# sarpaykent/GotenNet

Measured on AMD Instinct MI355X. Metric: molecules/sec (energy+force forward), rMD17 aspirin batch=128, 1/2/4/8 MI355X, higher is better.
Workload: dtype f32 (2xfp16-split MFMA with block exponents, fp32 accumulate); 1 GPU; rmd17_aspirin batch=128/GPU (N=2688 atoms, E=54368 edges incl. self-loops), n_atom_basis=256, n_interactions=6, lmax=2, n_rbf=32, heads=8, sep_dir/sep_tensor, energy+forces; global_batch=128, parallelism=dp1 (molecule shards, 1 all-reduce)

## Files before the change

gotennet_amd/_lib.py:

```python
from __future__ import annotations

import ctypes as C
import os

_PKG = os.path.dirname(os.path.abspath(__file__))
LIB_PATH = os.environ.get("GN_LIB_PATH") or os.path.join(_PKG, "libgotennet_hip.so")

GN_ERR_BAD_ARG = 10001
ABI_VERSION = 11
LMAX_SLICED = 0x100
LMAX_MEAN, LMAX_MAX = 0x200, 0x400

ACT_NONE = 11
_P, _I, _F, _L, _D = C.c_void_p, C.c_int, C.c_float, C.c_long, C.c_double

class GemmDesc(C.Structure):
    _fields_ = [("A", _P), ("lda", _I), ("W", _P), ("bias", _P), ("C", _P), ("ldc", _I),
                ("M", _I), ("N", _I), ("K", _I), ("act_lo", _I), ("act_hi", _I),
                ("row_cnt", _I), ("row_gstride", _I), ("row_goff", _I),
                ("res", _P), ("gate", _P), ("gate_mode", _I), ("pre_out", _P),
                ("pro_mode", _I), ("pro_lo", _I), ("pro_hi", _I), ("a_pre", _P), ("ldp", _I),
                ("a_gate", _P), ("ldg", _I), ("A2", _P), ("A3", _P), ("a_seg", _I), ("act_kind", _I), ("lda2", _I)]


class WgradDesc(C.Structure):
    _fields_ = [("dY", _P), ("ldy", _I), ("y_off", _I), ("A", _P), ("lda", _I), ("a_off", _I),
                ("dW", _P), ("ldw", _I), ("db", _P), ("rows", _I), ("nout", _I), ("K", _I),
                ("row_cnt", _I), ("row_gstride", _I), ("row_goff", _I)]


SIGNATURES = {
    "gn_abi_version": [C.POINTER(C.c_char_p)],
    "gn_build_csr": [_P, _I, _I, _P, _P, _P, _P],
    "gn_check_edges": [_P, _I, _I, _P, _P],
    "gn_build_csc": [_P, _P, _I, _I, _P, _P, _P, _P, _P],
    "gn_molecule_ptr": [_P, _I, _I, _P, _P],
    "gn_cosine_cutoff": [_P, _I, _F, _P, _P],
    "gn_out_degree": [_P, _I, _P, _P],
    "gn_edge_geometry": [_P, _P, _P, _P, _I, _I, _I, _I, _P, _P, _F, _P, _P, _P, _P],
    "gn_node_init": [_P, _P, _P, _P, _I, _P, _P, _P, _I, _I, _P, _P],
    "gn_edge_init": [_P, _P, _P, _P, _I, _I, _I, _P, _P],
    "gn_layernorm_silu": [_P, _P, _P, _F, _I, _I, _P, _I, _P],
    "gn_layernorm": [_P, _P, _P, _F, _I, _I, _P, _P],
    "gn_tensor_norm": [_P, _P, _F, _I, _I, _I, _P, _P],
    "gn_gemm": [_P, _I, _P, _P, _P, _I, _I, _I, _I, _I, _I, _I, _I, _I, _P, _P, _P],
    "gn_attn_softmax": [_P, _P, _I, _P, _I, _P, _P, _P, _I, _I, _I, _P, _I, _P],
    "gn_attn_softmax_dropout": [_P, _P, _I, _P, _I, _P, _P, _P, _I, _I, _I, _P, _P, _P, _I, _D, _I, _P],
    "gn_attn_dropout_mask": [_P, _I, _D, _L, _I, _P, _P],
    "gn_message_aggregate": [_P, _P, _I, _P, _I, _P, _P, _P, _P, _P, _P, _P, _P, _P, _I, _I, _I, _I, _I, _I, _P],
    "gn_eqff_fused_supported": [_I, _I, _I],
    "gn_eqff_fused_forward": [_P, _P, _P, _P, _P, _F, _I, _I, _I, _P, _P, _P, _P, _P, _I, _P],
    "gn_eqff_fused_backward": [_P, _P, _P, _P, _P, _P, _P, _P, _I, _I, _I, _P, _P, _I, _P],
    "gn_htr_edge": [_P, _P, _P, _P, _P, _I, _I, _I, _I, _P, _P, _P],
    "gn_eqff_context": [_P, _P, _F, _I, _I, _I, _P, _P],
    "gn_eqff_update": [_P, _P, _I, _I, _I, _P, _P, _P],
    "gn_gemm_ex": [_P, _I, _P, _P, _P, _I, _I, _I, _I, _I, _I, _I, _I, _I, _P, _P, _I, _P, _I, _I, _I, _P, _I, _P, _I, _I, _P],
    "gn_gemm_group": [_P, _I, _P],
    "gn_edge_vectors": [_P, _P, _P, _I, _P, _P, _P],
    "gn_gemm_split": [_P, _I, _P, _P, _P, _I, _I, _I, _I, _I, _I, _I, _I, _I, _P, _P, _I, _P, _I, _I, _I, _P, _I, _P, _I, _I, _P],
    "gn_split_bf16x3": [_P, _I, _I, _P, _P],
    "gn_split_bf16x3_size": [_I, _I],
    "gn_gemm_group_split": [_P, _I, _P],
    "gn_gemm_f16x2": [_P, _I, _P, _P, _P, _I, _I, _I, _I, _I, _I, _I, _I, _I, _P, _P, _I, _P, _I, _I, _I, _P, _I, _P, _I, _I, _P],
    "gn_split_f16x2": [_P, _I, _I, _P, _P],
    "gn_split_f16x2_size": [_I, _I],
    "gn_gemm_group_f16x2": [_P, _I, _P],
    "gn_htr_backward": [_P, _P, _P, _P, _P, _P, _P, _P, _P, _P, _P, _P, _I, _I, _I, _I, _P, _P, _P, _P, _I, _P],
    "gn_message_backward": [_P, _P, _I, _P, _I, _P, _P, _I, _P, _P, _P, _P, _P, _P, _P, _P, _P, _P, _P,
                            _P, _P, _P, _I, _P, _P, _P, _P, _P, _P, C.c_long, _I, _I, _I, _I, _I, _I, _I, _P],
    "gn_message_backward_dropout": [_P, _P, _I, _P, _I, _P, _P, _P, _I, _P, _P, _P, _P, _P, _P, _P, _P, _P, _P, _P,
                                    _P, _P, _P, _I, _P, _P, _P, _P, _P, _P, C.c_long, _I, _I, _I, _I, _I, _I, _I, _P],
    "gn_message_backward_groups": [_I, _I, _I, _I],
    "gn_eqff_backward_a": [_P, _P, _P, _P, _I, _I, _I, _P, _P, _P],
    "gn_eqff_backward_b": [_P, _P, _P, _P, _I, _I, _I, _P, _P, _P],
    "gn_edge_init_backward": [_P, _P, _P, _I, _P, _P, _P, _P, _I, _I, _P, _P, _P],
    "gn_node_init_backward": [_P, _P, _P, _I, _P, _P, _P, _P, _I, _I, _P, _P, _P],
    "gn_layernorm_silu_backward": [_P, _P, _P, _F, _P, _I, _I, _P, _I, _P],
    "gn_layernorm_backward": [_P, _P, _F, _P, _I, _I, _P, _P],
    "gn_tensor_norm_backward": [_P, _P, _P, _F, _I, _I, _I, _P, _P],
    "gn_gate": [_P, _I, _L, _P, _P],
    "gn_gate_backward": [_P, _P, _I, _L, _P, _P],
    "gn_edge_gate_backward": [_P, _P, _I, _P, _L, _P, _P, _P],
    "gn_edge_geometry_backward": [_P, _P, _P, _P, _I, _I, _I, _I, _P, _P, _F, _P, _I, _P, _I, _P, _P, _P, _P],
    "gn_pos_scatter": [_P, _P, _P, _P, _P, _P, _I, _F, _P, _P],
    "gn_head_energy": [_P, _P, _F, _F, _F, _F, _P, _P, _P, _I, _I, _P, _P, _I, _P, _I, _P],
    "gn_head_grad": [_P, _P, _F, _P, _I, _I, _P, _I, _P],
    "gn_geb_context": [_P, _I, _I, _P, _I, _I, _I, _P, _I, _P],
    "gn_geb_gate": [_P, _I, _I, _I, _P, _I, _I, _I, _I, _P, _I, _P, _I, _P],
    "gn_dipole_reduce": [_P, _I, _P, _I, _P, _P, _I, _F, _F, _I, _I, _P, _P, _P],
    "gn_ese_reduce": [_P, _P, _P, _P, _I, _P, _I, _P, _P],
    "gn_radius_count": [_P, _P, _I, _F, _I, _P, _P],
    "gn_radius_fill": [_P, _P, _I, _F, _I, _P, C.c_int64, _P, _P, _P, _P],
    "gn_weight_grad_workspace": [_P, _I],
    "gn_weight_grad_group": [_P, _I, _P, _L, _P],
    "gn_embedding_grad": [_P, _P, _I, _P, _P, _P, _P, _P, _P, _I, _I, _I, _P, _P, _P, _P],
    "gn_layernorm_param_grad_workspace": [_I, _I],
    "gn_layernorm_param_grad": [_P, _P, _P, _F, _P, _I, _I, _I, _P, _P, _P, _P],
}

_LONG_RESULT = ("gn_split_bf16x3_size", "gn_split_f16x2_size", "gn_weight_grad_workspace", "gn_layernorm_param_grad_workspace")

_lib = None


class GotenNetHipError(RuntimeError):
    pass


def load():
    global _lib
    if _lib is not None:
        return _lib
    if not os.path.exists(LIB_PATH):
        raise GotenNetHipError(
            f"{LIB_PATH} is missing: the HIP extension has not been built "
            "(python gotennet_amd/build.py). There is no CPU fallback.")
    lib = C.CDLL(LIB_PATH)
    for name, argtypes in SIGNATURES.items():
        fn = getattr(lib, name)
        fn.argtypes = argtypes
        fn.restype = C.c_long if name in _LONG_RESULT else C.c_int
    if lib.gn_abi_version(None) != ABI_VERSION:
        raise GotenNetHipError("libgotennet_hip.so ABI version mismatch; rebuild")
    _lib = lib
    return lib


TIMER = None


def call(name: str, *args) -> None:
    t = TIMER
    tag = t.want(name, args) if t is not None else None
    if tag is not None:
        import torch
        e0, e1 = torch.cuda.Event(enable_timing=True), torch.cuda.Event(enable_timing=True)
        e0.record()
        rc = getattr(load(), name)(*args)
        e1.record()
        t.events.append((tag, e0, e1))
    else:
        rc = getattr(load(), name)(*args)
    if rc != 0:
        what = "unsupported shape/flag combination" if rc == GN_ERR_BAD_ARG else f"hipError_t {rc}"
        raise GotenNetHipError(f"{name} failed: {what}")


def ptr(t) -> int:
    return None if t is None else t.data_ptr()
```

gotennet_amd/csrc/gn_backward.hip:

```cpp
#include "gn_common.h"
#include "gn_tune.h"
#include "gn_sh.h"
#include "gn_highl.h"

namespace gn {



template <int LMAX, int FC = 0>
__global__ __launch_bounds__(256) GN_WPE(GN_W_HTR_TGT) void htr_bwd_target_kernel(
    const float* __restrict__ gtp, const float* __restrict__ pre_t, const float* __restrict__ w,
    const float* __restrict__ EQ, const float* __restrict__ EK, const float* __restrict__ rl,
    const int* __restrict__ rowptr, const int* __restrict__ src, int N, int F_rt,
    float* __restrict__ gEQ, float* __restrict__ g_rl, float* __restrict__ g_pre_t, int ) {
    constexpr int act = GN_ACT_SILU;
    constexpr int D = (LMAX + 1) * (LMAX + 1) - 1;
    constexpr int KP = D <= 4 ? 4 : (D <= 8 ? 8 : (D <= 16 ? 16 : 32));
    constexpr int CH = D < 9 ? D : 9;
    __shared__ __attribute__((aligned(16))) float red[CH * 1024];
    const int F = FC ? FC : F_rt;
    const int i = xcd_item(blockIdx.x, N);
    if (i < 0) return;
    GN_SLOT_GEOMETRY(FC);
    const int e0 = rowptr[i], e1 = rowptr[i + 1];
    float4 eq[D], acc[D];
#pragma unroll
    for (int m = 0; m < D; ++m) { eq[m] = ld4(EQ + ((size_t)i * D + m) * F + c0); acc[m] = zero4(); }
    for (int e = e0 + slot; e < e1; e += ns) {
        const float4 gte = ld4(gtp + (size_t)e * F + c0), pte = ld4(pre_t + (size_t)e * F + c0);
        float4 a_pt, d_pt;
        act_pair4(pte, act, a_pt, d_pt);
        const float4 gw = gte * a_pt;
        st4(g_pre_t + (size_t)e * F + c0, gte * ld4_nt(w + (size_t)e * F + c0) * d_pt);
        const float* kj = EK + (size_t)src[e] * D * F + c0;
        const float* re = rl + (size_t)e * D;
        float part[KP];
#pragma unroll
        for (int m = D; m < KP; ++m) part[m] = 0.f;
        int m0 = 0;
#pragma unroll
        for (int l = 1; l <= LMAX; ++l) {
            float4 ek[2 * LMAX + 1];
            float r[2 * LMAX + 1];
            float4 pa = zero4(), pb = zero4();
            float rr = 0.f;
#pragma unroll
            for (int mm = 0; mm < 2 * l + 1; ++mm) {
                ek[mm] = ld4(kj + (size_t)(m0 + mm) * F);
                r[mm] = re[m0 + mm];
                pa = fma4(r[mm], eq[m0 + mm], pa);
                pb = fma4(r[mm], ek[mm], pb);
                rr = fmaf(r[mm], r[mm], rr);
            }
            const float c = 2.0f - rr;
            const float4 u = gw * pb * (-c), v = gw * pa * (-c), s2 = gw * (pa * pb) * 2.0f;
#pragma unroll
            for (int mm = 0; mm < 2 * l + 1; ++mm) {
                acc[m0 + mm] = fma4(r[mm], u, fma4(gw, ek[mm], acc[m0 + mm]));
                part[m0 + mm] = hsum4(fma4(r[mm], s2, fma4(v, ek[mm], u * eq[m0 + mm])));
            }
            m0 += 2 * l + 1;
        }
        if (lps >= KP) {
            multi_group_sum<KP>(part, lps, lp);
            const int stride = lps / KP;
            if ((lp & (stride - 1)) == 0 && lp / stride < D) g_rl[(size_t)e * D + lp / stride] = part[0];
        } else {
#pragma unroll
            for (int m = 0; m < D; ++m) {
                const float s = group_sum(part[m], lps);
                if (lp == 0) g_rl[(size_t)e * D + m] = s;
            }
        }
    }
    reduce_rows<D>(acc, red, slot, c0, F, ns, [&](int row, float4 s) { st4(gEQ + ((size_t)i * D + row) * F + c0, s); });
}

template <int LMAX, int FC = 0>
__global__ __launch_bounds__(256) GN_WPE(GN_W_HTR_SRC) void htr_bwd_source_kernel(
    const float* __restrict__ gtp, const float* __restrict__ pre_t,
    const float* __restrict__ EQ, const float* __restrict__ EK, const float* __restrict__ rl,
    const int* __restrict__ colptr, const int* __restrict__ perm, const int* __restrict__ dst, int N, int F_rt,
    float* __restrict__ gEK, int ) {
    constexpr int act = GN_ACT_SILU;
    constexpr int D = (LMAX + 1) * (LMAX + 1) - 1;
    constexpr int CH = D < 9 ? D : 9;
    __shared__ __attribute__((aligned(16))) float red[CH * 1024];
    const int F = FC ? FC : F_rt;
    const int j = xcd_item(blockIdx.x, N);
    if (j < 0) return;
    GN_SLOT_GEOMETRY(FC);
    const int p0 = colptr[j], p1 = colptr[j + 1];
    float4 ek[D], acc[D];
#pragma unroll
    for (int m = 0; m < D; ++m) { ek[m] = ld4(EK + ((size_t)j * D + m) * F + c0); acc[m] = zero4(); }
    for (int pp = p0 + slot; pp < p1; pp += ns) {
        const int e = perm[pp];
        const float4 gw = ld4(gtp + (size_t)e * F + c0) * act4(ld4(pre_t + (size_t)e * F + c0), act);
        const float* qi = EQ + (size_t)dst[pp] * D * F + c0;
        const float* re = rl + (size_t)e * D;
        int m0 = 0;
#pragma unroll
        for (int l = 1; l <= LMAX; ++l) {
            float4 eq[2 * LMAX + 1];
            float r[2 * LMAX + 1];
            float4 pa = zero4();
            float rr = 0.f;
#pragma unroll
            for (int mm = 0; mm < 2 * l + 1; ++mm) {
                eq[mm] = ld4(qi + (size_t)(m0 + mm) * F);
                r[mm] = re[m0 + mm];
                pa = fma4(r[mm], eq[mm], pa);
                rr = fmaf(r[mm], r[mm], rr);
            }
            const float4 v = gw * pa * (rr - 2.0f);
#pragma unroll
            for (int mm = 0; mm < 2 * l + 1; ++mm)
                acc[m0 + mm] = fma4(r[mm], v, fma4(gw, eq[mm], acc[m0 + mm]));
            m0 += 2 * l + 1;
        }
    }
    reduce_rows<D>(acc, red, slot, c0, F, ns, [&](int row, float4 s) { st4(gEK + ((size_t)j * D + row) * F + c0, s); });
}

template <int LMAX, bool SEP_DIR, bool SEP_TENSOR>
struct MsgShape {
    static constexpr int D = (LMAX + 1) * (LMAX + 1) - 1;
    static constexpr int ND = SEP_DIR ? LMAX : 1;
    static constexpr int NT = SEP_TENSOR ? LMAX : 1;
    static constexpr int M = 1 + ND + NT;
    __host__ __device__ static constexpr bool is_dir(int b) { return b >= 1 && b < 1 + ND; }
    __host__ __device__ static constexpr int lo(int b) { return is_dir(b) ? (SEP_DIR ? b : 1) : (SEP_TENSOR ? b - ND : 1); }
    __host__ __device__ static constexpr int hi(int b) { return is_dir(b) ? (SEP_DIR ? b : LMAX) : (SEP_TENSOR ? b - ND : LMAX); }
    __host__ __device__ static constexpr int first_row(int l) { return l * l - 1; }
};


constexpr int GS_CAP = 2048;
template <int LMAX, bool SEP_DIR, bool SEP_TENSOR, bool GS_LDS, bool FIRST, int FC>
__device__ __forceinline__ void msg_bwd_target_body(const MsgBwdArgs& p, float* gsl, float* red, float* hsum, const float* __restrict__ x_, const float* __restrict__ v_, const float* __restrict__ eproj_, const float* __restrict__ a_, const float* __restrict__ qk_, const float* __restrict__ X_in_, const float* __restrict__ rl_, const float* __restrict__ cut_, const int* __restrict__ outdeg_, const float* __restrict__ g_h1_, const float* __restrict__ g_X1_, const int* __restrict__ rowptr_, const int* __restrict__ src_, float* __restrict__ g_eproj_, float* __restrict__ g_s_, float* __restrict__ g_nproj_, float* __restrict__ g_rl_, float* __restrict__ g_cut_) {
    using S = MsgShape<LMAX, SEP_DIR, SEP_TENSOR>;
    constexpr int D = S::D, M = S::M;
    constexpr int KP = D <= 4 ? 4 : (D <= 8 ? 8 : (D <= 16 ? 16 : 32));
    const int N = p.N, F = FC ? FC : p.F, H = p.H;
    const int i = xcd_item(blockIdx.x, N);
    if (i < 0) return;
    GN_SLOT_GEOMETRY(FC);
    const int e0 = rowptr_[i], e1 = rowptr_[i + 1];
    const int per_head = (M * F) / H;
    int hb[M];
#pragma unroll
    for (int b = 0; b < M; ++b) hb[b] = (b * F + c0) / per_head;
    auto GS = [&](int e, int h) -> float& {
        if constexpr (GS_LDS) return gsl[(e - e0) * H + h];
        else return g_s_[(size_t)e * H + h];
    };

    const float4 gdh = ld4(g_h1_ + (size_t)i * F + c0);
    float4 gdX[D];
#pragma unroll
    for (int m = 0; m < D; ++m) gdX[m] = ld4(g_X1_ + ((size_t)i * D + m) * F + c0);

    for (int e = e0 + slot; e < e1; e += ns) {
        const int j = src_[e];
        const float ce = cut_[e];
        const float* xr = x_ + (size_t)j * p.ldxv + c0;
        const float* vr = v_ + (size_t)j * p.ldxv + c0;
        const float* tr = eproj_ + (size_t)e * p.lde + F + c0;
        float* gtr = g_eproj_ + (size_t)e * p.lde + F + c0;
        const float* ar = a_ + (size_t)e * H;
        const float* Xj = X_in_ + (size_t)j * D * F + c0;
        const float* re = rl_ + (size_t)e * D;
        float pa_h[M];
        float cutp = 0.f;
        float rlp[D];
#pragma unroll
        for (int b = 0; b < M; ++b) {
            if (FIRST && b > 0 && !S::is_dir(b)) { pa_h[b] = 0.f; continue; }
            float4 go;
            if (b == 0) {
                go = gdh;
            } else {
                go = zero4();
#pragma unroll
                for (int l = S::lo(b); l <= S::hi(b); ++l)
#pragma unroll
                    for (int m = S::first_row(l); m < S::first_row(l) + 2 * l + 1; ++m)
                        go = S::is_dir(b) ? fma4(re[m], gdX[m], go) : fma4(gdX[m], ld4(Xj + (size_t)m * F), go);
            }
            const float4 tfb = ld4(tr + b * F), xb = ld4(xr + b * F), vb = ld4(vr + b * F);
            st4_nt(gtr + b * F, (go * xb) * ce);
            cutp += hsum4(go * tfb * xb);
            pa_h[b] = hsum4(go * vb);
            if (S::is_dir(b)) {
                const float4 od = fma4(ar[hb[b]], vb, (tfb * xb) * ce);
#pragma unroll
                for (int l = S::lo(b); l <= S::hi(b); ++l)
#pragma unroll
                    for (int m = S::first_row(l); m < S::first_row(l) + 2 * l + 1; ++m) rlp[m] = hsum4(gdX[m] * od);
            }
        }
        cutp = group_sum(cutp, lps);
        if (lp == 0) g_cut_[e] = cutp;
        {
            float* hrow = hsum + slot * (M * lps);
#pragma unroll
            for (int b = 0; b < M; ++b) hrow[b * lps + lp] = pa_h[b];
            const int rpl = lps / H, hh = lp / rpl, part = lp - hh * rpl;
            const float* hp = hrow + hh * (M * rpl) + part * M;
            float hv = hp[0];
#pragma unroll
            for (int k = 1; k < M; ++k) hv += hp[k];
            hv = group_sum(hv, rpl);
            if (part == 0) GS(e, hh) = hv;
        }
// ... 817 lines not shown
        if (basis == 0) {
            const float u = expf(alpha * (-d));
            auto term = [&](int r, float gp) {
                const float w = u - means[r];
                const float G = expf(-betas[r] * (w * w));
                s += gp * G * (dc + c * (2.0f * betas[r] * w * alpha * u));
            };
            if ((R & 3) == 0) {
                for (int r = 0; r < R; r += 4) {
                    const float4 gp = ld4(g_phi + (size_t)e * R + r);
                    term(r, gp.x); term(r + 1, gp.y); term(r + 2, gp.z); term(r + 3, gp.w);
                }
            } else {
                for (int r = 0; r < R; ++r) term(r, g_phi[(size_t)e * R + r]);
            }
        }
        float gc = 0.f;
        int q = 0;
        for (; q + 4 <= n_cut; q += 4) {
            const float c0 = g_cut[(size_t)q * E + e], c1 = g_cut[(size_t)(q + 1) * E + e];
            const float c2 = g_cut[(size_t)(q + 2) * E + e], c3 = g_cut[(size_t)(q + 3) * E + e];
            gc += c0; gc += c1; gc += c2; gc += c3;
        }
        for (; q < n_cut; ++q) gc += g_cut[(size_t)q * E + e];
        gd += s + gc * dc;
    }
    g_diff[e] = gd;
    const float x = vec[3 * e], y = vec[3 * e + 1], z = vec[3 * e + 2];
    const float n = sqrtf(x * x + y * y + z * z);
    const float ux = x / n, uy = y / n, uz = z / n;
    Dual3 o[D];
    real_harmonics<LMAX, Dual3>(Dual3{ux, {1.f, 0.f, 0.f}}, Dual3{uy, {0.f, 1.f, 0.f}}, Dual3{uz, {0.f, 0.f, 1.f}}, o);
    float gsum[D];
#pragma unroll
    for (int m = 0; m < D; ++m) gsum[m] = 0.f;
#pragma unroll 2
    for (int q = 0; q < n_rl; ++q) {
        const float* row = g_rl + ((size_t)q * E + e) * D;
        if constexpr (D % 4 == 0) {
#pragma unroll
            for (int m = 0; m < D; m += 4) {
                const float4 v = ld4(row + m);
                gsum[m] += v.x; gsum[m + 1] += v.y; gsum[m + 2] += v.z; gsum[m + 3] += v.w;
            }
        } else {
#pragma unroll
            for (int m = 0; m < D; ++m) gsum[m] += row[m];
        }
    }
    float gu0 = 0.f, gu1 = 0.f, gu2 = 0.f;
#pragma unroll
    for (int m = 0; m < D; ++m) {
        gu0 += gsum[m] * o[m].d[0]; gu1 += gsum[m] * o[m].d[1]; gu2 += gsum[m] * o[m].d[2];
    }
    const float dotp = gu0 * ux + gu1 * uy + gu2 * uz;
    g_vec[3 * e] = (gu0 - dotp * ux) / n;
    g_vec[3 * e + 1] = (gu1 - dotp * uy) / n;
    g_vec[3 * e + 2] = (gu2 - dotp * uz) / n;
}

__global__ __launch_bounds__(256) void pos_scatter_kernel(const float* __restrict__ g_vec, const float* __restrict__ g_diff,
                                                          const float* __restrict__ vec,
                                                          const int* __restrict__ rowptr, const int* __restrict__ colptr,
                                                          const int* __restrict__ perm, int N, float sign, float* __restrict__ g_pos) {
    const int n = blockIdx.x * 4 + (threadIdx.x >> 6), lane = threadIdx.x & 63;
    if (n >= N) return;
    float sx = 0.f, sy = 0.f, sz = 0.f;
    auto add = [&](int e, float w) {
        const float x = vec[3 * e], y = vec[3 * e + 1], z = vec[3 * e + 2];
        const float gd = g_diff[e];
        float rx = g_vec[3 * e], ry = g_vec[3 * e + 1], rz = g_vec[3 * e + 2];
        if (gd != 0.f) {
            const float q = gd / sqrtf(x * x + y * y + z * z);
            rx += q * x; ry += q * y; rz += q * z;
        }
        sx += w * rx; sy += w * ry; sz += w * rz;
    };
    const int p0 = colptr[n], p1 = colptr[n + 1], e0 = rowptr[n], e1 = rowptr[n + 1];
    for (int pp = p0 + lane; pp < p1; pp += 64) add(perm[pp], 1.0f);
    for (int e = e0 + lane; e < e1; e += 64) add(e, -1.0f);
    sx = wave_sum(sx); sy = wave_sum(sy); sz = wave_sum(sz);
    if (lane == 0) {
        g_pos[3 * n] = sign * sx;
        g_pos[3 * n + 1] = sign * sy;
        g_pos[3 * n + 2] = sign * sz;
    }
}

__global__ __launch_bounds__(1024) void head_energy_kernel(
    const float* __restrict__ pre1, const float* __restrict__ W2, float b2, float scale, float shift, float mol_shift,
    const float* __restrict__ atomref, const int* __restrict__ z, const int* __restrict__ mol_ptr,
    int Hd, float* __restrict__ y, float* __restrict__ energy, int mean, float* __restrict__ atom_scale, int act) {
    const int b = blockIdx.x;
    const int n0 = mol_ptr[b], n1 = mol_ptr[b + 1];
    const int wave = threadIdx.x >> 6, lane = threadIdx.x & 63;
    for (int n = n0 + wave; n < n1; n += 16) {
        float s = 0.f;
        for (int k = lane; k < Hd; k += 64) s += act1(pre1[(size_t)n * Hd + k], act) * W2[k];
        s = wave_sum(s);
        if (lane == 0) y[n] = (s + b2) * scale + shift + (atomref ? atomref[z[n]] : 0.f);
    }
    __syncthreads();
    if (wave == 0) {
        float s = 0.f;
        for (int n = n0 + lane; n < n1; n += 64) s += y[n];
        s = wave_sum(s);
        if (lane == 0) energy[b] = ((mean && n1 > n0) ? s / (float)(n1 - n0) : s) + mol_shift;
    }
    if (atom_scale)
        for (int n = n0 + (int)threadIdx.x; n < n1; n += 1024) atom_scale[n] = mean ? 1.0f / (float)(n1 - n0) : 1.0f;
}

__global__ void head_grad_kernel(const float* __restrict__ pre1, const float* __restrict__ W2, float scale,
                                 const float* __restrict__ atom_scale, int N, int Hd, float* __restrict__ gpre1, int act) {
    const size_t idx = (size_t)blockIdx.x * blockDim.x + threadIdx.x;
    if (idx >= (size_t)N * Hd) return;
    const float sc = atom_scale ? scale * atom_scale[idx / Hd] : scale;
    gpre1[idx] = sc * W2[idx % Hd] * dact1(pre1[idx], act);
}

}

static bool bwd_dim_ok_wide(int F) { return F >= 16 && F <= 1024 && gn::is_pow2(F); }

#define GN_SWITCH_LMAX(KERNEL, grid, block, st, ...)                                                   \
    switch (lmax) {                                                                                    \
        case 1: hipLaunchKernelGGL(gn::KERNEL<1>, grid, block, 0, st, __VA_ARGS__); break;             \
        case 2: hipLaunchKernelGGL(gn::KERNEL<2>, grid, block, 0, st, __VA_ARGS__); break;             \
        case 3: hipLaunchKernelGGL(gn::KERNEL<3>, grid, block, 0, st, __VA_ARGS__); break;             \
        default: hipLaunchKernelGGL(gn::KERNEL<4>, grid, block, 0, st, __VA_ARGS__); break;            \
    }

#define GN_SWITCH_LMAX8(KERNEL, grid, block, st, ...)                                                  \
    switch (lmax) {                                                                                    \
        case 1: hipLaunchKernelGGL(gn::KERNEL<1>, grid, block, 0, st, __VA_ARGS__); break;             \
        case 2: hipLaunchKernelGGL(gn::KERNEL<2>, grid, block, 0, st, __VA_ARGS__); break;             \
        case 3: hipLaunchKernelGGL(gn::KERNEL<3>, grid, block, 0, st, __VA_ARGS__); break;             \
        case 4: hipLaunchKernelGGL(gn::KERNEL<4>, grid, block, 0, st, __VA_ARGS__); break;             \
        case 5: hipLaunchKernelGGL(gn::KERNEL<5>, grid, block, 0, st, __VA_ARGS__); break;             \
        case 6: hipLaunchKernelGGL(gn::KERNEL<6>, grid, block, 0, st, __VA_ARGS__); break;             \
        case 7: hipLaunchKernelGGL(gn::KERNEL<7>, grid, block, 0, st, __VA_ARGS__); break;             \
        default: hipLaunchKernelGGL(gn::KERNEL<8>, grid, block, 0, st, __VA_ARGS__); break;            \
    }

extern "C" int gn_htr_backward(const float* g_t_out, const float* pre_t, const float* w, const float* w_raw,
                               const float* EQ,
                               const float* EK, const float* rl, const int* rowptr, const int* src, const int* dst,
                               const int* colptr, const int* perm, int N, int F, int lmax_arg, int mode,
                               float* gEQ, float* gEK, float* g_rl, float* g_pre_t, int act, void* stream) {
    const int lmax = lmax_arg & 0xff;
    if ((lmax_arg & ~(0xff | GN_LMAX_SLICED)) || !bwd_dim_ok_wide(F) || N < 0 || lmax < 1 || lmax > 8 || mode < 0 || mode > 31 ||
        act < 0 || act >= GN_ACT_COUNT)
        return GN_ERR_BAD_ARG;
    if (N == 0) return GN_OK;
    hipStream_t st = (hipStream_t)stream;
    if (gn_use_highl(lmax_arg) || F > 256 || (!mode && act != GN_ACT_SILU))
        return gn_highl_htr_backward(g_t_out, pre_t, w, w_raw, EQ, EK, rl, rowptr, src, dst, colptr, perm, N, F, lmax,
                                     mode, gEQ, gEK, g_rl, g_pre_t, act, st);
    if (mode)
        return gn_htr_backward_general(g_t_out, pre_t, w, w_raw, EQ, EK, rl, rowptr, src, dst, colptr, perm, N, F, lmax,
                                       mode, gEQ, gEK, g_rl, g_pre_t, act, st);
    const dim3 grid(gn::xcd_grid(N)), block(256);
#define GN_HTRB_T(L, LLO, LHI, FIRST, FC)                                                                        \
    hipLaunchKernelGGL((gn::htr_bwd_target_group_kernel<L, LLO, LHI, FIRST, FC>), grid, block, 0, st, g_t_out, pre_t, w, \
                       EQ, EK, rl, rowptr, src, N, F, gEQ, g_rl, g_pre_t, act)
#define GN_HTRB_S(L, LLO, LHI, FC)                                                                               \
    hipLaunchKernelGGL((gn::htr_bwd_source_group_kernel<L, LLO, LHI, FC>), grid, block, 0, st, g_t_out, pre_t, EQ, EK, \
                       rl, colptr, perm, dst, N, F, gEK, act)
#define GN_HTRB(L, LLO, LHI, FIRST, FC) GN_HTRB_T(L, LLO, LHI, FIRST, FC); GN_HTRB_S(L, LLO, LHI, FC)
#define GN_HTRB_ALL(FC)                                                                                          \
    if (lmax == 1) {                                                                                             \
        hipLaunchKernelGGL((gn::htr_bwd_target_kernel<1, FC>), grid, block, 0, st, g_t_out, pre_t, w, EQ, EK, rl, rowptr, src, N, F, gEQ, g_rl, g_pre_t, act); \
        hipLaunchKernelGGL((gn::htr_bwd_source_kernel<1, FC>), grid, block, 0, st, g_t_out, pre_t, EQ, EK, rl, colptr, perm, dst, N, F, gEK, act); \
    } else if (lmax == 2) {                                                                                      \
        hipLaunchKernelGGL((gn::htr_bwd_target_kernel<2, FC>), grid, block, 0, st, g_t_out, pre_t, w, EQ, EK, rl, rowptr, src, N, F, gEQ, g_rl, g_pre_t, act); \
        hipLaunchKernelGGL((gn::htr_bwd_source_kernel<2, FC>), grid, block, 0, st, g_t_out, pre_t, EQ, EK, rl, colptr, perm, dst, N, F, gEK, act); \
    } else if (lmax == 3) {                                                                                      \
        if (GN_HTRB_TGT_MODE == 1) { GN_HTRB_T(3, 1, 3, true, FC); }                                             \
        else { GN_HTRB_T(3, 1, 2, true, FC); GN_HTRB_T(3, 3, 3, false, FC); }                                    \
        if (GN_HTRB_SRC_ONE) { GN_HTRB_S(3, 1, 3, FC); }                                                         \
        else { GN_HTRB_S(3, 1, 2, FC); GN_HTRB_S(3, 3, 3, FC); }                                                 \
    } else {                                                                                                     \
        GN_HTRB_T(4, 1, 2, true, FC);                                                                            \
        if (GN_HTRB_TGT_MODE == 1) { GN_HTRB_T(4, 3, 4, false, FC); }                                            \
        else { GN_HTRB_T(4, 3, 3, false, FC); GN_HTRB_T(4, 4, 4, false, FC); }                                   \
        if (GN_HTRB_SRC_ONE) { GN_HTRB_S(4, 1, 4, FC); }                                                         \
        else { GN_HTRB_S(4, 1, 2, FC); GN_HTRB_S(4, 3, 3, FC); GN_HTRB_S(4, 4, 4, FC); }                         \
    }
    if (F == 256) { GN_HTRB_ALL(256) } else { GN_HTRB_ALL(0) }
    GN_LAUNCH_CHECK();
    return GN_OK;
}

template <int L, int LLO, int LHI, bool SC, int FC>
static inline void gn_launch_msg_bwd_group(dim3 grid, dim3 block, hipStream_t st, const gn::MsgBwdArgs& p, float* ga_slice, float* cut_slice) {
    if constexpr (LLO == 3 && LHI == 3)
        hipLaunchKernelGGL((gn::msg_bwd_merged_group3_kernel<L, LLO, LHI, SC, FC>), grid, block, 0, st, p, ga_slice, cut_slice);
    else
        hipLaunchKernelGGL((gn::msg_bwd_merged_group_kernel<L, LLO, LHI, SC, FC>), grid, block, 0, st, p, ga_slice, cut_slice);
}
template <int L, bool SD, bool ST, int FC>
static inline void gn_launch_msg_bwd_merged(dim3 grid, dim3 block, hipStream_t st, const gn::MsgBwdArgs& p, float* ga_parts) {
    if constexpr (!(L >= 3 && SD && ST))
        hipLaunchKernelGGL((gn::msg_bwd_merged_kernel<L, SD, ST, FC>), grid, block, 0, st, p, ga_parts);
}
#define GN_MSGB_LAUNCH_FC(L, SD, ST, FC)                                                                 \
    do {                                                                                                  \
        if (!X_in) {                                                                                      \
            if (GN_MSGB_MERGED_FIRST && ga_parts != nullptr) {    \
                hipLaunchKernelGGL((gn::msg_bwd_merged_first_kernel<L, SD, ST, FC>), grid, block, 0, st, p, ga_parts); \
                hipLaunchKernelGGL(gn::attn_bwd_kernel<FC>, grid, block, 0, st, p, ga_parts, 1, (size_t)0); \
                hipLaunchKernelGGL(gn::msg_bwd_gk_kernel<FC>, grid, block, 0, st, p);                     \
                break;                                                                                    \
            }                                                                                             \
            hipLaunchKernelGGL((gn::msg_bwd_target_kernel<L, SD, ST, true, FC>), grid, block, 0, st, p);  \
            hipLaunchKernelGGL((gn::msg_bwd_source_kernel<L, SD, ST, true, FC>), grid, block, 0, st, p);  \
            break;                                                                                        \
        }                                                                                                 \
        if (GN_MSGB_MERGED && ga_parts != nullptr) {      \
            gn_launch_msg_bwd_merged<L, SD, ST, FC>(grid, block, st, p, ga_parts);                        \
            hipLaunchKernelGGL(gn::attn_bwd_kernel<FC>, grid, block, 0, st, p, ga_parts, 1, (size_t)0);   \
            hipLaunchKernelGGL(gn::msg_bwd_gk_kernel<FC>, grid, block, 0, st, p);                         \
            break;                                                                                        \
        }                                                                                                 \
        hipLaunchKernelGGL((gn::msg_bwd_target_kernel<L, SD, ST>), grid, block, 0, st, p);                \
        hipLaunchKernelGGL((gn::msg_bwd_source_kernel<L, SD, ST>), grid, block, 0, st, p);                \
    } while (0)
#define GN_MSGB_LAUNCH(L, SD, ST) GN_MSGB_LAUNCH_FC(L, SD, ST, 0)
#define GN_MSGB_LAUNCH_DEFAULT(L)                                                                        \
    do {                                                                                                  \
        if (F == 256) GN_MSGB_LAUNCH_FC(L, true, true, 256); else GN_MSGB_LAUNCH_FC(L, true, true, 0);    \
    } while (0)

extern "C" int gn_message_backward_groups(int lmax_arg, int sep_dir, int sep_tensor, int act) {
    const int lmax = lmax_arg & 0xff;
    if (gn_use_highl(lmax_arg) || act != GN_ACT_SILU) return 1;
    return (lmax >= 3 && sep_dir && sep_tensor) ? lmax - 1 : 1;
}

static int message_backward(
    const float* x, const float* v, int ldxv, const float* eproj, int lde, const float* a,
    const float* qk, int ldqk, const float* X_in, const float* rl, const float* cut, const int* outdeg,
    const float* g_h1, const float* g_X1,
    const int* rowptr, const int* src, const int* dst, const int* colptr, const int* perm,
    float* g_eproj, float* g_s, float* g_nproj, int ldn, float* g_x, float* g_v, float* g_X_out,
    float* g_rl, float* g_cut, float* ga_parts, long E,
    int N, int F, int H, int lmax_arg, int sep_dir, int sep_tensor, int act, void* stream, const float* a_soft) {
    const int lmax = lmax_arg & 0xff;
    const bool amax = (lmax_arg & GN_LMAX_MAX) != 0;
    if (amax && ((lmax_arg & GN_LMAX_MEAN) || !ga_parts || !X_in)) return GN_ERR_BAD_ARG;
    if ((lmax_arg & ~(0xff | GN_LMAX_SLICED | GN_LMAX_MEAN | GN_LMAX_MAX)) || !bwd_dim_ok_wide(F) || N < 0 || H <= 0 || !gn::is_pow2(H) || (F / 4) % H || (F / 4) / H > 64 || lmax < 1 || lmax > 8 ||
        (ldxv & 3) || (lde & 3) || (ldqk & 3) || (ldn & 3) || g_X_out == g_X1 || act < 0 || act >= GN_ACT_COUNT)
        return GN_ERR_BAD_ARG;
    if (!X_in && (act != GN_ACT_SILU || gn_use_highl(lmax_arg) || F > 256)) return GN_ERR_BAD_ARG;
    if (N == 0) return GN_OK;
    gn::MsgBwdArgs p{x, v, ldxv, eproj, lde, a, qk, ldqk, X_in, rl, cut, outdeg, g_h1, g_X1,
                     rowptr, src, dst, colptr, perm, g_eproj, g_s, g_nproj, ldn, g_x, g_v, g_X_out, g_rl, g_cut,
                     N, F, H, (float)(1.0 / sqrt((double)F)), act, (lmax_arg & GN_LMAX_MEAN) ? 1 : 0, amax ? ga_parts : nullptr, a_soft};
    hipStream_t st = (hipStream_t)stream;
    const dim3 grid(gn::xcd_grid(N)), block(256);
    if (gn_use_highl(lmax_arg) || F > 256 || act != GN_ACT_SILU) return gn_highl_message_backward(p, lmax, sep_dir, sep_tensor, st);
    if (X_in && gn_message_backward_groups(lmax_arg, sep_dir, sep_tensor, act) > 1) {
        if (ga_parts == nullptr || E <= 0) return GN_ERR_BAD_ARG;
        const size_t gs = (size_t)E * H;
#define GN_MSGB_M(L, LLO, LHI, SC, G, FC)                                                                    \
    gn_launch_msg_bwd_group<L, LLO, LHI, SC, FC>(grid, block, st, p, ga_parts + (size_t)(G) * gs, g_cut + (size_t)(G) * E)
#define GN_MSGB_GROUPS(FC)                                                                                       \
        if (lmax == 3) { GN_MSGB_M(3, 1, 2, true, 0, FC); GN_MSGB_M(3, 3, 3, false, 1, FC); }                    \
        else { GN_MSGB_M(4, 1, 2, true, 0, FC); GN_MSGB_M(4, 3, 3, false, 1, FC); GN_MSGB_M(4, 4, 4, false, 2, FC); } \
        hipLaunchKernelGGL(gn::attn_bwd_kernel<FC>, grid, block, 0, st, p, ga_parts, lmax - 1, gs);              \
        hipLaunchKernelGGL(gn::msg_bwd_gk_kernel<FC>, grid, block, 0, st, p);
        if (F == 256) { GN_MSGB_GROUPS(256) } else { GN_MSGB_GROUPS(0) }
        GN_LAUNCH_CHECK();
        return GN_OK;
    }
    const int key = lmax * 4 + (sep_dir ? 2 : 0) + (sep_tensor ? 1 : 0);
    switch (key) {
        case 4: case 5: case 6: case 7:
            if (F == 256) GN_MSGB_LAUNCH_FC(1, false, false, 256); else GN_MSGB_LAUNCH(1, false, false);
            break;
        case 8: GN_MSGB_LAUNCH(2, false, false); break;
        case 9: GN_MSGB_LAUNCH(2, false, true); break;
        case 10: GN_MSGB_LAUNCH(2, true, false); break;
        case 11: GN_MSGB_LAUNCH_DEFAULT(2); break;
        case 12: GN_MSGB_LAUNCH(3, false, false); break;
        case 13: GN_MSGB_LAUNCH(3, false, true); break;
        case 14: GN_MSGB_LAUNCH(3, true, false); break;
        case 15: GN_MSGB_LAUNCH_DEFAULT(3); break;
        case 16: GN_MSGB_LAUNCH(4, false, false); break;
        case 17: GN_MSGB_LAUNCH(4, false, true); break;
        case 18: GN_MSGB_LAUNCH(4, true, false); break;
        default: GN_MSGB_LAUNCH_DEFAULT(4); break;
    }
    GN_LAUNCH_CHECK();
    return GN_OK;
}

extern "C" int gn_message_backward(
    const float* x, const float* v, int ldxv, const float* eproj, int lde, const float* a,
    const float* qk, int ldqk, const float* X_in, const float* rl, const float* cut, const int* outdeg,
    const float* g_h1, const float* g_X1,
    const int* rowptr, const int* src, const int* dst, const int* colptr, const int* perm,
    float* g_eproj, float* g_s, float* g_nproj, int ldn, float* g_x, float* g_v, float* g_X_out,
    float* g_rl, float* g_cut, float* ga_parts, long E,
    int N, int F, int H, int lmax_arg, int sep_dir, int sep_tensor, int act, void* stream) {
    return message_backward(x, v, ldxv, eproj, lde, a, qk, ldqk, X_in, rl, cut, outdeg, g_h1, g_X1, rowptr, src, dst, colptr,
                            perm, g_eproj, g_s, g_nproj, ldn, g_x, g_v, g_X_out, g_rl, g_cut, ga_parts, E, N, F, H, lmax_arg,
                            sep_dir, sep_tensor, act, stream, nullptr);
}

extern "C" int gn_message_backward_dropout(
    const float* x, const float* v, int ldxv, const float* eproj, int lde, const float* a, const float* a_soft,
    const float* qk, int ldqk, const float* X_in, const float* rl, const float* cut, const int* outdeg,
    const float* g_h1, const float* g_X1,
    const int* rowptr, const int* src, const int* dst, const int* colptr, const int* perm,
    float* g_eproj, float* g_s, float* g_nproj, int ldn, float* g_x, float* g_v, float* g_X_out,
    float* g_rl, float* g_cut, float* ga_parts, long E,
    int N, int F, int H, int lmax_arg, int sep_dir, int sep_tensor, int act, void* stream) {
    if (!a_soft) return GN_ERR_BAD_ARG;
    return message_backward(x, v, ldxv, eproj, lde, a, qk, ldqk, X_in, rl, cut, outdeg, g_h1, g_X1, rowptr, src, dst, colptr,
                            perm, g_eproj, g_s, g_nproj, ldn, g_x, g_v, g_X_out, g_rl, g_cut, ga_parts, E, N, F, H, lmax_arg,
                            sep_dir, sep_tensor, act, stream, a_soft);
}

extern "C" int gn_eqff_backward_a(const float* g_h, const float* g_X, const float* m, const float* Xp,
                                  int N, int F, int D, float* g_m, float* g_Xp, void* stream) {
    if (N < 0 || F <= 0 || (F & 3) || D <= 0) return GN_ERR_BAD_ARG;
    if (N == 0) return GN_OK;
// ... 107 lines not shown
```

gotennet_amd/csrc/gn_gata.hip:

```cpp
#include "gn_common.h"
#include "gn_tune.h"
#include "gn_highl.h"
#include "gn_dropout.h"

namespace gn {

constexpr int ATTN_CAP = 2048;
template <bool IN_LDS, bool ASILU, bool DROP = false>
__device__ __forceinline__ void attn_softmax_body(
    const float* __restrict__ q, const float* __restrict__ k, int ldqk, const float* __restrict__ ta, int ldt,
    const int* __restrict__ src, const int* __restrict__ outdeg, int i, int e0, int e1, int F, int H, float inv_sqrt_f,
    float* __restrict__ a, float* sc, int act, const AttnDrop drop = AttnDrop{}) {
    unsigned dk0 = 0, dk1 = 0;
    if constexpr (DROP) {
        const unsigned long long key = (unsigned long long)drop.key[0];
        dk0 = (unsigned)key, dk1 = (unsigned)(key >> 32);
    }
    auto mult = [&](size_t n) { return drop_mult(dk0, dk1, drop.layer, drop.thresh, drop.scale, drop.all, n); };
    const int lps = F >> 2, ns = 256 / lps;
    const int slot = threadIdx.x / lps, lp = threadIdx.x % lps, c0 = lp * 4;
    const int lph = lps / H;
    auto S = [&](int e, int h) -> float& {
        if constexpr (IN_LDS) return sc[(e - e0) * H + h];
        else if constexpr (DROP) return drop.a_soft[(size_t)e * H + h];
        else return a[(size_t)e * H + h];
    };
    const float4 qi = ld4(q + (size_t)i * ldqk + c0);
    for (int e = e0 + slot; e < e1; e += 2 * ns) {
        const int eb = e + ns < e1 ? e + ns : e;
        const int ja = src[e], jb = src[eb];
        const float4 ka = ld4(k + (size_t)ja * ldqk + c0), kb = ld4(k + (size_t)jb * ldqk + c0);
        const float4 ta_ = act4(ld4_nt(ta + (size_t)e * ldt + c0), act);
        const float4 tb_ = act4(ld4_nt(ta + (size_t)eb * ldt + c0), act);
        float pa = qi.x * ka.x * ta_.x;
        pa += qi.y * ka.y * ta_.y;
        pa += qi.z * ka.z * ta_.z;
        pa += qi.w * ka.w * ta_.w;
        float pb = qi.x * kb.x * tb_.x;
        pb += qi.y * kb.y * tb_.y;
        pb += qi.z * kb.z * tb_.z;
        pb += qi.w * kb.w * tb_.w;
        pa = group_sum(pa, lph);
        pb = group_sum(pb, lph);
        if ((lp & (lph - 1)) == 0) {
            S(e, lp / lph) = pa;
            if (eb != e) S(eb, lp / lph) = pb;
        }
    }
    __syncthreads();
    const int wave = threadIdx.x >> 6, lane = threadIdx.x & 63;
    for (int h = wave; h < H; h += 4) {
        float mx = -INFINITY;
        for (int e = e0 + lane; e < e1; e += 64) mx = fmaxf(mx, S(e, h));
        mx = wave_max(mx);
        float sm = 0.f;
        for (int e = e0 + lane; e < e1; e += 64) {
            const float ex = fast_exp(S(e, h) - mx);
            S(e, h) = ex;
            sm += ex;
        }
        const float rsm = __builtin_amdgcn_rcpf(wave_sum(sm) + 1e-16f);
        for (int e = e0 + lane; e < e1; e += 64) {
            const float nrm = outdeg ? sqrtf((float)outdeg[src[e]]) * inv_sqrt_f : inv_sqrt_f;
            S(e, h) = S(e, h) * rsm * nrm;
            if constexpr (DROP && !IN_LDS) a[(size_t)e * H + h] = S(e, h) * mult((size_t)e * H + h);
        }
    }
    if constexpr (IN_LDS) {
        __syncthreads();
        const int n = (e1 - e0) * H;
        for (int idx = threadIdx.x; idx < n; idx += 256) {
            if constexpr (DROP) {
                drop.a_soft[(size_t)e0 * H + idx] = sc[idx];
                a[(size_t)e0 * H + idx] = sc[idx] * mult((size_t)e0 * H + idx);
            } else {
                a[(size_t)e0 * H + idx] = sc[idx];
            }
        }
    }
}

template <bool ASILU>
__global__ __launch_bounds__(256) GN_WPE(GN_W_ATTN) void attn_softmax_kernel(
    const float* __restrict__ q, const float* __restrict__ k, int ldqk,
    const float* __restrict__ ta, int ldt,
    const int* __restrict__ rowptr, const int* __restrict__ src, const int* __restrict__ outdeg,
    int N, int F, int H, float inv_sqrt_f, float* __restrict__ a, int act_rt) {
    __shared__ float sc[ATTN_CAP];
    const int act = ASILU ? (int)GN_ACT_SILU : act_rt;
    const int i = xcd_item(blockIdx.x, N);
    if (i < 0) return;
    const int e0 = rowptr[i], e1 = rowptr[i + 1];
    if ((e1 - e0) * H <= ATTN_CAP)
        attn_softmax_body<true, ASILU>(q, k, ldqk, ta, ldt, src, outdeg, i, e0, e1, F, H, inv_sqrt_f, a, sc, act);
    else
        attn_softmax_body<false, ASILU>(q, k, ldqk, ta, ldt, src, outdeg, i, e0, e1, F, H, inv_sqrt_f, a, sc, act);
}

template <bool ASILU>
__global__ __launch_bounds__(256) void attn_softmax_drop_kernel(
    const float* __restrict__ q, const float* __restrict__ k, int ldqk,
    const float* __restrict__ ta, int ldt,
    const int* __restrict__ rowptr, const int* __restrict__ src, const int* __restrict__ outdeg,
    int N, int F, int H, float inv_sqrt_f, float* __restrict__ a, int act_rt, const AttnDrop drop) {
    __shared__ float sc[ATTN_CAP];
    const int act = ASILU ? (int)GN_ACT_SILU : act_rt;
    const int i = xcd_item(blockIdx.x, N);
    if (i < 0) return;
    const int e0 = rowptr[i], e1 = rowptr[i + 1];
    if ((e1 - e0) * H <= ATTN_CAP)
        attn_softmax_body<true, ASILU, true>(q, k, ldqk, ta, ldt, src, outdeg, i, e0, e1, F, H, inv_sqrt_f, a, sc, act, drop);
    else
        attn_softmax_body<false, ASILU, true>(q, k, ldqk, ta, ldt, src, outdeg, i, e0, e1, F, H, inv_sqrt_f, a, sc, act, drop);
}

constexpr int ATTN_W_STRIP = 512;
template <bool IN_LDS, bool ASILU, int FC, bool DROP = false>
__device__ __forceinline__ void attn_softmax_wave_body(
    const float* __restrict__ q, const float* __restrict__ k, int ldqk, const float* __restrict__ ta, int ldt,
    const int* __restrict__ src, const int* __restrict__ outdeg, int i, int e0, int e1, int F_rt, int H, float inv_sqrt_f,
    float* __restrict__ a, float* sc, int act, const AttnDrop drop = AttnDrop{}) {
    const int F = FC ? FC : F_rt;
    const int lane = threadIdx.x & 63;
    const int lps = F >> 2, ns = 64 / lps;
    const int slot = FC == 256 ? 0 : lane / lps, lp = lane % lps, c0 = lp * 4;
    const int lph = lps / H;
    float* const S = IN_LDS ? sc : (DROP ? drop.a_soft : a) + (size_t)e0 * H;
    const int n = (e1 - e0) * H;
    const float4 qi = ld4(q + (size_t)i * ldqk + c0);
    constexpr int U = 8;
    for (int eb = e0; eb < e1; eb += U * ns) {
        float4 kj[U], te[U];
        int ee[U];
#pragma unroll
        for (int u = 0; u < U; ++u) {
            const int e = eb + u * ns + slot;
            ee[u] = e < e1 ? e : e1 - 1;
            kj[u] = ld4(k + (size_t)src[ee[u]] * ldqk + c0);
            te[u] = ld4_nt(ta + (size_t)ee[u] * ldt + c0);
        }
#pragma unroll
        for (int u = 0; u < U; ++u) {
            const float4 t4 = act4(te[u], act);
            float p = qi.x * kj[u].x * t4.x;
            p += qi.y * kj[u].y * t4.y;
            p += qi.z * kj[u].z * t4.z;
            p += qi.w * kj[u].w * t4.w;
            p = group_sum(p, lph);
            if ((lp & (lph - 1)) == 0 && eb + u * ns + slot < e1) S[(ee[u] - e0) * H + lp / lph] = p;
        }
    }
    if constexpr (!IN_LDS) __builtin_amdgcn_s_waitcnt(0);
    __builtin_amdgcn_wave_barrier();
    float mx = -INFINITY;
    for (int idx = lane; idx < n; idx += 64) mx = fmaxf(mx, S[idx]);
    mx = stride_max(mx, H);
// ... 107 lines not shown
    for (int e = e0 + slot; e < e1; e += ns) {
        const int j = src[e];
        const float ce = cut[e];
        const float* xr = x + (size_t)j * ldxv + c0;
        const float* vr = v + (size_t)j * ldxv + c0;
        const float* tr = tf + (size_t)e * ldt + c0;
        const float* ar = a + (size_t)e * H;
        const float* Xj = X_in + (size_t)j * D * F + c0;
        const float* re = rl + (size_t)e * D;
        float4 o[M];
#pragma unroll
        for (int b = 0; b < (FIRST ? 1 + ND : M); ++b) {
            const float4 sp = (ld4_nt(tr + b * F) * ld4(xr + b * F)) * ce;
            const float ab = ar[hb[b]];
            o[b] = fma4(ab, ld4(vr + b * F), sp);
        }
        acc[0] = acc[0] + o[0];
        int m = 0;
#pragma unroll
        for (int l = 1; l <= LMAX; ++l) {
            const float4 od = o[SEP_DIR ? l : 1];
#pragma unroll
            for (int mm = 0; mm < 2 * l + 1; ++mm, ++m) {
                if constexpr (FIRST)
                    acc[1 + m] = acc[1 + m] + od * re[m];
                else
                    acc[1 + m] = acc[1 + m] + fma4(ld4(Xj + (size_t)m * F), o[1 + ND + (SEP_TENSOR ? l - 1 : 0)], od * re[m]);
            }
        }
    }

#pragma unroll
    for (int base = 0; base < ROWS; base += CH) {
        if (base) __syncthreads();
#pragma unroll
        for (int r = 0; r < CH; ++r)
            if (base + r < ROWS) st4(&red[r * 1024 + slot * F + c0], acc[base + r]);
        __syncthreads();
        for (int r = slot; r < CH && base + r < ROWS; r += ns) {
            const float4 s = red4(red + r * 1024, c0, F, ns);
            const int row = base + r;
            if (row == 0) {
                st4(h_out + (size_t)i * F + c0, ld4(h_in + (size_t)i * F + c0) + s);
            } else {
                const size_t off = ((size_t)i * D + (row - 1)) * F + c0;
                if constexpr (FIRST) st4(X_out + off, s);
                else st4(X_out + off, ld4(X_in + off) + s);
            }
        }
    }
}

template <int LMAX, bool SEP_DIR, bool SEP_TENSOR, int LLO, int LHI, bool SCALAR, int FC>
__device__ __forceinline__ void message_aggregate_group_body(
    const float* __restrict__ x, const float* __restrict__ v, int ldxv,
    const float* __restrict__ tf, int ldt, const float* __restrict__ a,
    const float* __restrict__ rl, const float* __restrict__ cut,
    const int* __restrict__ rowptr, const int* __restrict__ src,
    const float* __restrict__ h_in, const float* __restrict__ X_in,
    float* __restrict__ h_out, float* __restrict__ X_out, int N, int F_rt, int H) {
    constexpr int D = (LMAX + 1) * (LMAX + 1) - 1;
    constexpr int ND = SEP_DIR ? LMAX : 1;
    constexpr int NT = SEP_TENSOR ? LMAX : 1;
    constexpr int M = 1 + ND + NT;
    constexpr int XROWS = (LHI + 1) * (LHI + 1) - LLO * LLO;
    constexpr int ROWS = (SCALAR ? 1 : 0) + XROWS;
    constexpr int M0 = LLO * LLO - 1;
    constexpr int CH = ROWS < GN_K6G_CH ? ROWS : GN_K6G_CH;
    __shared__ __attribute__((aligned(16))) float red[CH * 1024];

    const int F = FC ? FC : F_rt;
    const int i = xcd_item(blockIdx.x, N);
    if (i < 0) return;
    GN_SLOT_GEOMETRY(FC);
    const int e0 = rowptr[i], e1 = rowptr[i + 1];
    const int per_head = (M * F) / H;

    int hb[M];
#pragma unroll
    for (int b = 0; b < M; ++b) hb[b] = (b * F + c0) / per_head;

    float4 acc[ROWS];
#pragma unroll
    for (int r = 0; r < ROWS; ++r) acc[r] = zero4();

    for (int e = e0 + slot; e < e1; e += ns) {
        const int j = src[e];
        const float ce = cut[e];
        const float* xr = x + (size_t)j * ldxv + c0;
        const float* vr = v + (size_t)j * ldxv + c0;
        const float* tr = tf + (size_t)e * ldt + c0;
        const float* ar = a + (size_t)e * H;
        const float* Xj = X_in + (size_t)j * D * F + c0;
        const float* re = rl + (size_t)e * D;
        auto gate = [&](int b) {
            const float4 sp = (ld4_nt(tr + b * F) * ld4(xr + b * F)) * ce;
            const float ab = ar[hb[b]];
            return fma4(ab, ld4(vr + b * F), sp);
        };
        constexpr int NL = LHI - LLO + 1;
        float4 gd[NL], gt[NL];
#pragma unroll
        for (int l = LLO; l <= LHI; ++l) {
            gd[l - LLO] = (SEP_DIR || l == LLO) ? gate(SEP_DIR ? l : 1) : gd[0];
            gt[l - LLO] = (SEP_TENSOR || l == LLO) ? gate(1 + ND + (SEP_TENSOR ? l - 1 : 0)) : gt[0];
        }
        if (SCALAR) acc[0] = acc[0] + gate(0);
#pragma unroll
        for (int l = LLO; l <= LHI; ++l) {
#pragma unroll
            for (int mm = 0; mm < 2 * l + 1; ++mm) {
                const int m = l * l - 1 + mm;
                acc[(SCALAR ? 1 : 0) + m - M0] = acc[(SCALAR ? 1 : 0) + m - M0] +
                                                 fma4(ld4(Xj + (size_t)m * F), gt[l - LLO], gd[l - LLO] * re[m]);
            }
        }
    }

#pragma unroll
    for (int base = 0; base < ROWS; base += CH) {
        if (base) __syncthreads();
#pragma unroll
        for (int r = 0; r < CH; ++r)
            if (base + r < ROWS) st4(&red[r * 1024 + slot * F + c0], acc[base + r]);
        __syncthreads();
        for (int r = slot; r < CH && base + r < ROWS; r += ns) {
            const float4 s = red4(red + r * 1024, c0, F, ns);
            const int row = base + r;
            if (SCALAR && row == 0) {
                st4(h_out + (size_t)i * F + c0, ld4(h_in + (size_t)i * F + c0) + s);
            } else {
                const size_t off = ((size_t)i * D + (M0 + row - (SCALAR ? 1 : 0))) * F + c0;
                st4(X_out + off, ld4(X_in + off) + s);
            }
        }
    }
}

#define GN_MSG_GROUP_ARGS                                                                                   \
    const float *__restrict__ x, const float *__restrict__ v, int ldxv, const float *__restrict__ tf, int ldt,            \
        const float *__restrict__ a, const float *__restrict__ rl, const float *__restrict__ cut, const int *__restrict__ rowptr,    \
        const int *__restrict__ src, const float *__restrict__ h_in, const float *__restrict__ X_in,                     \
        float *__restrict__ h_out, float *__restrict__ X_out, int N, int F, int H
#define GN_MSG_GROUP_PASS x, v, ldxv, tf, ldt, a, rl, cut, rowptr, src, h_in, X_in, h_out, X_out, N, F, H
template <int LMAX, bool SEP_DIR, bool SEP_TENSOR, int LLO, int LHI, bool SCALAR, int FC = 0>
__global__ __launch_bounds__(256) GN_WPE(GN_W_K6_G) void message_aggregate_group_kernel(GN_MSG_GROUP_ARGS) {
    message_aggregate_group_body<LMAX, SEP_DIR, SEP_TENSOR, LLO, LHI, SCALAR, FC>(GN_MSG_GROUP_PASS);
}
template <int LMAX, bool SEP_DIR, bool SEP_TENSOR, int LLO, int LHI, bool SCALAR, int FC = 0>
__global__ __launch_bounds__(256) GN_WPE(GN_W_K6_G34) void message_aggregate_group34_kernel(GN_MSG_GROUP_ARGS) {
    message_aggregate_group_body<LMAX, SEP_DIR, SEP_TENSOR, LLO, LHI, SCALAR, FC>(GN_MSG_GROUP_PASS);
}

template <int LMAX, int FC = 0>
__global__ __launch_bounds__(256) GN_WPE(GN_W_HTR_EDGE) void htr_edge_kernel(
    const float* __restrict__ EQ, const float* __restrict__ EK, const float* __restrict__ rl,
    const int* __restrict__ rowptr, const int* __restrict__ src, int N, int F_rt, float* __restrict__ w) {
    constexpr int D = (LMAX + 1) * (LMAX + 1) - 1;
    constexpr bool CLOSED = LMAX == 3 && GN_HTR_CLOSED;
    const int F = FC ? FC : F_rt;
    const int i = xcd_item(blockIdx.x, N);
    if (i < 0) return;
    GN_SLOT_GEOMETRY(FC);
    const int e0 = rowptr[i], e1 = rowptr[i + 1];
    float4 eq[D];
#pragma unroll
    for (int m = 0; m < D; ++m) eq[m] = ld4(EQ + ((size_t)i * D + m) * F + c0);
    for (int e = e0 + slot; e < e1; e += ns) {
        const float* kj = EK + (size_t)src[e] * D * F + c0;
        const float* re = rl + (size_t)e * D;
        float4 wsum = zero4();
        int m0 = 0;
#if GN_HTR_CLOSED_ALL
        if constexpr (LMAX >= GN_HTR_CLOSED_ALL) {
            float4 eka[D];
            float ra[D];
#pragma unroll
            for (int m = 0; m < D; ++m) { eka[m] = ld4(kj + (size_t)m * F); ra[m] = re[m]; }
            __builtin_amdgcn_sched_barrier(0);
#pragma unroll
            for (int l = 1; l <= LMAX; ++l) {
                float4 pq = zero4(), pk = zero4(), ab = zero4();
                float rr = 0.f;
#pragma unroll
                for (int mm = 0; mm < 2 * l + 1; ++mm) {
                    const int m = l * l - 1 + mm;
                    rr = fmaf(ra[m], ra[m], rr);
                    pq = fma4(ra[m], eq[m], pq);
                    pk = fma4(ra[m], eka[m], pk);
                    ab = fma4(eq[m], eka[m], ab);
                }
                wsum = wsum + (ab + (pq * pk) * (rr - 2.0f));
            }
            st4_nt(w + (size_t)e * F + c0, wsum);
            continue;
        }
#endif
#pragma unroll
        for (int l = 1; l <= LMAX; ++l) {
            float4 ek[2 * LMAX + 1];
            float r[2 * LMAX + 1];
            float4 pq = zero4(), pk = zero4();
            if constexpr (CLOSED) {
                float4 ab = zero4();
                float rr = 0.f;
#pragma unroll
                for (int mm = 0; mm < 2 * l + 1; ++mm) {
                    ek[mm] = ld4(kj + (size_t)(m0 + mm) * F);
                    r[mm] = re[m0 + mm];
                }
#pragma unroll
                for (int mm = 0; mm < 2 * l + 1; ++mm) {
                    rr = fmaf(r[mm], r[mm], rr);
                    pq = fma4(r[mm], eq[m0 + mm], pq);
                    pk = fma4(r[mm], ek[mm], pk);
                    ab = fma4(eq[m0 + mm], ek[mm], ab);
                }
                wsum = wsum + (ab + (pq * pk) * (rr - 2.0f));
            } else {
#pragma unroll
                for (int mm = 0; mm < 2 * l + 1; ++mm) {
                    ek[mm] = ld4(kj + (size_t)(m0 + mm) * F);
                    r[mm] = re[m0 + mm];
                    pq = fma4(r[mm], eq[m0 + mm], pq);
                    pk = fma4(-r[mm], ek[mm], pk);
                }
#pragma unroll
                for (int mm = 0; mm < 2 * l + 1; ++mm) {
                    const float4 a_ = eq[m0 + mm] + pq * (-r[mm]);
                    const float4 b_ = ek[mm] + pk * r[mm];
                    wsum = fma4(a_, b_, wsum);
                }
            }
            m0 += 2 * l + 1;
        }
        st4_nt(w + (size_t)e * F + c0, wsum);
    }
}

}

static bool feature_dim_ok(int F) { return F >= 16 && F <= 1024 && gn::is_pow2(F); }

extern "C" int gn_attn_softmax(const float* q, const float* k, int ldqk, const float* t_attn, int ldt,
                               const int* rowptr, const int* src, const int* outdeg,
                               int N, int F, int H, float* a, int act, void* stream) {
    if (!feature_dim_ok(F) || N < 0 || H <= 0 || !gn::is_pow2(H) || (F / 4) % H || (F / 4) / H > 64 ||
        (ldqk & 3) || (ldt & 3) || act < 0 || act >= GN_ACT_COUNT)
        return GN_ERR_BAD_ARG;
    if (N == 0) return GN_OK;
    const float inv_sqrt_f = (float)(1.0 / sqrt((double)F));
    if (GN_ATTN_WAVE && F <= 256 && H <= 64) {
        const dim3 grid(gn::xcd_grid((N + 3) / 4)), block(256);
        if (act == GN_ACT_SILU && F == 256)
            hipLaunchKernelGGL((gn::attn_softmax_wave_kernel<true, 256>), grid, block, 0, (hipStream_t)stream,
                               q, k, ldqk, t_attn, ldt, rowptr, src, outdeg, N, F, H, inv_sqrt_f, a, act);
        else if (act == GN_ACT_SILU)
            hipLaunchKernelGGL(gn::attn_softmax_wave_kernel<true>, grid, block, 0, (hipStream_t)stream,
                               q, k, ldqk, t_attn, ldt, rowptr, src, outdeg, N, F, H, inv_sqrt_f, a, act);
        else
            hipLaunchKernelGGL(gn::attn_softmax_wave_kernel<false>, grid, block, 0, (hipStream_t)stream,
                               q, k, ldqk, t_attn, ldt, rowptr, src, outdeg, N, F, H, inv_sqrt_f, a, act);
        GN_LAUNCH_CHECK();
        return GN_OK;
    }
    if (act == GN_ACT_SILU)
        hipLaunchKernelGGL(gn::attn_softmax_kernel<true>, dim3(gn::xcd_grid(N)), dim3(256), 0, (hipStream_t)stream,
                           q, k, ldqk, t_attn, ldt, rowptr, src, outdeg, N, F, H, inv_sqrt_f, a, act);
    else
        hipLaunchKernelGGL(gn::attn_softmax_kernel<false>, dim3(gn::xcd_grid(N)), dim3(256), 0, (hipStream_t)stream,
                           q, k, ldqk, t_attn, ldt, rowptr, src, outdeg, N, F, H, inv_sqrt_f, a, act);
    GN_LAUNCH_CHECK();
    return GN_OK;
}

static bool drop_params(double p, unsigned& thresh, float& scale, int& all) {
    if (!(p >= 0.0)) return false;
    all = p >= 1.0 ? 1 : 0;
    thresh = all ? 0xffffffffu : (unsigned)floor(p * 4294967296.0);
    scale = all ? 0.f : (float)(1.0 / (1.0 - p));
    return true;
}

extern "C" int gn_attn_softmax_dropout(const float* q, const float* k, int ldqk, const float* t_attn, int ldt,
                                       const int* rowptr, const int* src, const int* outdeg,
                                       int N, int F, int H, float* a_soft, float* a, const long long* key, int layer, double p,
                                       int act, void* stream) {
    gn::AttnDrop d{a_soft, key, (unsigned)layer, 0u, 0.f, 0};
    if (!feature_dim_ok(F) || N < 0 || H <= 0 || !gn::is_pow2(H) || (F / 4) % H || (F / 4) / H > 64 ||
        (ldqk & 3) || (ldt & 3) || act < 0 || act >= GN_ACT_COUNT || !key || !a_soft || a_soft == a || layer < 0 ||
        !drop_params(p, d.thresh, d.scale, d.all))
        return GN_ERR_BAD_ARG;
    if (N == 0) return GN_OK;
    const float inv_sqrt_f = (float)(1.0 / sqrt((double)F));
    if (GN_ATTN_WAVE && F <= 256 && H <= 64) {
        const dim3 grid(gn::xcd_grid((N + 3) / 4)), block(256);
        if (act == GN_ACT_SILU)
            hipLaunchKernelGGL(gn::attn_softmax_drop_wave_kernel<true>, grid, block, 0, (hipStream_t)stream,
                               q, k, ldqk, t_attn, ldt, rowptr, src, outdeg, N, F, H, inv_sqrt_f, a, act, d);
        else
            hipLaunchKernelGGL(gn::attn_softmax_drop_wave_kernel<false>, grid, block, 0, (hipStream_t)stream,
                               q, k, ldqk, t_attn, ldt, rowptr, src, outdeg, N, F, H, inv_sqrt_f, a, act, d);
        GN_LAUNCH_CHECK();
        return GN_OK;
    }
    if (act == GN_ACT_SILU)
        hipLaunchKernelGGL(gn::attn_softmax_drop_kernel<true>, dim3(gn::xcd_grid(N)), dim3(256), 0, (hipStream_t)stream,
                           q, k, ldqk, t_attn, ldt, rowptr, src, outdeg, N, F, H, inv_sqrt_f, a, act, d);
    else
        hipLaunchKernelGGL(gn::attn_softmax_drop_kernel<false>, dim3(gn::xcd_grid(N)), dim3(256), 0, (hipStream_t)stream,
                           q, k, ldqk, t_attn, ldt, rowptr, src, outdeg, N, F, H, inv_sqrt_f, a, act, d);
    GN_LAUNCH_CHECK();
    return GN_OK;
}

extern "C" int gn_attn_dropout_mask(const long long* key, int layer, double p, long E, int H, float* m_out, void* stream) {
    unsigned thresh; float scale; int all;
    if (!key || layer < 0 || E < 0 || H <= 0 || !drop_params(p, thresh, scale, all)) return GN_ERR_BAD_ARG;
    const unsigned long long n = (unsigned long long)E * (unsigned long long)H;
    if (n == 0) return GN_OK;
    const unsigned long long blocks = (n + 255) / 256;
    hipLaunchKernelGGL(gn::attn_dropout_mask_kernel, dim3((unsigned)(blocks < 65536 ? blocks : 65536)), dim3(256), 0,
                       (hipStream_t)stream, key, (unsigned)layer, thresh, scale, all, n, m_out);
    GN_LAUNCH_CHECK();
    return GN_OK;
}

#define GN_MSG_ONE(L, SD, ST, LLO, LHI, SC, FC)                                                                 \
    hipLaunchKernelGGL((gn::message_aggregate_group_kernel<L, SD, ST, LLO, LHI, SC, FC>), dim3(gn::xcd_grid(N)), dim3(256), \
                       0, (hipStream_t)stream, x, v, ldxv, t_filter, ldt, a, rl, cut, rowptr, src, h_in, X_in,      \
                       h_out, X_out, N, F, H)
#define GN_MSG_MONO(L, SD, ST, FC)                                                                          \
    if (X_in)                                                                                                   \
        hipLaunchKernelGGL((gn::message_aggregate_kernel<L, SD, ST, false, FC>), dim3(gn::xcd_grid(N)), dim3(256), 0, \
                           (hipStream_t)stream, x, v, ldxv, t_filter, ldt, a, rl, cut, rowptr, src, h_in, X_in, \
                           h_out, X_out, N, F, H);                                                              \
    else                                                                                                        \
        hipLaunchKernelGGL((gn::message_aggregate_kernel<L, SD, ST, true, FC>), dim3(gn::xcd_grid(N)), dim3(256), 0,  \
                           (hipStream_t)stream, x, v, ldxv, t_filter, ldt, a, rl, cut, rowptr, src, h_in, X_in, \
                           h_out, X_out, N, F, H)
#define GN_MSG_LAUNCH_FC(L, SD, ST, FC)                                   \
    do {                                                                  \
        if (L <= 2 || !X_in) { GN_MSG_MONO(L, SD, ST, FC); }   \
        else {                                                            \
            GN_MSG_ONE(L, SD, ST, 1, 2, true, FC);                        \
            if constexpr (L >= 4 && GN_K6_MERGE34) {                      \
                hipLaunchKernelGGL((gn::message_aggregate_group34_kernel<L, SD, ST, 3, 4, false, FC>), dim3(gn::xcd_grid(N)), \
                                   dim3(256), 0, (hipStream_t)stream, x, v, ldxv, t_filter, ldt, a, rl, cut, rowptr, src, \
                                   h_in, X_in, h_out, X_out, N, F, H);    \
            }                                                             \
            else {                                                        \
                GN_MSG_ONE(L, SD, ST, 3, 3, false, FC);                   \
                if constexpr (L >= 4) { GN_MSG_ONE(L, SD, ST, 4, 4, false, FC); } \
            }                                                             \
        }                                                                 \
    } while (0)
#define GN_MSG_LAUNCH(L, SD, ST) GN_MSG_LAUNCH_FC(L, SD, ST, 0)
#define GN_MSG_LAUNCH_DEFAULT(L)                                                                 \
    do {                                                                                          \
        if (F == 256) GN_MSG_LAUNCH_FC(L, true, true, 256); else GN_MSG_LAUNCH_FC(L, true, true, 0); \
    } while (0)

extern "C" int gn_message_aggregate(const float* x, const float* v, int ldxv, const float* t_filter, int ldt,
                                    const float* a, const float* rl, const float* cut,
                                    const int* rowptr, const int* src,
                                    const float* h_in, const float* X_in, float* h_out, float* X_out,
                                    int N, int F, int H, int lmax_arg, int sep_dir, int sep_tensor, void* stream) {
    const int lmax = lmax_arg & 0xff;
    const int aggr = (lmax_arg & GN_LMAX_MEAN) ? 1 : ((lmax_arg & GN_LMAX_MAX) ? 2 : 0);
    if ((lmax_arg & ~(0xff | GN_LMAX_SLICED | GN_LMAX_MEAN | GN_LMAX_MAX)) ||
        ((lmax_arg & GN_LMAX_MEAN) && (lmax_arg & GN_LMAX_MAX)) || !feature_dim_ok(F) || N < 0 || H <= 0 || lmax < 1 ||
        lmax > 8 || (ldxv & 3) || (ldt & 3) || X_in == X_out)
        return GN_ERR_BAD_ARG;
    if (!X_in && gn_use_highl(lmax_arg)) return GN_ERR_BAD_ARG;
    const int M = 1 + (sep_dir ? lmax : 1) + (sep_tensor ? lmax : 1);
    if ((M * F) % H || ((M * F) / H) % 4) return GN_ERR_BAD_ARG;
    if (N == 0) return GN_OK;
    if (gn_use_highl(lmax_arg))
        return gn_highl_message(x, v, ldxv, t_filter, ldt, a, rl, cut, rowptr, src, h_in, X_in, h_out, X_out, N, F, H,
                                lmax, sep_dir, sep_tensor, aggr, (hipStream_t)stream);
    const int key = lmax * 4 + (sep_dir ? 2 : 0) + (sep_tensor ? 1 : 0);
    switch (key) {
        case 4: case 5: case 6: case 7:
            if (F == 256) GN_MSG_LAUNCH_FC(1, false, false, 256); else GN_MSG_LAUNCH(1, false, false);
            break;
        case 8: GN_MSG_LAUNCH(2, false, false); break;
        case 9: GN_MSG_LAUNCH(2, false, true); break;
        case 10: GN_MSG_LAUNCH(2, true, false); break;
        case 11: GN_MSG_LAUNCH_DEFAULT(2); break;
        case 12: GN_MSG_LAUNCH(3, false, false); break;
        case 13: GN_MSG_LAUNCH(3, false, true); break;
        case 14: GN_MSG_LAUNCH(3, true, false); break;
        case 15: GN_MSG_LAUNCH_DEFAULT(3); break;
        case 16: GN_MSG_LAUNCH(4, false, false); break;
        case 17: GN_MSG_LAUNCH(4, false, true); break;
        case 18: GN_MSG_LAUNCH(4, true, false); break;
        default: GN_MSG_LAUNCH_DEFAULT(4); break;
    }
    GN_LAUNCH_CHECK();
    return GN_OK;
}

extern "C" int gn_htr_edge(const float* EQ, const float* EK, const float* rl, const int* rowptr, const int* src,
                           int N, int F, int lmax_arg, int mode, float* w_raw, float* w, void* stream) {
    const int lmax = lmax_arg & 0xff;
    if ((lmax_arg & ~(0xff | GN_LMAX_SLICED)) || !feature_dim_ok(F) || N < 0 || lmax < 1 || lmax > 8 || mode < 0 || mode > 15)
        return GN_ERR_BAD_ARG;
    if (N == 0) return GN_OK;
    hipStream_t st = (hipStream_t)stream;
    if (gn_use_highl(lmax_arg)) return gn_highl_htr_edge(EQ, EK, rl, rowptr, src, N, F, lmax, mode, w_raw, w, st);
    if (mode) return gn_htr_edge_general(EQ, EK, rl, rowptr, src, N, F, lmax, mode, w_raw, w, st);
    const dim3 grid(gn::xcd_grid(N)), block(256);
#define GN_HTR_EDGE(FC)                                                                                                  \
    switch (lmax) {                                                                                                      \
        case 1: hipLaunchKernelGGL((gn::htr_edge_kernel<1, FC>), grid, block, 0, st, EQ, EK, rl, rowptr, src, N, F, w); break; \
        case 2: hipLaunchKernelGGL((gn::htr_edge_kernel<2, FC>), grid, block, 0, st, EQ, EK, rl, rowptr, src, N, F, w); break; \
        case 3: hipLaunchKernelGGL((gn::htr_edge_kernel<3, FC>), grid, block, 0, st, EQ, EK, rl, rowptr, src, N, F, w); break; \
        default: hipLaunchKernelGGL((gn::htr_edge_kernel<4, FC>), grid, block, 0, st, EQ, EK, rl, rowptr, src, N, F, w); break; \
    }
    if (F == 256) { GN_HTR_EDGE(256) } else { GN_HTR_EDGE(0) }
    GN_LAUNCH_CHECK();
    return GN_OK;
}
```

gotennet_amd/csrc/gn_gemm.h:

```cpp
#pragma once
#include "gn_common.h"

namespace gn {

typedef float f32x16 __attribute__((ext_vector_type(16)));

struct GemmArgs {
    const float* A; const float* W; const float* bias; float* C;
    const float* res; const float* gate; float* pre_out;
    const float* a_pre; const float* a_gate;
    int lda, ldc, ldp, ldg, M, N, K;
    int act_lo, act_hi;
    int pro_mode, pro_lo, pro_hi;
    int row_cnt, row_gstride, row_goff;
    int gate_mode;
    const float* A2; const float* A3; int a_seg;
    int nt_store;
    int act_kind;
    int lda2;
};

constexpr int GN_MAX_GROUP = 4;
struct GroupArgs {
    GemmArgs g[GN_MAX_GROUP];
    int tile_end[GN_MAX_GROUP];
    int n;
    int spread;
};

constexpr int BK = 32, PITCH = 36;

typedef __bf16 bf16x8 __attribute__((ext_vector_type(8)));
typedef __bf16 bf16x4 __attribute__((ext_vector_type(4)));
constexpr int SPLIT_PB = 40;

__device__ __forceinline__ unsigned pack_hi16(float a, float b) {
    return __builtin_amdgcn_perm(__float_as_uint(b), __float_as_uint(a), 0x07060302u);
}
__device__ __forceinline__ float trunc_bf16(float x) { return __uint_as_float(__float_as_uint(x) & 0xffff0000u); }
__device__ __forceinline__ void split4_trunc(float4 v, bf16x4& hi, bf16x4& mid, bf16x4& lo) {
    const float r0 = v.x - trunc_bf16(v.x), r1 = v.y - trunc_bf16(v.y);
    const float r2 = v.z - trunc_bf16(v.z), r3 = v.w - trunc_bf16(v.w);
    const float s0 = r0 - trunc_bf16(r0), s1 = r1 - trunc_bf16(r1);
    const float s2 = r2 - trunc_bf16(r2), s3 = r3 - trunc_bf16(r3);
    uint2 h, m, l;
    h.x = pack_hi16(v.x, v.y); h.y = pack_hi16(v.z, v.w);
    m.x = pack_hi16(r0, r1);   m.y = pack_hi16(r2, r3);
    l.x = pack_hi16(s0, s1);   l.y = pack_hi16(s2, s3);
    hi = __builtin_bit_cast(bf16x4, h);
    mid = __builtin_bit_cast(bf16x4, m);
    lo = __builtin_bit_cast(bf16x4, l);
}

typedef _Float16 f16x8 __attribute__((ext_vector_type(8)));
typedef _Float16 f16x4 __attribute__((ext_vector_type(4)));
typedef _Float16 f16x2 __attribute__((ext_vector_type(2)));
typedef float f32x2 __attribute__((ext_vector_type(2)));
__device__ __forceinline__ void split4_f16(float4 v, float scale , f16x4& hi, f16x4& lo) {
    const f32x2 a0 = f32x2{v.x, v.y} * scale, a1 = f32x2{v.z, v.w} * scale;
    const f16x2 h0 = __builtin_convertvector(a0, f16x2), h1 = __builtin_convertvector(a1, f16x2);
    const f16x2 l0 = __builtin_convertvector(a0 - __builtin_convertvector(h0, f32x2), f16x2);
    const f16x2 l1 = __builtin_convertvector(a1 - __builtin_convertvector(h1, f32x2), f16x2);
    hi = f16x4{h0.x, h0.y, h1.x, h1.y};
    lo = f16x4{l0.x, l0.y, l1.x, l1.y};
}

__device__ __forceinline__ unsigned wave_umax_sgpr(unsigned v) {
    auto mx = [](unsigned a, unsigned b) { return a > b ? a : b; };
    v = mx(v, (unsigned)__builtin_amdgcn_update_dpp(0, (int)v, 0x111, 0xf, 0xf, true));
    v = mx(v, (unsigned)__builtin_amdgcn_update_dpp(0, (int)v, 0x112, 0xf, 0xf, true));
    v = mx(v, (unsigned)__builtin_amdgcn_update_dpp(0, (int)v, 0x114, 0xf, 0xf, true));
    v = mx(v, (unsigned)__builtin_amdgcn_update_dpp(0, (int)v, 0x118, 0xf, 0xf, true));
    v = mx(v, (unsigned)__builtin_amdgcn_update_dpp(0, (int)v, 0x142, 0xa, 0xf, false));
    v = mx(v, (unsigned)__builtin_amdgcn_update_dpp(0, (int)v, 0x143, 0xc, 0xf, false));
    return (unsigned)__builtin_amdgcn_readlane((int)v, 63);
}

__device__ __forceinline__ int phys_row(const GemmArgs& p, int r) {
    if (p.row_cnt == 1) return r * p.row_gstride + p.row_goff;
    return (r / p.row_cnt) * p.row_gstride + p.row_goff + (r % p.row_cnt);
}



}

namespace gn {
struct ClArgs {
    GemmArgs g[GN_MAX_GROUP];
    long wend[GN_MAX_GROUP];
    int n;
};
constexpr int CL_KC = 256;
__device__ __forceinline__ void lds_barrier() { asm volatile("s_waitcnt lgkmcnt(0)\n\ts_barrier" ::: "memory"); }
}

int gn_gemm_launch(const gn::GemmArgs* g, int n, hipStream_t st, int split);
int gn_gemm_panel_launch(const gn::GemmArgs* g, int n, hipStream_t st);
int gn_gemm_colpipe_launch(const gn::GemmArgs* g, int n, hipStream_t st);
```

gotennet_amd/csrc/gn_gemm.hip:

```cpp
#include <type_traits>
#include "gn_gemm.h"
#include "gn_tune.h"

#ifndef GN_SPLIT_LOOP
#define GN_SPLIT_LOOP 2
#endif
#ifndef GN_SPLIT_MINW
#define GN_SPLIT_MINW 2
#endif

namespace gn {

template <int TM, int TN, int WM, int WN, bool PRO, int PF, int MODE, bool ASILU>
__device__ __forceinline__ void gemm_body(const GroupArgs ga) {
    static_assert(WM * WN == 4, "four waves per workgroup");
    constexpr bool SPLIT = MODE != 0;
    constexpr bool F16 = MODE == 2;
    constexpr int NP = F16 ? 2 : 3;
    constexpr int BM = 32 * TM * WM, BN = 32 * TN * WN;
    constexpr int RA = BM / 32, RB = BN / 32;
    constexpr int STAGE = (BM + BN) * PITCH;
    constexpr int CP = BN + 4;
    constexpr int APL = BM * SPLIT_PB;
    constexpr int STAGE_S = NP * APL;
// ... 397 lines not shown
#pragma unroll
            for (int j = 0; j < TN; ++j) {
                const float* bp = &Bs[(wn * 32 * TN + j * 32 + frow) * PITCH + khalf + hh * 8];
                const float4 b0 = ld4(bp), b1 = ld4(bp + 4);
                b[j][0] = b0.x; b[j][1] = b0.y; b[j][2] = b0.z; b[j][3] = b0.w;
                b[j][4] = b1.x; b[j][5] = b1.y; b[j][6] = b1.z; b[j][7] = b1.w;
            }
#pragma unroll
            for (int q = 0; q < 8; ++q)
#pragma unroll
                for (int i = 0; i < TM; ++i)
#pragma unroll
                    for (int j = 0; j < TN; ++j)
                        acc[i][j] = __builtin_amdgcn_mfma_f32_32x32x2f32(a[i][q], b[j][q], acc[i][j], 0, 0, 0);
        }
        if (kt + 1 < nk) stash((kt + 1) & 1, pa[s], pb[s]);
        __syncthreads();
        if (kt + 1 + PF < nk) fetch((kt + 1 + PF) * BK, pa[s], pb[s]);
      }
    }
    }

    const int next = idx + stride;
    const bool has_next = next < tile_stop;
    const bool same = has_next && next < g_end;
    if (same) {
        set_tile(next);
        fetch(0, pa[0], pb[0]);
    }

    {
#pragma unroll
    for (int i = 0; i < TM; ++i)
#pragma unroll
        for (int j = 0; j < TN; ++j)
#pragma unroll
            for (int r = 0; r < 16; ++r) {
                const int row = wm * 32 * TM + i * 32 + (r & 3) + 8 * (r >> 2) + 4 * (lane >> 5);
                float v = acc[i][j][r];
                if constexpr (F16) v = ldexpf(v, (int)(signed char)(e_acc >> (8 * (r >> 2))) + ewt);
                smem[row * CP + wn * 32 * TN + j * 32 + (lane & 31)] = v;
            }
    __syncthreads();
    {
        constexpr int C4 = BN / 4;
        const int cc = (tid % C4) * 4, gn = n0 + cc;
        if (gn < p.N) {
            const float4 bias4 = p.bias ? ld4(p.bias + gn) : zero4();
            const bool act = gn >= p.act_lo && gn < p.act_hi;
            if (p.res || p.gate) {
                constexpr int ITS = (BM * C4) / 256, UN = ITS < 4 ? ITS : 4;
                for (int it0 = 0; it0 < ITS; it0 += UN) {
                    size_t off[UN];
                    bool ok[UN];
                    float4 rv[UN], gv[UN];
#pragma unroll
                    for (int u = 0; u < UN; ++u) {
                        const int gm = m0 + (it0 + u) * (256 / C4) + tid / C4;
                        ok[u] = gm < p.M;
                        off[u] = (size_t)phys_row(p, ok[u] ? gm : 0) * p.ldc + gn;
                        rv[u] = (ok[u] && p.res) ? ld4(p.res + off[u]) : zero4();
                        gv[u] = (ok[u] && p.gate) ? ld4(p.gate + off[u]) : zero4();
                    }
#pragma unroll
                    for (int u = 0; u < UN; ++u) {
                        if (!ok[u]) continue;
                        const int row = (it0 + u) * (256 / C4) + tid / C4;
                        float4 v = ld4(&smem[row * CP + cc]) + bias4;
                        if (p.pre_out) st4(p.pre_out + off[u], v);
                        if (act) v = act4(v, ASILU ? (int)GN_ACT_SILU : p.act_kind);
                        if (p.gate) v = v * (p.gate_mode ? dact4(gv[u], ASILU ? (int)GN_ACT_SILU : p.act_kind) : gv[u]);
                        if (p.res) v = rv[u] + v;
                        st4(p.C + off[u], v);
                    }
                }
            } else {
#pragma unroll 4
                for (int it = 0; it < (BM * C4) / 256; ++it) {
                    const int row = it * (256 / C4) + tid / C4;
                    const int gm = m0 + row;
                    if (gm >= p.M) continue;
                    float4 v = ld4(&smem[row * CP + cc]) + bias4;
                    const size_t off = (size_t)phys_row(p, gm) * p.ldc + gn;
                    if (p.pre_out) st4(p.pre_out + off, v);
                    if (act) v = act4(v, ASILU ? (int)GN_ACT_SILU : p.act_kind);
                    if (gn >= p.nt_store) st4_nt(p.C + off, v); else st4(p.C + off, v);
                }
            }
        }
    }
    __syncthreads();
    }
    if (!has_next) break;
    if (!same) {
        select(next);
        set_tile(next);
        fetch(0, pa[0], pb[0]);
    }
    idx = next;
  }
}

template <int TM, int TN, int WM, int WN, bool PRO, int PF, bool ASILU>
__global__ __launch_bounds__(256) void gemm_f32_mfma(const GroupArgs ga) {
    gemm_body<TM, TN, WM, WN, PRO, PF, 0, ASILU>(ga);
}

template <int TM, int TN, int WM, int WN, bool PRO, bool ASILU>
__global__ __launch_bounds__(256, GN_SPLIT_MINW) void gemm_bf16x3_mfma(const GroupArgs ga) {
    gemm_body<TM, TN, WM, WN, PRO, 1, 1, ASILU>(ga);
}

template <int TM, int TN, int WM, int WN, bool PRO, bool ASILU>
__global__ __launch_bounds__(256, GN_SPLIT_MINW) void gemm_f16x2_mfma(const GroupArgs ga) {
    gemm_body<TM, TN, WM, WN, PRO, 1, 2, ASILU>(ga);
}

}

extern "C" int gn_gemm_ex(const float* A, int lda, const float* W, const float* bias, float* C, int ldc,
                          int Mrows, int Nout, int K, int act_lo, int act_hi,
                          int row_cnt, int row_gstride, int row_goff,
                          const float* res, const float* gate, int gate_mode, float* pre_out,
                          int pro_mode, int pro_lo, int pro_hi, const float* a_pre, int ldp,
                          const float* a_gate, int ldg, int act_kind, void* stream) {
    if (act_kind < 0 || act_kind >= GN_ACT_COUNT) return GN_ERR_BAD_ARG;
    if (Mrows < 0 || Nout <= 0 || K <= 0 || (K & 3) || (lda & 3) || (Nout & 3) || (ldc & 3) || (act_lo & 3) ||
        (act_hi & 3) || row_cnt <= 0)
        return GN_ERR_BAD_ARG;
    if (gate != nullptr && res == nullptr && gate_mode == 0) return GN_ERR_BAD_ARG;
    if (pro_mode < 0 || pro_mode > 2 || (pro_mode == 2 && (!a_pre || (ldp & 3))) || (a_gate && (ldg & 3)) ||
        (pro_mode && ((pro_lo & 3) || (pro_hi & 3))))
        return GN_ERR_BAD_ARG;
    if (Mrows == 0) return GN_OK;
    gn::GemmArgs p{A, W, bias, C, res, gate, pre_out, a_pre, a_gate, lda, ldc, ldp, ldg, Mrows, Nout, K,
                   act_lo, act_hi, pro_mode, pro_lo, pro_hi, row_cnt, row_gstride, row_goff, gate_mode,
                   nullptr, nullptr, 0, 0, act_kind};
    return gn_gemm_launch(&p, 1, (hipStream_t)stream, 0);
}

static int gemm_args_ok(int Mrows, int Nout, int K, int lda, int ldc, int act_lo, int act_hi, int row_cnt,
                        const float* res, const float* gate, int gate_mode, int pro_mode, int pro_lo, int pro_hi,
                        const float* a_pre, int ldp, const float* a_gate, int ldg) {
    if (Mrows < 0 || Nout <= 0 || K <= 0 || (K & 3) || (lda & 3) || (Nout & 3) || (ldc & 3) || (act_lo & 3) ||
        (act_hi & 3) || row_cnt <= 0)
        return 0;
    if (gate != nullptr && res == nullptr && gate_mode == 0) return 0;
    if (pro_mode < 0 || pro_mode > 2 || (pro_mode == 2 && (!a_pre || (ldp & 3))) || (a_gate && (ldg & 3)) ||
        (pro_mode && ((pro_lo & 3) || (pro_hi & 3))))
        return 0;
    return 1;
}

static int gemm_group_impl(const gn_gemm_desc* d, int n, void* stream, int split) {
    if (n < 0 || n > gn::GN_MAX_GROUP || (n > 0 && !d)) return GN_ERR_BAD_ARG;
    gn::GemmArgs g[gn::GN_MAX_GROUP];
    int m = 0;
    for (int i = 0; i < n; ++i) {
        const gn_gemm_desc& q = d[i];
        if (!gemm_args_ok(q.M, q.N, q.K, q.lda, q.ldc, q.act_lo, q.act_hi, q.row_cnt, q.res, q.gate, q.gate_mode,
                          q.pro_mode, q.pro_lo, q.pro_hi, q.a_pre, q.ldp, q.a_gate, q.ldg))
            return GN_ERR_BAD_ARG;
        if (q.a_seg < 0 || (q.a_seg && ((q.a_seg % gn::BK) || q.pro_mode || q.a_gate || q.K > 3 * q.a_seg ||
                                        !q.A2 || (q.K > 2 * q.a_seg && !q.A3) || q.lda2 < 0 || (q.lda2 & 3))))
            return GN_ERR_BAD_ARG;
        if (q.M == 0) continue;
        g[m++] = gn::GemmArgs{q.A, q.W, q.bias, q.C, q.res, q.gate, q.pre_out, q.a_pre, q.a_gate, q.lda, q.ldc, q.ldp,
                              q.ldg, q.M, q.N, q.K, q.act_lo, q.act_hi, q.pro_mode, q.pro_lo, q.pro_hi, q.row_cnt,
                              q.row_gstride, q.row_goff, q.gate_mode, q.A2, q.A3, q.a_seg};
        if (q.act_kind < 0 || q.act_kind >= GN_ACT_COUNT) return GN_ERR_BAD_ARG;
        g[m - 1].act_kind = q.act_kind;
        g[m - 1].lda2 = q.lda2 ? q.lda2 : q.lda;
    }
    if (m == 0) return GN_OK;
    return gn_gemm_launch(g, m, (hipStream_t)stream, split);
}

extern "C" int gn_gemm_group(const gn_gemm_desc* d, int n, void* stream) { return gemm_group_impl(d, n, stream, 0); }
extern "C" int gn_gemm_group_split(const gn_gemm_desc* d, int n, void* stream) { return gemm_group_impl(d, n, stream, 1); }
extern "C" int gn_gemm_group_f16x2(const gn_gemm_desc* d, int n, void* stream) { return gemm_group_impl(d, n, stream, 2); }

int gn_gemm_launch(const gn::GemmArgs* g, int n, hipStream_t st, int split) {
#ifndef GN_SPLIT_GRID
#define GN_SPLIT_GRID 14
#endif
#if GN_SPLIT_GRID == 12
    const int BMB = split ? 64 : 128, BNB = 128;
    const long cap_big = split ? 768 : 512;
#else
    const int BMB = 128, BNB = 128;
    const long cap_big = GN_GEMM_BIG_CAP;
#endif
    if (split == 2) {
        const int r = gn_gemm_panel_launch(g, n, st);
        if (r != 0) return r > 0 ? GN_OK : -r;
    }
    gn::GroupArgs ga;
    long big = 0;
    bool pro = false;
    for (int i = 0; i < n; ++i) {
        big += (long)((g[i].M + 127) / 128) * ((g[i].N + 127) / 128);
        pro = pro || g[i].pro_mode != 0 || g[i].a_gate != nullptr;
    }
    const bool use_big = big >= (long)GN_GEMM_BIG_MIN;
    bool wide = GN_F16_SMALL_WIDE && split == 2;
    for (int i = 0; i < n; ++i) wide = wide && g[i].N >= 128;
    long rows_all = 0;
    bool gated = false;
    for (int i = 0; i < n; ++i) {
        rows_all += g[i].M;
        gated = gated || (g[i].gate != nullptr && g[i].res != nullptr);
    }
    const bool mid = wide && !use_big && gated && GN_F16_MID_ROWS > 0 && rows_all >= (long)GN_F16_MID_ROWS;
    long end = 0;
    const double nt_min = (double)GN_GEMM_NT_MB * 1048576.0;
    for (int i = 0; i < gn::GN_MAX_GROUP; ++i) {
        ga.g[i] = g[i < n ? i : n - 1];
        const int nt_lo = GN_GEMM_NT_LO >= 0 ? GN_GEMM_NT_LO : ga.g[i].K;
        ga.g[i].nt_store = (double)ga.g[i].M * ga.g[i].N * 4.0 >= nt_min ? (ga.g[i].N > nt_lo ? nt_lo : 0) : 0x7fffffff;
        if (i < n) end += use_big ? (long)((g[i].M + BMB - 1) / BMB) * ((g[i].N + BNB - 1) / BNB)
                                  : (mid ? (long)((g[i].M + 63) / 64) * ((g[i].N + 127) / 128)
                                  : wide ? (long)((g[i].M + 31) / 32) * ((g[i].N + 127) / 128)
                                                                     : (long)((g[i].M + 63) / 64) * ((g[i].N + 63) / 64));
        ga.tile_end[i] = (int)end;
    }
    ga.n = n;
    if (split == 2) {
        const int r = gn_gemm_colpipe_launch(ga.g, n, st);
        if (r != 0) return r > 0 ? GN_OK : -r;
    }
    ga.spread = 0;
    for (int i = 1; i < n; ++i) {
        const long t0 = ga.tile_end[0], ti = ga.tile_end[i] - ga.tile_end[i - 1];
        ga.spread |= (g[i].K != g[0].K) || ti * 4 < t0 || t0 * 4 < ti;
    }
    if (end == 0) return GN_OK;
    long grid = 8L * ((end + 7) / 8);
    const long cap = use_big ? cap_big : (mid ? (long)GN_F16_MID_CAP : (wide ? (long)GN_F16_SMALL_CAP : 1024));
    if (grid > cap) grid = cap;
    bool silu = true;
    for (int i = 0; i < n; ++i) silu = silu && g[i].act_kind == GN_ACT_SILU;
#define GN_GEMM_GO_S(TM_, TN_, WM_, WN_, PRO_)                                                                        \
    do {                                                                                                              \
        if (silu) hipLaunchKernelGGL((gn::gemm_bf16x3_mfma<TM_, TN_, WM_, WN_, PRO_, true>), dim3((unsigned)grid), dim3(256), 0, st, ga); \
        else hipLaunchKernelGGL((gn::gemm_bf16x3_mfma<TM_, TN_, WM_, WN_, PRO_, false>), dim3((unsigned)grid), dim3(256), 0, st, ga);     \
    } while (0)
#define GN_GEMM_GO_H(TM_, TN_, WM_, WN_, PRO_)                                                                        \
    do {                                                                                                              \
        if (silu) hipLaunchKernelGGL((gn::gemm_f16x2_mfma<TM_, TN_, WM_, WN_, PRO_, true>), dim3((unsigned)grid), dim3(256), 0, st, ga); \
        else hipLaunchKernelGGL((gn::gemm_f16x2_mfma<TM_, TN_, WM_, WN_, PRO_, false>), dim3((unsigned)grid), dim3(256), 0, st, ga);     \
    } while (0)
#define GN_GEMM_GO_F(TM_, TN_, WM_, WN_, PRO_)                                                                        \
    do {                                                                                                              \
        if (silu) hipLaunchKernelGGL((gn::gemm_f32_mfma<TM_, TN_, WM_, WN_, PRO_, 1, true>), dim3((unsigned)grid), dim3(256), 0, st, ga); \
        else hipLaunchKernelGGL((gn::gemm_f32_mfma<TM_, TN_, WM_, WN_, PRO_, 1, false>), dim3((unsigned)grid), dim3(256), 0, st, ga);     \
    } while (0)
#if GN_SPLIT_GRID == 14
#define GN_SPLIT_BIG(PRO_) GN_GEMM_GO_S(4, 1, 1, 4, PRO_)
#elif GN_SPLIT_GRID == 12
#define GN_SPLIT_BIG(PRO_) GN_GEMM_GO_S(2, 1, 1, 4, PRO_)
#else
#define GN_SPLIT_BIG(PRO_) GN_GEMM_GO_S(2, 2, 2, 2, PRO_)
#endif
    if (split == 2) {
        if (use_big) { if (pro) GN_GEMM_GO_H(4, 1, 1, 4, true); else GN_GEMM_GO_H(4, 1, 1, 4, false); }
        else if (mid) { if (pro) GN_GEMM_GO_H(2, 1, 1, 4, true); else GN_GEMM_GO_H(2, 1, 1, 4, false); }
        else if (wide) { if (pro) GN_GEMM_GO_H(1, 1, 1, 4, true); else GN_GEMM_GO_H(1, 1, 1, 4, false); }
        else { if (pro) GN_GEMM_GO_H(1, 1, 2, 2, true); else GN_GEMM_GO_H(1, 1, 2, 2, false); }
    } else if (split) {
        if (use_big) { if (pro) GN_SPLIT_BIG(true); else GN_SPLIT_BIG(false); }
        else { if (pro) GN_GEMM_GO_S(1, 1, 2, 2, true); else GN_GEMM_GO_S(1, 1, 2, 2, false); }
    } else {
        if (use_big) { if (pro) GN_GEMM_GO_F(2, 2, 2, 2, true); else GN_GEMM_GO_F(2, 2, 2, 2, false); }
        else { if (pro) GN_GEMM_GO_F(1, 1, 2, 2, true); else GN_GEMM_GO_F(1, 1, 2, 2, false); }
    }
#undef GN_SPLIT_BIG
#undef GN_GEMM_GO_S
#undef GN_GEMM_GO_H
#undef GN_GEMM_GO_F
    GN_LAUNCH_CHECK();
    return GN_OK;
}

static int gemm_planes_single(const float* A, int lda, const unsigned short* W3, const float* bias, float* C, int ldc,
                              int Mrows, int Nout, int K, int act_lo, int act_hi,
                              int row_cnt, int row_gstride, int row_goff,
                              const float* res, const float* gate, int gate_mode, float* pre_out,
                              int pro_mode, int pro_lo, int pro_hi, const float* a_pre, int ldp,
                              const float* a_gate, int ldg, int act_kind, void* stream, int mode) {
    if (!gemm_args_ok(Mrows, Nout, K, lda, ldc, act_lo, act_hi, row_cnt, res, gate, gate_mode, pro_mode, pro_lo, pro_hi,
                      a_pre, ldp, a_gate, ldg) || !W3 || act_kind < 0 || act_kind >= GN_ACT_COUNT)
        return GN_ERR_BAD_ARG;
    if (Mrows == 0) return GN_OK;
    gn::GemmArgs p{A, reinterpret_cast<const float*>(W3), bias, C, res, gate, pre_out, a_pre, a_gate, lda, ldc, ldp, ldg,
                   Mrows, Nout, K, act_lo, act_hi, pro_mode, pro_lo, pro_hi, row_cnt, row_gstride, row_goff, gate_mode,
                   nullptr, nullptr, 0, 0, act_kind};
    return gn_gemm_launch(&p, 1, (hipStream_t)stream, mode);
}

extern "C" int gn_gemm_split(const float* A, int lda, const unsigned short* W3, const float* bias, float* C, int ldc,
                             int Mrows, int Nout, int K, int act_lo, int act_hi,
                             int row_cnt, int row_gstride, int row_goff,
                             const float* res, const float* gate, int gate_mode, float* pre_out,
                             int pro_mode, int pro_lo, int pro_hi, const float* a_pre, int ldp,
                             const float* a_gate, int ldg, int act_kind, void* stream) {
    return gemm_planes_single(A, lda, W3, bias, C, ldc, Mrows, Nout, K, act_lo, act_hi, row_cnt, row_gstride, row_goff, res,
                              gate, gate_mode, pre_out, pro_mode, pro_lo, pro_hi, a_pre, ldp, a_gate, ldg, act_kind, stream, 1);
}

extern "C" int gn_gemm_f16x2(const float* A, int lda, const unsigned short* W2, const float* bias, float* C, int ldc,
                             int Mrows, int Nout, int K, int act_lo, int act_hi,
                             int row_cnt, int row_gstride, int row_goff,
                             const float* res, const float* gate, int gate_mode, float* pre_out,
                             int pro_mode, int pro_lo, int pro_hi, const float* a_pre, int ldp,
                             const float* a_gate, int ldg, int act_kind, void* stream) {
    return gemm_planes_single(A, lda, W2, bias, C, ldc, Mrows, Nout, K, act_lo, act_hi, row_cnt, row_gstride, row_goff, res,
                              gate, gate_mode, pre_out, pro_mode, pro_lo, pro_hi, a_pre, ldp, a_gate, ldg, act_kind, stream, 2);
}

extern "C" int gn_gemm(const float* A, int lda, const float* W, const float* bias, float* C, int ldc,
                       int Mrows, int Nout, int K, int act_lo, int act_hi,
                       int row_cnt, int row_gstride, int row_goff,
                       const float* res, const float* gate, void* stream) {
    return gn_gemm_ex(A, lda, W, bias, C, ldc, Mrows, Nout, K, act_lo, act_hi, row_cnt, row_gstride, row_goff,
                      res, gate, 0, nullptr, 0, 0, 0, nullptr, 0, nullptr, 0, GN_ACT_SILU, stream);
}
```

gotennet_amd/csrc/gn_gemm_colpipe.hip:

```cpp
#include <type_traits>
#include "gn_gemm.h"
#include "gn_tune.h"

#ifndef GN_CP_NB
#define GN_CP_NB 2
#endif
#ifndef GN_CP_GRID
#define GN_CP_GRID 512
#endif
#ifndef GN_CP_MIN_N
#define GN_CP_MIN_N 1024
#endif
#ifndef GN_CP_MIN_TILES
#define GN_CP_MIN_TILES 2048
#endif

namespace gn {

__global__ __launch_bounds__(256, 2) void gemm_f16x2_colpipe(const ClArgs ca) {
    constexpr int TM = 2, BM = 64, BN = 128, KC = CL_KC;
    constexpr int NS = KC / 16;
    constexpr int NB = GN_CP_NB;
    constexpr int RPW = BM / 4;
    constexpr int APL = BM * KC;
    static_assert(NS % NB == 0, "ring slots are compile-time");
    __shared__ __attribute__((aligned(16))) _Float16 panel[2 * APL];
    __shared__ __attribute__((aligned(16))) float scratch[4 * 1024];

    const int tid = threadIdx.x, lane = tid & 63;
    const int wave = __builtin_amdgcn_readfirstlane(tid >> 6);
    float* const scr = scratch + wave * 1024;
    const int lm = lane & 31, lh = lane >> 5;
    const int x0 = lh ^ (lm & 15);
    const _Float16* const Arow = panel + lm * KC;
    const int c4 = lane & 7, rq = lane >> 3;

    long T = ca.wend[0];
#pragma unroll
    for (int gi = 1; gi < GN_MAX_GROUP; ++gi)
        if (gi < ca.n) T = ca.wend[gi];
    const long w_lo = T * (long)blockIdx.x / (long)gridDim.x, w_hi = T * ((long)blockIdx.x + 1) / (long)gridDim.x;

    for (int gi = 0; gi < ca.n; ++gi) {
#if defined(__HIP_DEVICE_COMPILE__)
        typedef const __attribute__((address_space(4))) ClArgs* KargPtr;
        const GemmArgs& p = ((KargPtr)__builtin_amdgcn_kernarg_segment_ptr())->g[gi];
        const long base = gi ? ((KargPtr)__builtin_amdgcn_kernarg_segment_ptr())->wend[gi - 1] : 0;
#else
        const GemmArgs& p = ca.g[gi];
        const long base = gi ? ca.wend[gi - 1] : 0;
#endif
        const int M = p.M, N = p.N;
        const int npass = (N + BN - 1) / BN;
        const long nun = (long)((M + BM - 1) / BM) * npass;
        long k0l = w_lo - base, k1l = w_hi - base;
        k0l = k0l < 0 ? 0 : (k0l < nun ? k0l : nun);
        k1l = k1l < 0 ? 0 : (k1l < nun ? k1l : nun);
        int k = (int)k0l;
        const int k1 = (int)k1l;
        if (k >= k1) continue;
        const uint4* const wfrag = reinterpret_cast<const uint4*>(p.W) + 16 + lane;
        const int ewt = __builtin_amdgcn_readfirstlane(*reinterpret_cast<const int*>(p.W));
        const int nt_last = (N + 31) / 32 - 1;
        auto boff = [&](int ps) -> unsigned {
            int nt = ps * 4 + wave;
            nt = nt < nt_last ? nt : nt_last;
            return (unsigned)nt * (NS * 128u);
        };
        uint4 bq[NB][2];
        auto load_b = [&](unsigned bo, int g, uint4 (&q)[2]) __attribute__((always_inline)) {
            q[0] = wfrag[bo + (unsigned)g * 128u];
            q[1] = wfrag[bo + (unsigned)g * 128u + 64u];
        };
        const int kind = GN_ACT_SILU;
        const float* const res = p.res; const float* const gate = p.gate; float* const pre_out = p.pre_out; float* const C = p.C;
        const float* const bias = p.bias;
        const int ldc = p.ldc, gate_mode = p.gate_mode, nt_store = p.nt_store, act_lo = p.act_lo, act_hi = p.act_hi;

        while (k < k1) {
            const int m0 = (k / npass) * BM;
            const int ps0 = k % npass;
            const int ps1 = ps0 + (k1 - k) < npass ? ps0 + (k1 - k) : npass;
            k += ps1 - ps0;
            const int prow_v = phys_row(p, m0 + lane < M ? m0 + lane : 0);
            {
                float4 va[RPW];
                const float* Ak = p.A + 4 * lane;
                const int lda = p.lda;
#pragma unroll
                for (int u = 0; u < RPW; ++u)
                    va[u] = ld4(Ak + (size_t)__builtin_amdgcn_readlane(prow_v, 4 * u + wave) * lda);
                const unsigned bo0 = boff(ps0);
#pragma unroll
                for (int g = 0; g < NB; ++g) load_b(bo0, g, bq[g]);
#pragma unroll
                for (int u = 0; u < RPW; ++u) {
                    const int r = 4 * u + wave;
                    const bool inside = m0 + r < M;
                    const float4 v = make_float4(inside ? va[u].x : 0.f, inside ? va[u].y : 0.f, inside ? va[u].z : 0.f, inside ? va[u].w : 0.f);
                    const float m = fmaxf(fmaxf(fabsf(v.x), fabsf(v.y)), fmaxf(fabsf(v.z), fabsf(v.w)));
                    int need = (int)((wave_umax_sgpr(__float_as_uint(m)) >> 23) & 0xffu) - 126 - 15;
                    need = need < -120 ? -120 : need;
                    const float scale = __uint_as_float((unsigned)(127 - need) << 23);
                    f16x4 h, l;
                    split4_f16(v, scale, h, l);
                    _Float16* d = panel + r * KC + (((lane >> 1) ^ (r & 15)) << 3) + ((lane & 1) << 2);
                    *reinterpret_cast<f16x4*>(d) = h;
                    *reinterpret_cast<f16x4*>(d + APL) = l;
                    if (lane < 4) reinterpret_cast<int*>(scratch + lane * 1024)[r] = need;
                }
            }
            lds_barrier();
            int e_r[TM][4], prow_e[TM][4];
#pragma unroll
            for (int i = 0; i < TM; ++i)
#pragma unroll
                for (int q = 0; q < 4; ++q) {
                    e_r[i][q] = reinterpret_cast<const int*>(scr)[i * 32 + 8 * q + rq] + ewt;
                    prow_e[i][q] = __shfl(prow_v, i * 32 + 8 * q + rq, 64);
                }
            asm volatile("s_waitcnt lgkmcnt(0)" ::: "memory");

            f32x16 acc[2][TM];
            float4 t[4], rv[4], gv[4], bias4 = zero4();
            auto read_a = [&](int g, f16x8 (&a)[TM][2]) __attribute__((always_inline)) {
                const int ch8 = ((2 * g) ^ x0) * 8;
#pragma unroll
                for (int i = 0; i < TM; ++i) {
                    a[i][0] = *reinterpret_cast<const f16x8*>(Arow + i * 32 * KC + ch8);
                    a[i][1] = *reinterpret_cast<const f16x8*>(Arow + APL + i * 32 * KC + ch8);
                }
            };
            auto epi_slice = [&](auto PP, int g, int ps) __attribute__((always_inline)) {
                constexpr int P = decltype(PP)::value;
                const int i = g >> 3, sub = g & 7;
                const int gn = ps * BN + wave * 32 + 4 * c4;
                const bool col_ok = gn < N;
                if (sub == 0) {
                    if (i == 0) bias4 = (bias && col_ok) ? ld4(bias + gn) : zero4();
                    __builtin_amdgcn_wave_barrier();
#pragma unroll
                    for (int gg = 0; gg < 4; ++gg)
                        st4(scr + lm * 32 + (((2 * gg + lh) ^ (lm & 7)) << 2),
                            make_float4(acc[P][i][4 * gg + 0], acc[P][i][4 * gg + 1], acc[P][i][4 * gg + 2], acc[P][i][4 * gg + 3]));
                    __builtin_amdgcn_wave_barrier();
                } else if (sub == 2) {
#pragma unroll
                    for (int q = 0; q < 4; ++q) {
                        const int rr = 8 * q + rq;
                        t[q] = ld4(scr + rr * 32 + ((c4 ^ (rr & 7)) << 2));
                    }
                    if (res || gate) {
#pragma unroll
                        for (int q = 0; q < 4; ++q) {
                            const bool ok = m0 + i * 32 + 8 * q + rq < M && col_ok;
                            const size_t off = (size_t)prow_e[i][q] * ldc + gn;
                            rv[q] = (ok && res) ? ld4(res + off) : zero4();
                            gv[q] = (ok && gate) ? ld4(gate + off) : zero4();
                        }
                    }
                    __builtin_amdgcn_wave_barrier();
                } else if (sub == 4 || sub == 6) {
                    const bool act = gn >= act_lo && gn < act_hi;
#pragma unroll
                    for (int qq = 0; qq < 2; ++qq) {
                        const int q = (sub == 4 ? 0 : 2) + qq;
                        const bool ok = m0 + i * 32 + 8 * q + rq < M && col_ok;
                        if (!ok) continue;
                        const size_t off = (size_t)prow_e[i][q] * ldc + gn;
                        const int e = e_r[i][q];
                        float4 v = make_float4(ldexpf(t[q].x, e), ldexpf(t[q].y, e), ldexpf(t[q].z, e), ldexpf(t[q].w, e)) + bias4;
                        if (pre_out) st4(pre_out + off, v);
                        if (act) v = act4(v, kind);
                        if (gate) v = v * (gate_mode ? dact4(gv[q], kind) : gv[q]);
                        if (res) v = rv[q] + v;
                        if (gn >= nt_store) st4_nt(C + off, v); else st4(C + off, v);
                    }
                }
            };
            auto pass = [&](auto PP, auto EE, int ps, bool has_next) __attribute__((always_inline)) {
                constexpr int P = decltype(PP)::value;
                constexpr bool EPI = decltype(EE)::value;
                const unsigned bo = boff(ps), bo_next = boff(has_next ? ps + 1 : ps);
                f16x8 ab[2][TM][2];
                read_a(0, ab[0]);
#pragma unroll
                for (int g = 0; g < NS; ++g) {
                    if (g + 1 < NS) read_a(g + 1, ab[(g + 1) & 1]);
                    __builtin_amdgcn_sched_barrier(0);
                    constexpr int TA[3] = {1, 0, 0};
                    constexpr int TB[3] = {0, 1, 0};
#pragma unroll
                    for (int tt = 0; tt < 3; ++tt)
#pragma unroll
                        for (int i = 0; i < TM; ++i) {
                            if (g == 0 && tt == 0) {
                                f32x16 z;
#pragma unroll
                                for (int r = 0; r < 16; ++r) z[r] = 0.f;
                                acc[P][i] = __builtin_amdgcn_mfma_f32_32x32x16_f16(
                                    __builtin_bit_cast(f16x8, bq[g % NB][TB[tt]]), ab[g & 1][i][TA[tt]], z, 0, 0, 0);
                            } else {
                                acc[P][i] = __builtin_amdgcn_mfma_f32_32x32x16_f16(
                                    __builtin_bit_cast(f16x8, bq[g % NB][TB[tt]]), ab[g & 1][i][TA[tt]], acc[P][i], 0, 0, 0);
                            }
                        }
                    __builtin_amdgcn_sched_barrier(0);
                    if (g + NB < NS) load_b(bo, g + NB, bq[g % NB]);
                    else if (has_next) load_b(bo_next, g + NB - NS, bq[g % NB]);
                    if constexpr (EPI) {
                        epi_slice(std::integral_constant<int, P ^ 1>{}, g, ps - 1);
                    }
                }
            };
            using P0 = std::integral_constant<int, 0>; using P1 = std::integral_constant<int, 1>;
            using No = std::false_type; using Yes = std::true_type;
            int ps = ps0;
            pass(P0{}, No{}, ps, ps + 1 < ps1);
            ++ps;
            while (ps + 1 < ps1) {
                pass(P1{}, Yes{}, ps, true);
                pass(P0{}, Yes{}, ps + 1, ps + 2 < ps1);
                ps += 2;
            }
            if (ps < ps1) {
                pass(P1{}, Yes{}, ps, false);
#pragma unroll
                for (int g = 0; g < NS; g += 2) epi_slice(P1{}, g, ps);
            } else {
#pragma unroll
                for (int g = 0; g < NS; g += 2) epi_slice(P0{}, g, ps - 1);
            }
            lds_barrier();
        }
    }
}

}

int gn_gemm_colpipe_launch(const gn::GemmArgs* g, int n, hipStream_t st) {
    if (GN_CP_MIN_TILES < 0) return 0;
    gn::ClArgs ca;
    int n_max = 0;
    long end = 0;
    for (int i = 0; i < n; ++i) {
        if (g[i].pro_mode != 0 || g[i].a_gate != nullptr || g[i].K != gn::CL_KC || g[i].a_seg != 0 || g[i].act_kind != GN_ACT_SILU) return 0;
        n_max = g[i].N > n_max ? g[i].N : n_max;
    }
    for (int i = 0; i < gn::GN_MAX_GROUP; ++i) {
        ca.g[i] = g[i < n ? i : n - 1];
        if (i < n) end += (long)((g[i].M + 63) / 64) * ((g[i].N + 127) / 128);
        ca.wend[i] = end;
    }
    ca.n = n;
    if (n_max < GN_CP_MIN_N || end < (long)GN_CP_MIN_TILES) return 0;
    const unsigned grid = (unsigned)(end < (long)GN_CP_GRID ? end : (long)GN_CP_GRID);
    hipLaunchKernelGGL(gn::gemm_f16x2_colpipe, dim3(grid), dim3(256), 0, st, ca);
    hipError_t e = hipGetLastError();
    if (e != hipSuccess) return -(int)e;
    return 1;
}
```

gotennet_amd/engine.py:

```python
from __future__ import annotations

import dataclasses
import os
from dataclasses import dataclass, field
from typing import Any, List, Optional

import torch

from . import _lib
from ._lib import call, ptr


@dataclass
class LayerWeights:
    Wn1: Optional[torch.Tensor] = None; bn1: Optional[torch.Tensor] = None
    Ws2: Optional[torch.Tensor] = None; bs2: Optional[torch.Tensor] = None
    Wv2: Optional[torch.Tensor] = None; bv2: Optional[torch.Tensor] = None
    We: Optional[torch.Tensor] = None; be: Optional[torch.Tensor] = None
    Wvu: Optional[torch.Tensor] = None
    Wm0: Optional[torch.Tensor] = None; bm0: Optional[torch.Tensor] = None
    Wm1: Optional[torch.Tensor] = None; bm1: Optional[torch.Tensor] = None
    Wt: Optional[torch.Tensor] = None; bt: Optional[torch.Tensor] = None
    Wvq: Optional[torch.Tensor] = None
    Wvk: List[torch.Tensor] = field(default_factory=list)
    ln_w: Optional[torch.Tensor] = None; ln_b: Optional[torch.Tensor] = None
    tln_w: Optional[torch.Tensor] = None
    Wt0: Optional[torch.Tensor] = None; bt0: Optional[torch.Tensor] = None
    t_ln_w: Optional[torch.Tensor] = None; t_ln_b: Optional[torch.Tensor] = None
    Wedp: Optional[torch.Tensor] = None; bedp: Optional[torch.Tensor] = None
    w_ln_w: Optional[torch.Tensor] = None; w_ln_b: Optional[torch.Tensor] = None
    T: dict = field(default_factory=dict)


@dataclass
class PackedWeights:
    A_na: torch.Tensor; A_nbr: torch.Tensor
    Winit: torch.Tensor; binit: torch.Tensor
    Wa: torch.Tensor; ba: torch.Tensor; ln_w: torch.Tensor; ln_b: torch.Tensor
    Wb: torch.Tensor; bb: torch.Tensor
    rb0: torch.Tensor; rb1: torch.Tensor
    layers: List[LayerWeights] = field(default_factory=list)
    T: dict = field(default_factory=dict)
    emb_idx: Optional[torch.Tensor] = None
    F_model: int = 0


ZERO_X_FIRST = os.environ.get("GN_ZERO_X_FIRST", "1") != "0"
MSG_BWD_PAIR = False
DT_KCAT = True


def zero_X_in(cfg: "Config", li: int) -> bool:
    return (ZERO_X_FIRST and li == 0 and cfg.lmax <= 4 and cfg.act == 0 and not cfg.steerable_norm and not cfg.sliced
            and cfg.aggr == 0 and not cfg.wide)


def derived(holder, key, build):
    t = holder.T.get(key)
    if t is None:
        t = holder.T[key] = build()
    return t


def _T(holder, name: str, lo: int = 0, hi: Optional[int] = None) -> torch.Tensor:
    key = name if hi is None else (name, lo, hi)
    t = holder.T.get(key)
    return t if t is not None else derived(holder, key, lambda: getattr(holder, name)[lo:hi].t().contiguous())


def _rows(lw, name: str, n: int) -> torch.Tensor:
    return derived(lw, ("rows", name, n), lambda: getattr(lw, name)[:n])


@dataclass
class Config:
    F: int; L: int; R: int; H: int; lmax: int; M: int
    cutoff: float; eps: float
    scale_edge: bool; sep_dir: bool; sep_tensor: bool
    basis: int = 0
    htr_mode: int = 0
    layernorm: bool = False
    steerable_norm: bool = False
    composed_update: bool = False
    gate_kind: int = 0
    t_last_act: int = 3
    lin_w: int = 0
    lin_ln: int = 0
    act: int = 0
    evec: int = 0
    emlp: int = 0
    gemm_mode: str = ""
    sliced: bool = False
    aggr: int = 0
    Fc: int = 0
    F_model: int = 0
    fuse_eqff: Optional[bool] = None
    attn_p: float = 0.0

    @property
    def Fe(self) -> int:
        return self.evec or self.F

    @property
    def Fm(self) -> int:
        return self.emlp or self.F

    @property
    def D(self) -> int:
        return (self.lmax + 1) ** 2 - 1

    def degree_blocks(self, N: int, explicit: bool = False):
        D = self.D
        if self.htr_mode & 1:
            return [(0, N * D, (D, D, 0) if explicit else (1, 1, 0))]
        blocks, off = [], 0
        for l in range(1, self.lmax + 1):
            blocks.append((l - 1, N * (2 * l + 1), (2 * l + 1, D, off)))
            off += 2 * l + 1
        return blocks

    @property
    def lmax_arg(self) -> int:
        return self.lmax | (_lib.LMAX_SLICED if self.sliced else 0)

    @property
    def wide(self) -> bool:
        return self.F > 256 or self.Fe > 256

    @property
    def lmax_arg_bwd(self) -> int:
        return self.lmax_arg | (_lib.LMAX_SLICED if self.wide else 0)

    @property
    def lmax_arg_msg_bwd(self) -> int:
        return self.lmax_arg_msg | (_lib.LMAX_SLICED if self.wide else 0)

    @property
    def lmax_arg_msg(self) -> int:
        return self.lmax_arg | {0: 0, 1: _lib.LMAX_MEAN, 2: _lib.LMAX_MAX}[self.aggr]


_raw_stream = getattr(torch._C, "_cuda_getCurrentRawStream", None)


def _stream() -> int:
    if _raw_stream is not None:
        return _raw_stream(torch.cuda.current_device())
    return torch.cuda.current_stream().cuda_stream


GEMM_MODE = os.environ.get("GN_GEMM_MODE", "f16x2")
MODES = ("f16x2", "split", "f32")


_PLANE_MODES = {"split": ("gn_gemm_split", "gn_gemm_group_split", "gn_split_bf16x3", "gn_split_bf16x3_size", torch.bfloat16),
                "f16x2": ("gn_gemm_f16x2", "gn_gemm_group_f16x2", "gn_split_f16x2", "gn_split_f16x2_size", torch.float16)}


def resolve_mode(mode: Optional[str]) -> str:
    mode = mode or GEMM_MODE
    if mode not in MODES:
        raise ValueError(f"projection arithmetic {mode!r}: one of {MODES}")
    return mode


def split_weight(W: torch.Tensor, mode: Optional[str] = None) -> torch.Tensor:
    mode = resolve_mode(mode)
    key = "_gn_split_" + mode
    cached = getattr(W, key, None)
    if cached is not None and cached[0] == W._version and cached[1] == W.data_ptr():
        return cached[2]
    _, _, packer, sizer, dt = _PLANE_MODES[mode]
    N, K = W.shape
    planes = torch.empty(getattr(_lib.load(), sizer)(N, K), dtype=dt, device=W.device)
    call(packer, ptr(W.contiguous()), N, K, ptr(planes), _stream())
    setattr(W, key, (W._version, W.data_ptr(), planes))
    return planes


def gemm(A, lda, W, bias, C, ldc, rows, nout, K, act=(0, 0), rowmap=(1, 1, 0), res=None, gate=None,
         a_off=0, c_off=0, pre_out=None, pro=(0, 0, 0), a_pre=None, ldp=0, p_off=0, a_gate=None, ldg=0,
         dgate=None, g_off=0, kind=None, mode=None):
    mode = resolve_mode(mode)
    name = "gn_gemm_ex"
    if mode in _PLANE_MODES:
        name, W = _PLANE_MODES[mode][0], split_weight(W, mode)
    call(name, A.data_ptr() + 4 * a_off, lda, ptr(W), ptr(bias), C.data_ptr() + 4 * c_off, ldc,
         rows, nout, K, act[0], act[1], rowmap[0], rowmap[1], rowmap[2], ptr(res),
         (dgate.data_ptr() + 4 * g_off) if dgate is not None else ptr(gate), 1 if dgate is not None else 0, ptr(pre_out),
         pro[0], pro[1], pro[2], (a_pre.data_ptr() + 4 * p_off) if a_pre is not None else None, ldp,
         ptr(a_gate), ldg, 0 if kind is None else kind, _stream())


def gemm_group(problems, mode=None, kind=None):
    mode = resolve_mode(mode)
    kind = 0 if kind is None else kind
    problems = [q for q in problems if q is not None]
    split = mode in _PLANE_MODES
    for i0 in range(0, len(problems), 4):
        chunk = problems[i0:i0 + 4]
        arr = (_lib.GemmDesc * len(chunk))()
        for d, q in zip(arr, chunk):
            g = q.get
            act, rowmap, pro = g("act", (0, 0)), g("rowmap", (1, 1, 0)), g("pro", (0, 0, 0))
            dgate = g("dgate")
            d.A = q["A"].data_ptr() + 4 * g("a_off", 0); d.lda = q["lda"]
            d.W = ptr(split_weight(q["W"], mode) if split else q["W"]); d.bias = ptr(g("bias"))
            d.C = q["C"].data_ptr() + 4 * g("c_off", 0); d.ldc = q["ldc"]
            d.M, d.N, d.K = q["rows"], q["nout"], q["K"]
            d.act_lo, d.act_hi = act
            d.row_cnt, d.row_gstride, d.row_goff = rowmap
            d.res = ptr(g("res"))
            d.gate = (dgate.data_ptr() + 4 * g("g_off", 0)) if dgate is not None else ptr(g("gate"))
            d.gate_mode = 1 if dgate is not None else 0
            d.pre_out = ptr(g("pre_out"))
            d.pro_mode, d.pro_lo, d.pro_hi = pro
            a_pre = g("a_pre")
            d.a_pre = (a_pre.data_ptr() + 4 * g("p_off", 0)) if a_pre is not None else None
            d.ldp = g("ldp", 0)
            d.a_gate = ptr(g("a_gate")); d.ldg = g("ldg", 0)
            d.A2, d.A3, d.a_seg = ptr(g("A2")), ptr(g("A3")), g("a_seg", 0)
            d.act_kind = g("kind", kind)
            d.lda2 = g("lda2", 0)
        call(_PLANE_MODES[mode][1] if split else "gn_gemm_group", arr, len(chunk), _stream())


class _Call:
    __slots__ = ("mode", "act", "cfg", "g", "st", "N", "E", "F", "D", "Fe", "lde", "blocks", "cols", "key")

    def __init__(self, cfg: "Config", g: Optional["Graph"] = None, explicit_blocks: bool = False,
                 key: Optional[torch.Tensor] = None):
        self.key = key
        self.mode, self.act, self.cfg, self.g, self.st = resolve_mode(cfg.gemm_mode), cfg.act, cfg, g, _stream()
        self.F, self.D, self.Fe, self.lde = cfg.F, cfg.D, cfg.Fe, (1 + cfg.M) * cfg.F
        n = cfg.lmax if cfg.sep_dir else 1
        self.cols = ((self.lde, cfg.M * cfg.F), ((2 + n) * cfg.F, (1 + n) * cfg.F))
        self.N, self.E = (g.N, g.E) if g is not None else (None, None)
        self.blocks = cfg.degree_blocks(g.N, explicit_blocks) if g is not None else None

    def gemm(self, *args, **kw):
        kw.setdefault("kind", self.act)
        kw.setdefault("mode", self.mode)
        return gemm(*args, **kw)

    def group(self, problems):
        return gemm_group(problems, mode=self.mode, kind=self.act)


def validate_edges(edge_index: torch.Tensor, n_atoms: int) -> int:
    flag = torch.zeros(1, dtype=torch.int32, device=edge_index.device)
    call("gn_check_edges", ptr(edge_index), edge_index.shape[1], n_atoms, ptr(flag), _stream())
    return int(flag.item())


def sorted_edges(edge_index, edge_diff, edge_vec, n_atoms: int):
    if edge_index.shape[1] == 0:
        return edge_index, edge_diff, edge_vec, None
    bits = validate_edges(edge_index, n_atoms)
    if bits & 2:
        raise ValueError(f"edge_index holds indices outside [0, {n_atoms})")
    if not bits & 1:
        return edge_index, edge_diff, edge_vec, None
    order = torch.sort(edge_index[1], stable=True).indices
    return edge_index[:, order].contiguous(), edge_diff[order], edge_vec[order], order


class Graph:

    def __init__(self, cfg: Config, pw: PackedWeights, n_atoms: int, edge_index: torch.Tensor,
                 edge_diff: Optional[torch.Tensor] = None, edge_vec: Optional[torch.Tensor] = None):
        dev = edge_index.device
        E = edge_index.shape[1]
        self.N, self.E = n_atoms, E
        self.cfg, self.pw = cfg, pw
        i32 = dict(dtype=torch.int32, device=dev)
        f32 = dict(dtype=torch.float32, device=dev)
        self.src = torch.empty(E, **i32)
        self.dst = torch.empty(E, **i32)
        self.rowptr = torch.empty(n_atoms + 1, **i32)
        call("gn_build_csr", ptr(edge_index), E, n_atoms, ptr(self.src), ptr(self.dst), ptr(self.rowptr), _stream())
        self.outdeg = None
        if cfg.scale_edge:
            self.outdeg = torch.zeros(n_atoms, **i32)
            call("gn_out_degree", ptr(self.src), E, ptr(self.outdeg), _stream())
        self.rl = torch.empty((E, cfg.D), **f32)
        self.phi = torch.empty((E, max(cfg.R, 0)), **f32)
        self.cut = torch.empty(E, **f32)
        self.perm = self.colptr = self.tgt_by_src = None
        self.edge_diff = self.edge_vec = None
        if edge_vec is not None:
            self.set_geometry(edge_diff, edge_vec)

    def set_geometry(self, edge_diff: torch.Tensor, edge_vec: torch.Tensor):
        cfg, pw = self.cfg, self.pw
        self.edge_diff, self.edge_vec = edge_diff, edge_vec
        call("gn_edge_geometry", ptr(edge_vec), ptr(edge_diff), ptr(self.src), ptr(self.dst), self.E,
             cfg.lmax, cfg.R, cfg.basis, ptr(pw.rb0), ptr(pw.rb1), float(cfg.cutoff),
             ptr(self.rl), ptr(self.phi), ptr(self.cut), _stream())

    def set_positions(self, pos: torch.Tensor):
        if self.edge_vec is None:
            self.edge_vec = torch.empty((self.E, 3), dtype=torch.float32, device=pos.device)
            self.edge_diff = torch.empty(self.E, dtype=torch.float32, device=pos.device)
        call("gn_edge_vectors", ptr(pos), ptr(self.src), ptr(self.dst), self.E, ptr(self.edge_vec), ptr(self.edge_diff),
             _stream())
        self.set_geometry(self.edge_diff, self.edge_vec)

    def csc(self):
        if self.perm is None:
            i32 = dict(dtype=torch.int32, device=self.src.device)
            self.colptr, self.perm = torch.empty(self.N + 1, **i32), torch.empty(self.E, **i32)
            self.tgt_by_src = torch.empty(self.E, **i32)
            work = torch.empty(self.N + self.E, **i32)
            call("gn_build_csc", ptr(self.src), ptr(self.dst), self.E, self.N, ptr(self.colptr), ptr(self.perm),
                 ptr(self.tgt_by_src), ptr(work), _stream())
        return self.colptr, self.perm


@dataclass
class LayerTape:
    first: bool = False
    h_in: torch.Tensor = None; X_in: torch.Tensor = None; t_in: torch.Tensor = None
    nproj: torch.Tensor = None; xs: torch.Tensor = None; vs: torch.Tensor = None
    eproj: torch.Tensor = None; attn: torch.Tensor = None
    attn_soft: torch.Tensor = None
    EQ: torch.Tensor = None; EK: torch.Tensor = None; w: torch.Tensor = None; pre_t: torch.Tensor = None
    w_raw: torch.Tensor = None; h_raw: torch.Tensor = None; X_raw: torch.Tensor = None
    upd: dict = None
    Xp: torch.Tensor = None; ctx: torch.Tensor = None; pre_g1: torch.Tensor = None; mm: torch.Tensor = None
    X_msg: torch.Tensor = None; nact: torch.Tensor = None; g1act: torch.Tensor = None


@dataclass
class Tape:
    feat: torch.Tensor = None; y_pre: torch.Tensor = None; h0: torch.Tensor = None
    ctx0: torch.Tensor = None; y: torch.Tensor = None
    layers: List[LayerTape] = field(default_factory=list)
    key: torch.Tensor = None


def draw_dropout_key(device, generator: Optional[torch.Generator] = None) -> torch.Tensor:
    return torch.randint(0, 2 ** 63 - 1, (2,), dtype=torch.int64, device=device, generator=generator)


def attention_dropout_mask(key: torch.Tensor, layer: int, E: int, H: int, p: float) -> torch.Tensor:
    if not key.is_cuda or key.dtype != torch.int64 or key.numel() < 2 or not key.is_contiguous():
        raise ValueError("key: a contiguous int64 device tensor of two values (GotenNet.last_dropout_key)")
    m = torch.empty((E, H), dtype=torch.float32, device=key.device)
    with torch.cuda.device(key.device):
        call("gn_attn_dropout_mask", ptr(key), int(layer), float(p), E, H, ptr(m), _stream())
    return m


def check_backward_supported(cfg: Config) -> None:
    if cfg.wide and (cfg.F // 4) // cfg.H > 64:
        raise NotImplementedError(f"n_atom_basis={cfg.F_model or cfg.F} with {cfg.H} heads: the input-gradient kernels keep one "
                                  "attention head inside one wave (at most 256 channels per head)")


def check_param_grads_supported(cfg: Config) -> None:
    if cfg.composed_update:
        raise NotImplementedError("parameter_grads: composed edge updates (edge_updates with 'mlp' / 'mlpa' / 'linw' / "
                                  "'linwa'; evec_dim != n_atom_basis needs one) have no parameter-gradient path")
    if cfg.F_model or cfg.F & (cfg.F - 1):
        raise NotImplementedError(f"parameter_grads: n_atom_basis={cfg.F_model or cfg.F} is not a power of two (the model "
                                  "runs embedded in a wider one); parameter gradients need a power-of-two width")
    check_backward_supported(cfg)


def param_grad_config(cfg: Config) -> Config:
    return dataclasses.replace(cfg, fuse_eqff=False)


def _norm_h(lw: LayerWeights, h: torch.Tensor, emb_idx: Optional[torch.Tensor] = None) -> torch.Tensor:
    x = h if emb_idx is None else h.index_select(1, emb_idx)
    y = torch.empty_like(x)
    call("gn_layernorm", ptr(x), ptr(lw.ln_w), ptr(lw.ln_b), 1e-5, x.shape[0], x.shape[1], ptr(y), _stream())
    return y if emb_idx is None else torch.zeros_like(h).index_copy_(1, emb_idx, y)


def _norm_X(lw: LayerWeights, X: torch.Tensor, lmax: int, emb_idx: Optional[torch.Tensor] = None) -> torch.Tensor:
    x = X if emb_idx is None else X.index_select(2, emb_idx)
    y = torch.empty_like(x)
    call("gn_tensor_norm", ptr(x), ptr(lw.tln_w), 1e-12, x.shape[0], x.shape[2], lmax, ptr(y), _stream())
    return y if emb_idx is None else torch.zeros_like(X).index_copy_(2, emb_idx, y)


def _norm_h_backward(lw: LayerWeights, h_raw, g_y, g_x, emb_idx: Optional[torch.Tensor] = None):
    x, gy, gx = h_raw, g_y, g_x
    if emb_idx is not None:
        x, gy = h_raw.index_select(1, emb_idx), g_y.index_select(1, emb_idx)
        gx = torch.empty_like(gy)
    call("gn_layernorm_backward", ptr(x), ptr(lw.ln_w), 1e-5, ptr(gy), x.shape[0], x.shape[1], ptr(gx), _stream())
    if emb_idx is not None:
        g_x.zero_().index_copy_(1, emb_idx, gx)


def _norm_X_backward(lw: LayerWeights, X_raw, g_y, g_x, lmax: int, emb_idx: Optional[torch.Tensor] = None):
    x, gy, gx = X_raw, g_y, g_x
    if emb_idx is not None:
        x, gy = X_raw.index_select(2, emb_idx), g_y.index_select(2, emb_idx)
        gx = torch.empty_like(gy)
    call("gn_tensor_norm_backward", ptr(x), ptr(lw.tln_w), ptr(gy), 1e-12, x.shape[0], x.shape[2], lmax, ptr(gx), _stream())
    if emb_idx is not None:
        g_x.zero_().index_copy_(2, emb_idx, gx)


def gata_input_norms(cfg: Config, lw: LayerWeights, h: torch.Tensor, X: torch.Tensor):
    N = h.shape[0]
    return (_norm_h(lw, h) if cfg.layernorm and N else h), (_norm_X(lw, X, cfg.lmax) if cfg.steerable_norm and N else X)


def _htr_problems(p: _Call, lw: LayerWeights, X, EQ, EK):
    F_, Fe, N = p.F, p.Fe, p.N
    return [dict(A=X, lda=F_, W=lw.Wvq, C=EQ, ldc=Fe, rows=N * p.D, nout=Fe, K=F_)] + [
        dict(A=X, lda=F_, W=lw.Wvk[k], C=EK, ldc=Fe, rows=rows, nout=Fe, K=F_, rowmap=rowmap)
        for k, rows, rowmap in p.blocks]


def _init_forward(p: _Call, pw: PackedWeights, z32, new, tape: Optional[Tape], pgrads: bool):
    cfg, g, st, F_, R, N, E, gemm = p.cfg, p.g, p.st, p.F, p.cfg.R, p.N, p.E, p.gemm
    feat = new(E, 2 * F_)
    gemm(g.phi, R, pw.Winit, pw.binit, feat, 2 * F_, E, 2 * F_, R)
    ctx0 = new(N, 2 * F_)
    call("gn_node_init", ptr(z32), ptr(g.rowptr), ptr(g.src), ptr(feat), 2 * F_, ptr(g.cut),
         ptr(pw.A_na), ptr(pw.A_nbr), N, F_, ptr(ctx0), st)
    Fc = cfg.Fc or F_
    y_pre = new(N, Fc)
    gemm(ctx0, 2 * F_, pw.Wa, pw.ba, y_pre, Fc, N, Fc, 2 * F_)
    y = new(N, Fc)
    call("gn_layernorm_silu", ptr(y_pre), ptr(pw.ln_w), ptr(pw.ln_b), 1e-5, N, Fc, ptr(y), cfg.act, st)
    h = new(N, F_)
    gemm(y, Fc, pw.Wb, pw.bb, h, F_, N, F_, Fc)
    t = new(E, F_)
    call("gn_edge_init", ptr(h), ptr(g.rowptr), ptr(g.src), feat.data_ptr() + 4 * F_, 2 * F_, N, F_, ptr(t), st)
    if tape is not None:
        tape.feat, tape.y_pre, tape.h0 = feat, y_pre, h
        if pgrads:
            tape.ctx0, tape.y = ctx0, y
    return h, t


def _layer_buffers(cfg: Config, N: int, E: int, new, last: bool, save: bool, pgrads: bool = False):
    F_, D, M, Fe = cfg.F, cfg.D, cfg.M, cfg.Fe
    lt = LayerTape(xs=new(N, M * F_), vs=new(N, M * F_), eproj=new(E, (1 + M) * F_), attn=new(E, cfg.H),
                   Xp=new(N, D, F_), ctx=new(N, 2 * F_), mm=new(N, 2 * F_))
    if cfg.attn_p > 0:
        lt.attn_soft = new(E, cfg.H)
    if save:
        lt.nproj, lt.pre_g1 = new(N, 4 * F_), new(N, F_)
    if not last:
        lt.EQ, lt.EK, lt.w = new(N, D, Fe), new(N, D, Fe), new(E, Fe)
        if save:
            lt.pre_t = new(E, F_)
            lt.w_raw = new(E, Fe) if (cfg.htr_mode >> 2) else None
    if pgrads:
        lt.nact, lt.g1act = new(N, 4 * F_), new(N, F_)
    return lt, new(N, F_), new(N, D, F_), (None if last else new(E, F_))


def _gata_forward(p: _Call, lw: LayerWeights, lt: LayerTape, nact, h, X, t, h2, X2, li: int = 0):
    cfg, g, st, F_, lde, N, E, first = p.cfg, p.g, p.st, p.F, p.lde, p.N, p.E, lt.first
    H, M, xs, vs, eproj, attn = cfg.H, cfg.M, lt.xs, lt.vs, lt.eproj, lt.attn
    ne, nv = p.cols[first]
    p.group([dict(A=t, lda=F_, W=_rows(lw, "We", ne) if first else lw.We, bias=lw.be, C=eproj, ldc=lde, rows=E, nout=ne, K=F_),
             dict(A=h, lda=F_, W=lw.Wn1, bias=lw.bn1, C=nact, ldc=4 * F_, rows=N, nout=4 * F_, K=F_,
                  act=(2 * F_, 4 * F_), pre_out=lt.nproj)])
    p.group([dict(A=nact, lda=4 * F_, W=_rows(lw, "Ws2", nv) if first else lw.Ws2, bias=lw.bs2, C=xs, ldc=M * F_, rows=N,
                  nout=nv, K=F_, a_off=2 * F_),
             dict(A=nact, lda=4 * F_, W=_rows(lw, "Wv2", nv) if first else lw.Wv2, bias=lw.bv2, C=vs, ldc=M * F_, rows=N,
                  nout=nv, K=F_, a_off=3 * F_)])
    if cfg.attn_p > 0:
        call("gn_attn_softmax_dropout", ptr(nact), nact.data_ptr() + 4 * F_, 4 * F_, ptr(eproj), lde,
             ptr(g.rowptr), ptr(g.src), ptr(g.outdeg), N, F_, H, ptr(lt.attn_soft), ptr(attn), ptr(p.key), li,
             float(cfg.attn_p), cfg.act, st)
    else:
        call("gn_attn_softmax", ptr(nact), nact.data_ptr() + 4 * F_, 4 * F_, ptr(eproj), lde,
             ptr(g.rowptr), ptr(g.src), ptr(g.outdeg), N, F_, H, ptr(attn), cfg.act, st)
    call("gn_message_aggregate", ptr(xs), ptr(vs), M * F_, eproj.data_ptr() + 4 * F_, lde,
         ptr(attn), ptr(g.rl), ptr(g.cut), ptr(g.rowptr), ptr(g.src), ptr(h), None if first else ptr(X), ptr(h2), ptr(X2),
         N, F_, H, cfg.lmax_arg_msg, int(cfg.sep_dir), int(cfg.sep_tensor), st)


def _eqff_htr_forward(p: _Call, lw: LayerWeights, lt: LayerTape, g1act, h, X, t, t2, save: bool, eq_fused: bool):
    cfg, g, st, F_, D, Fe, N, E = p.cfg, p.g, p.st, p.F, p.D, p.Fe, p.N, p.E
    last, Xp, ctx, mm = lw.Wt is None, lt.Xp, lt.ctx, lt.mm
    xprods = [dict(A=X, lda=F_, W=lw.Wvu, C=Xp, ldc=F_, rows=N * D, nout=F_, K=F_)]
    if not last:
        xprods += _htr_problems(p, lw, X, lt.EQ, lt.EK)
    p.group(xprods)
    m0 = None
    if eq_fused:
        call("gn_eqff_fused_forward", ptr(Xp), ptr(split_weight(lw.Wm0, p.mode)), ptr(lw.bm0),
             ptr(split_weight(lw.Wm1, p.mode)), ptr(lw.bm1), float(cfg.eps), N, F_, D, ptr(h), ptr(X),
             ptr(ctx) if save else None, ptr(lt.pre_g1), ptr(mm) if save else None, 1 if p.mode == "split" else 2, st)
    else:
        call("gn_eqff_context", ptr(h), ptr(Xp), float(cfg.eps), N, F_, D, ptr(ctx), st)
        m0 = dict(A=ctx, lda=2 * F_, W=lw.Wm0, bias=lw.bm0, C=g1act, ldc=F_, rows=N, nout=F_, K=2 * F_, act=(0, F_),
                  pre_out=lt.pre_g1)
    if last:
        p.group([m0])
    else:
        call("gn_htr_edge", ptr(lt.EQ), ptr(lt.EK), ptr(g.rl), ptr(g.rowptr), ptr(g.src), N, Fe, cfg.lmax_arg, cfg.htr_mode,
             ptr(lt.w_raw), ptr(lt.w), st)
        if cfg.composed_update:
            upd = _edge_update_composed(cfg, lw, t, lt.w, t2, E, lt.pre_t)
            if save:
                lt.upd = upd
            p.group([m0])
        else:
            p.group([dict(A=t, lda=F_, W=lw.Wt, bias=lw.bt, C=t2, ldc=F_, rows=E, nout=F_, K=F_, act=(0, F_), res=t,
                          gate=lt.w, pre_out=lt.pre_t), m0])
    if not eq_fused:
        p.gemm(g1act, F_, lw.Wm1, lw.bm1, mm, 2 * F_, N, 2 * F_, F_)
        call("gn_eqff_update", ptr(mm), ptr(Xp), N, F_, D, ptr(h), ptr(X), st)


def forward(cfg: Config, pw: PackedWeights, z32: torch.Tensor, g: Graph, save: bool = False,
            trace: Optional[list] = None, pgrads: bool = False, key: Optional[torch.Tensor] = None):
    F_, D, N, E = cfg.F, cfg.D, g.N, g.E
    if save:
        check_backward_supported(cfg)
    if pgrads:
        check_param_grads_supported(cfg)
        if not save or cfg.fuse_eqff is not False:
            raise ValueError("internal: a parameter-gradient forward saves its tape and runs the un-fused EQFF chain")
    if cfg.attn_p > 0 and key is None:
        raise ValueError("internal: a forward with attention dropout needs the call's key (draw_dropout_key)")
    p = _Call(cfg, g, key=key)
    f32 = dict(dtype=torch.float32, device=z32.device)
    new = lambda *shape: torch.empty(shape, **f32)
    tape = Tape(key=key) if save else None
    h, t = _init_forward(p, pw, z32, new, tape, pgrads)
    X = new(N, D, F_) if (zero_X_in(cfg, 0) and pw.layers) else torch.zeros((N, D, F_), **f32)
    nact, g1act = new(N, 4 * F_), new(N, F_)
    eq_fused = eqff_fused_ok(cfg, N)
    if not save:
        lt, h2, X2, t2 = _layer_buffers(cfg, N, E, new, last=False, save=False)

    for li, lw in enumerate(pw.layers):
        first = zero_X_in(cfg, li)
        h_raw, X_raw = h, X
        if cfg.layernorm:
            h = _norm_h(lw, h, pw.emb_idx)
        if cfg.steerable_norm:
            X = _norm_X(lw, X, cfg.lmax, pw.emb_idx)
        if save:
            lt, h2, X2, t2 = _layer_buffers(cfg, N, E, new, lw.Wt is None, True, pgrads)
            lt.h_in, lt.t_in, lt.h_raw = h, t, h_raw
            if not first:
                lt.X_in, lt.X_raw = X, X_raw
            tape.layers.append(lt)
            if pgrads:
                nact, g1act = lt.nact, lt.g1act
        lt.first = first
        _gata_forward(p, lw, lt, nact, h, X, t, h2, X2, li)
        h, h2 = h2, h
        X, X2 = X2, X
        if pgrads:
            lt.X_msg = X.clone()
        _eqff_htr_forward(p, lw, lt, g1act, h, X, t, t2, save, eq_fused)
        if lw.Wt is not None:
            t, t2 = t2, t
        if trace is not None:
            trace.append((h.clone(), X.clone(), t.clone()) if pw.emb_idx is None else
                         tuple(v.index_select(v.dim() - 1, pw.emb_idx) for v in (h, X, t)))
    if pw.emb_idx is not None:
        h, X = h.index_select(1, pw.emb_idx), X.index_select(2, pw.emb_idx)
    return h, X, tape


def gata_layer(cfg: Config, lw: LayerWeights, g: "Graph", h: torch.Tensor, X: torch.Tensor, t: torch.Tensor,
               key: Optional[torch.Tensor] = None):
    F_, D, M, Fe, N, E = cfg.F, cfg.D, cfg.M, cfg.Fe, g.N, g.E
    if cfg.attn_p > 0 and key is None:
        raise ValueError("internal: a layer with attention dropout needs the call's key (draw_dropout_key)")
    p = _Call(cfg, g, key=key)
    new = lambda *shape: torch.empty(shape, dtype=torch.float32, device=h.device)
    if cfg.layernorm:
        h = _norm_h(lw, h)
    if cfg.steerable_norm:
        X = _norm_X(lw, X, cfg.lmax)
    lt = LayerTape(xs=new(N, M * F_), vs=new(N, M * F_), eproj=new(E, p.lde), attn=new(E, cfg.H),
                   attn_soft=new(E, cfg.H) if cfg.attn_p > 0 else None)
    h2, X2 = new(N, F_), new(N, D, F_)
    _gata_forward(p, lw, lt, new(N, 4 * F_), h, X, t, h2, X2)
    if lw.Wt is None:
        return h2, X2, t
    EQ, EK, w, t2 = new(N, D, Fe), new(N, D, Fe), new(E, Fe), new(E, F_)
    p.group(_htr_problems(p, lw, X2, EQ, EK))
    call("gn_htr_edge", ptr(EQ), ptr(EK), ptr(g.rl), ptr(g.rowptr), ptr(g.src), N, Fe, cfg.lmax_arg, cfg.htr_mode, None, ptr(w),
         p.st)
    if cfg.composed_update:
        _edge_update_composed(cfg, lw, t, w, t2, E, None)
    else:
        p.gemm(t, F_, lw.Wt, lw.bt, t2, F_, E, F_, F_, act=(0, F_), res=t, gate=w)
    return h2, X2, t2


def eqff_layer(cfg: Config, lw: LayerWeights, h: torch.Tensor, X: torch.Tensor):
    F_, D, N = cfg.F, cfg.D, h.shape[0]
    p = _Call(cfg)
    new = lambda *shape: torch.empty(shape, dtype=torch.float32, device=h.device)
    Xp, ctx, g1, mm = new(N, D, F_), new(N, 2 * F_), new(N, F_), new(N, 2 * F_)
    p.gemm(X, F_, lw.Wvu, None, Xp, F_, N * D, F_, F_)
    call("gn_eqff_context", ptr(h), ptr(Xp), float(cfg.eps), N, F_, D, ptr(ctx), p.st)
    p.gemm(ctx, 2 * F_, lw.Wm0, lw.bm0, g1, F_, N, F_, 2 * F_, act=(0, F_))
    p.gemm(g1, F_, lw.Wm1, lw.bm1, mm, 2 * F_, N, 2 * F_, F_)
    h, X = h.clone(), X.clone()
    call("gn_eqff_update", ptr(mm), ptr(Xp), N, F_, D, ptr(h), ptr(X), p.st)
    return h, X

EQFF_FUSED_MAX_ATOMS = 1024


def eqff_fused_ok(cfg: Config, n_atoms: Optional[int] = None) -> bool:
    mode = resolve_mode(cfg.gemm_mode)
    want = cfg.fuse_eqff if cfg.fuse_eqff is not None else (n_atoms is not None and n_atoms <= EQFF_FUSED_MAX_ATOMS)
    if not want or mode not in _PLANE_MODES:
        return False
    return bool(_lib.load().gn_eqff_fused_supported(cfg.F, cfg.act, 1 if mode == "split" else 2))


def _edge_update_composed(cfg: Config, lw: LayerWeights, t, w_raw, t2, E: int, pre_t):
    F_, Fe, Fm = cfg.F, cfg.Fe, cfg.Fm
    gemm = _Call(cfg).gemm
    new = lambda width=F_: torch.empty((E, width), dtype=torch.float32, device=t.device)
    st = _stream()
    u = dict(w_raw=w_raw)
    x = w_raw
    if cfg.lin_w:
        a_in = x
        if cfg.lin_ln == 1:
            a_in = new(Fe)
            call("gn_layernorm", ptr(x), ptr(lw.w_ln_w), ptr(lw.w_ln_b), 1e-5, E, Fe, ptr(a_in), st)
        lin = new()
        gemm(a_in, Fe, lw.Wedp, lw.bedp, lin, F_, E, F_, Fe, pro=(1, 0, Fe) if cfg.lin_w == 2 else (0, 0, 0))
        x = lin
        if cfg.lin_ln == 2:
            x = new()
            call("gn_layernorm", ptr(lin), ptr(lw.w_ln_w), ptr(lw.w_ln_b), 1e-5, E, F_, ptr(x), st)
        u.update(a_in=a_in, lin=lin)
    u["pre_gate"] = x
    if cfg.gate_kind:
        wg = new()
        call("gn_gate", ptr(x), cfg.gate_kind, E * F_, ptr(wg), st)
    else:
        wg = x
    u["wg"] = wg
    act = (0, F_) if cfg.t_last_act == 3 else (0, 0)
    if lw.Wt0 is not None:
        hid = new(Fm)
        gemm(t, F_, lw.Wt0, lw.bt0, hid, Fm, E, Fm, F_)
        u_in = hid
        if lw.t_ln_w is not None:
            u_in = new(Fm)
            call("gn_layernorm", ptr(hid), ptr(lw.t_ln_w), ptr(lw.t_ln_b), 1e-5, E, Fm, ptr(u_in), st)
        gemm(u_in, Fm, lw.Wt, lw.bt, t2, F_, E, F_, Fm, act=act, res=t, gate=wg, pre_out=pre_t, pro=(1, 0, Fm))
        u.update(hid=hid, u_in=u_in)
    else:
        gemm(t, F_, lw.Wt, lw.bt, t2, F_, E, F_, F_, act=act, res=t, gate=wg, pre_out=pre_t)
    return u


def _edge_update_composed_backward(cfg: Config, lw: LayerWeights, lt, gt, gt_a, E: int):
    F_, Fe, Fm = cfg.F, cfg.Fe, cfg.Fm
    gemm = _Call(cfg).gemm
    new = lambda width=F_: torch.empty((E, width), dtype=torch.float32, device=gt.device)
    st = _stream()
    u = lt.upd
    g_pre, g_wg = new(), new()
    call("gn_edge_gate_backward", ptr(gt), ptr(lt.pre_t), cfg.act if cfg.t_last_act else -1, ptr(u["wg"]), E * F_, ptr(g_pre), ptr(g_wg), st)
    if lw.Wt0 is not None:
        g_u = new(Fm)
        gemm(g_pre, F_, _T(lw, "Wt"), None, g_u, Fm, E, Fm, F_, dgate=u["u_in"])
        if lw.t_ln_w is not None:
            g_h = new(Fm)
            call("gn_layernorm_backward", ptr(u["hid"]), ptr(lw.t_ln_w), 1e-5, ptr(g_u), E, Fm, ptr(g_h), st)
            g_u = g_h
        gemm(g_u, Fm, _T(lw, "Wt0"), None, gt_a, F_, E, F_, Fm, res=gt)
    else:
        gemm(g_pre, F_, _T(lw, "Wt"), None, gt_a, F_, E, F_, F_, res=gt)
    gq = g_wg
    if cfg.gate_kind:
        g2 = new()
        call("gn_gate_backward", ptr(gq), ptr(u["pre_gate"]), cfg.gate_kind, E * F_, ptr(g2), st)
        gq = g2
    if cfg.lin_w:
        if cfg.lin_ln == 2:
            g2 = new()
            call("gn_layernorm_backward", ptr(u["lin"]), ptr(lw.w_ln_w), 1e-5, ptr(gq), E, F_, ptr(g2), st)
            gq = g2
        g3 = new(Fe)
        gemm(gq, F_, _T(lw, "Wedp"), None, g3, Fe, E, Fe, F_, dgate=u["a_in"] if cfg.lin_w == 2 else None)
        gq = g3
        if cfg.lin_ln == 1:
            g4 = new(Fe)
            call("gn_layernorm_backward", ptr(u["w_raw"]), ptr(lw.w_ln_w), 1e-5, ptr(gq), E, Fe, ptr(g4), st)
            gq = g4
    return gq


def weight_grad_group(problems):
    problems = [q for q in problems if q is not None]
    if not problems:
        return
    arr = (_lib.WgradDesc * len(problems))()
    for d, q in zip(arr, problems):
        g = q.get
# ... 301 lines not shown
```

include/gotennet_hip.h:

```cpp
#ifndef GOTENNET_HIP_H
#define GOTENNET_HIP_H

#include <stdint.h>

#ifdef __cplusplus
extern "C" {
#endif

#define GN_OK 0
#define GN_ERR_BAD_ARG 10001
#define GN_ABI_VERSION 11
#define GN_LMAX_SLICED 0x100
#define GN_LMAX_MEAN 0x200
#define GN_LMAX_MAX 0x400

enum {
    GN_ACT_SILU = 0, GN_ACT_SSP = 1, GN_ACT_RELU = 2, GN_ACT_TANH = 3, GN_ACT_SIGMOID = 4, GN_ACT_ELU = 5,
    GN_ACT_SELU = 6, GN_ACT_MISH = 7, GN_ACT_GELU = 8, GN_ACT_SOFTPLUS = 9, GN_ACT_LEAKY = 10,
    GN_ACT_NONE = 11 , GN_ACT_COUNT = 12
};

int gn_abi_version(const char** arch_out);


int gn_build_csr(const int64_t* edge_index, int E, int N, int* src, int* dst, int* rowptr, void* stream);

int gn_check_edges(const int64_t* edge_index, int E, int N, int* flag, void* stream);

int gn_build_csc(const int* src, const int* dst, int E, int N, int* colptr, int* perm, int* tgt_by_src, int* work,
                 void* stream);

int gn_molecule_ptr(const int64_t* batch, int N, int n_mol, int* mol_ptr, void* stream);

int gn_out_degree(const int* src, int E, int* outdeg, void* stream);

int gn_cosine_cutoff(const float* dist, int E, float cutoff, float* cut, void* stream);

int gn_edge_geometry(const float* edge_vec, const float* edge_diff, const int* src, const int* dst, int E,
                     int lmax, int R, int basis, const float* means, const float* betas, float cutoff,
                     float* rl, float* phi, float* cut, void* stream);


int gn_node_init(const int* z, const int* rowptr, const int* src, const float* feat, int ldf,
                 const float* cut, const float* A_na, const float* A_nbr,
                 int N, int F, float* ctx, void* stream);

int gn_edge_init(const float* h, const int* rowptr, const int* src, const float* feat, int ldf,
                 int N, int F, float* t, void* stream);

int gn_layernorm_silu(const float* x, const float* gamma, const float* beta, float eps,
                      int N, int F, float* y, int act , void* stream);

int gn_layernorm(const float* x, const float* gamma, const float* beta, float eps,
                 int N, int F, float* y, void* stream);
int gn_tensor_norm(const float* X, const float* weight, float eps, int N, int F, int lmax, float* Y, void* stream);

int gn_gemm(const float* A, int lda, const float* W, const float* bias, float* C, int ldc,
            int Mrows, int Nout, int K, int act_lo, int act_hi,
            int row_cnt, int row_gstride, int row_goff,
            const float* res, const float* gate, void* stream);

int gn_gemm_ex(const float* A, int lda, const float* W, const float* bias, float* C, int ldc,
               int Mrows, int Nout, int K, int act_lo, int act_hi,
               int row_cnt, int row_gstride, int row_goff,
               const float* res, const float* gate, int gate_mode, float* pre_out,
               int pro_mode, int pro_lo, int pro_hi, const float* a_pre, int ldp,
               const float* a_gate, int ldg, int act_kind , void* stream);

typedef struct gn_gemm_desc {
    const float* A; int lda;
    const float* W; const float* bias;
    float* C; int ldc;
    int M, N, K;
    int act_lo, act_hi;
    int row_cnt, row_gstride, row_goff;
    const float* res; const float* gate; int gate_mode;
    float* pre_out;
    int pro_mode, pro_lo, pro_hi;
    const float* a_pre; int ldp;
    const float* a_gate; int ldg;
    const float* A2; const float* A3; int a_seg;
    int act_kind;
    int lda2;
} gn_gemm_desc;
int gn_gemm_group(const gn_gemm_desc* problems, int n, void* stream);

long gn_split_bf16x3_size(int N, int K);
int gn_split_bf16x3(const float* w , int N, int K, unsigned short* out, void* stream);
int gn_gemm_split(const float* A, int lda, const unsigned short* W3, const float* bias, float* C, int ldc,
                  int Mrows, int Nout, int K, int act_lo, int act_hi,
                  int row_cnt, int row_gstride, int row_goff,
                  const float* res, const float* gate, int gate_mode, float* pre_out,
                  int pro_mode, int pro_lo, int pro_hi, const float* a_pre, int ldp,
                  const float* a_gate, int ldg, int act_kind, void* stream);
int gn_gemm_group_split(const gn_gemm_desc* problems, int n, void* stream);

long gn_split_f16x2_size(int N, int K);
int gn_split_f16x2(const float* w , int N, int K, unsigned short* out, void* stream);
int gn_gemm_f16x2(const float* A, int lda, const unsigned short* W2, const float* bias, float* C, int ldc,
                  int Mrows, int Nout, int K, int act_lo, int act_hi,
                  int row_cnt, int row_gstride, int row_goff,
                  const float* res, const float* gate, int gate_mode, float* pre_out,
                  int pro_mode, int pro_lo, int pro_hi, const float* a_pre, int ldp,
                  const float* a_gate, int ldg, int act_kind, void* stream);
int gn_gemm_group_f16x2(const gn_gemm_desc* problems, int n, void* stream);

int gn_attn_softmax(const float* q, const float* k, int ldqk, const float* t_attn, int ldt,
                    const int* rowptr, const int* src, const int* outdeg,
                    int N, int F, int H, float* a, int act , void* stream);

int gn_attn_softmax_dropout(const float* q, const float* k, int ldqk, const float* t_attn, int ldt,
                            const int* rowptr, const int* src, const int* outdeg,
                            int N, int F, int H, float* a_soft, float* a, const long long* key, int layer, double p,
                            int act, void* stream);
int gn_attn_dropout_mask(const long long* key, int layer, double p, long E, int H, float* m_out, void* stream);

int gn_message_aggregate(const float* x, const float* v, int ldxv, const float* t_filter, int ldt,
                         const float* a, const float* rl, const float* cut,
                         const int* rowptr, const int* src,
                         const float* h_in, const float* X_in, float* h_out, float* X_out,
                         int N, int F, int H, int lmax, int sep_dir, int sep_tensor, void* stream);

int gn_eqff_fused_supported(int F, int act, int arith);
int gn_eqff_fused_forward(const float* Xp, const void* W0p, const float* b0, const void* W1p, const float* b1,
                          float eps, int N, int F, int D, float* h, float* X,
                          float* ctx_out, float* pre_out, float* mm_out, int arith, void* stream);
int gn_eqff_fused_backward(const float* gh, const float* gX, const float* mm, const float* Xp, const float* ctx,
                           const float* pre_g1, const void* W1Tp, const void* W0Tp, int N, int F, int D,
                           float* gXp, float* gh1, int arith, void* stream);

#define GN_HTR_JOINT 1
#define GN_HTR_NOREJ 2
#define GN_HTR_GATE_SIGMOID (1 << 2)
#define GN_HTR_GATE_TANH (2 << 2)
#define GN_HTR_GATE_SILU (3 << 2)
#define GN_HTR_DIRECT 16
int gn_htr_edge(const float* EQ, const float* EK, const float* rl, const int* rowptr, const int* src,
                int N, int F, int lmax, int mode, float* w_raw, float* w, void* stream);

int gn_eqff_context(const float* h, const float* Xp, float eps, int N, int F, int D, float* ctx, void* stream);
int gn_eqff_update(const float* m, const float* Xp, int N, int F, int D, float* h, float* X, void* stream);


int gn_htr_backward(const float* g_t_out, const float* pre_t, const float* w, const float* w_raw,
                    const float* EQ, const float* EK,
                    const float* rl, const int* rowptr, const int* src, const int* tgt_by_src,
                    const int* colptr, const int* perm, int N, int F, int lmax, int mode,
                    float* gEQ, float* gEK, float* g_rl, float* g_pre_t, int act , void* stream);

int gn_message_backward(const float* x, const float* v, int ldxv, const float* eproj, int lde, const float* a,
                        const float* qk, int ldqk, const float* X_in, const float* rl, const float* cut,
                        const int* outdeg, const float* g_h1, const float* g_X1,
                        const int* rowptr, const int* src, const int* tgt_by_src, const int* colptr, const int* perm,
                        float* g_eproj, float* g_s, float* g_nproj, int ldn, float* g_x, float* g_v,
                        float* g_X_out, float* g_rl, float* g_cut, float* ga_parts, long E,
                        int N, int F, int H, int lmax, int sep_dir, int sep_tensor, int act, void* stream);
int gn_message_backward_dropout(const float* x, const float* v, int ldxv, const float* eproj, int lde, const float* a,
                                const float* a_soft,
                                const float* qk, int ldqk, const float* X_in, const float* rl, const float* cut,
                                const int* outdeg, const float* g_h1, const float* g_X1,
                                const int* rowptr, const int* src, const int* tgt_by_src, const int* colptr, const int* perm,
                                float* g_eproj, float* g_s, float* g_nproj, int ldn, float* g_x, float* g_v,
                                float* g_X_out, float* g_rl, float* g_cut, float* ga_parts, long E,
                                int N, int F, int H, int lmax, int sep_dir, int sep_tensor, int act, void* stream);
int gn_message_backward_groups(int lmax, int sep_dir, int sep_tensor, int act);

int gn_eqff_backward_a(const float* g_h, const float* g_X, const float* m, const float* Xp,
                       int N, int F, int D, float* g_m, float* g_Xp, void* stream);
int gn_eqff_backward_b(const float* g_ctx, const float* ctx, const float* Xp, const float* g_h,
                       int N, int F, int D, float* g_Xp, float* g_h1, void* stream);

int gn_edge_init_backward(const float* g_t0, const float* h, const float* feat, int ldf,
                          const int* rowptr, const int* src, const int* colptr, const int* perm,
                          int N, int F, float* g_feat, float* g_h, void* stream);
int gn_node_init_backward(const float* g_ctx, const int* z, const float* feat, int ldf, const float* cut,
                          const float* A_nbr, const int* rowptr, const int* src, int N, int F,
                          float* g_feat, float* g_cut, void* stream);
int gn_layernorm_silu_backward(const float* x, const float* gamma, const float* beta, float eps,
                               const float* g_out, int N, int F, float* g_x, int act, void* stream);
int gn_layernorm_backward(const float* x, const float* gamma, float eps,
                          const float* g_out, int N, int F, float* g_x, void* stream);
int gn_tensor_norm_backward(const float* X, const float* weight, const float* g_Y, float eps, int N, int F,
                            int lmax, float* g_X, void* stream);

int gn_gate(const float* x, int kind, long n, float* y, void* stream);
int gn_gate_backward(const float* g, const float* x, int kind, long n, float* g_x, void* stream);
int gn_edge_gate_backward(const float* g, const float* pre, int act, const float* wg, long n,
                          float* g_pre, float* g_wg, void* stream);

int gn_edge_geometry_backward(const float* edge_vec, const float* edge_diff, const int* src, const int* dst,
                              int E, int lmax, int R, int basis, const float* means, const float* betas, float cutoff,
                              const float* g_rl, int n_rl, const float* g_cut, int n_cut, const float* g_phi,
                              float* g_vec, float* g_diff, void* stream);
int gn_pos_scatter(const float* g_vec, const float* g_diff, const float* edge_vec,
                   const int* rowptr, const int* colptr, const int* perm, int N, float sign,
                   float* out, void* stream);

int gn_head_energy(const float* pre1, const float* W2, float b2, float scale, float shift, float mol_shift,
                   const float* atomref, const int* z, const int* mol_ptr, int n_mol, int Hd,
                   float* y, float* energy, int mean ,
                   float* atom_scale ,
                   int act , void* stream);
int gn_head_grad(const float* pre1, const float* W2, float scale, const float* atom_scale , int N, int Hd,
                 float* g_pre1, int act, void* stream);

int gn_geb_context(const float* s, int lds, int n_sin, const float* vmix, int ldv, int n_vout, int N,
                   float* ctx, int ldc, void* stream);
int gn_geb_gate(const float* x, int ldx, int n_sout, int n_vout, const float* vmix, int ldv, int w_off, int N,
                int sact, float* s_out, int lds, float* v_out, int ldo, void* stream);
int gn_dipole_reduce(const float* mu, int ldm, const float* q, int ldq, const float* pos, const int* mol_ptr,
                     int n_mol, float scale, float shift, int standardise, int magnitude, float* y, float* y_vec,
                     void* stream);
int gn_ese_reduce(const float* x, const float* pos, const int* z, const float* mass, int n_mass, const int* mol_ptr,
                  int n_mol, float* y, void* stream);

int gn_radius_count(const float* pos, const int64_t* batch, int N, float cutoff, int max_nbr,
                    int* deg, void* stream);
int gn_radius_fill(const float* pos, const int64_t* batch, int N, float cutoff, int max_nbr,
                   const int64_t* rowptr, int64_t E, int64_t* edge_index, float* edge_vec,
                   float* edge_diff, void* stream);
int gn_edge_vectors(const float* pos, const int* src, const int* dst, int E, float* edge_vec, float* edge_diff,
                    void* stream);

typedef struct gn_wgrad_desc {
    const float* dY; int ldy; int y_off;
    const float* A; int lda; int a_off;
    float* dW; int ldw;
    float* db;
    int rows, nout, K;
    int row_cnt, row_gstride, row_goff;
} gn_wgrad_desc;
long gn_weight_grad_workspace(const gn_wgrad_desc* problems, int n);
int gn_weight_grad_group(const gn_wgrad_desc* problems, int n, float* work, long work_floats, void* stream);
int gn_embedding_grad(const float* g_ctx, const float* feat, int ldf, const float* cut, const int* dst,
                      const int* colptr, const int* perm, const int* order, const int* sp_ptr, int n_species,
                      int N, int F, float* work, float* dA_na, float* dA_nbr, void* stream);
long gn_layernorm_param_grad_workspace(int N, int C);
int gn_layernorm_param_grad(const float* x, const float* gamma, const float* beta, float eps, const float* g_out,
                            int N, int C, int act, float* work, float* dgamma, float* dbeta, void* stream);


#ifdef __cplusplus
}
#endif
#endif
```

Measured before the change: 22390 molecules/s.

## Fuse edge-update into HTR edge kernel and segment edge projection GEMM

The per-edge t update (t2 = t + silu(pre_t) * w) is moved into the HTR edge kernel, so w no longer has to be written and reread by a separate edge-update step. The pre_t projection (Wt) is computed earlier as an extra column segment of the eproj GEMM, since both read the same input t. When lmax <= 2, w is not stored even when saving for backward, and the backward target kernel recomputes it. This cuts edge-sized memory traffic and kernel launches, at the cost of extra recompute in backward and more complex GEMM and kernel variants.

```diff
diff --git a/gotennet_amd/_lib.py b/gotennet_amd/_lib.py
--- a/gotennet_amd/_lib.py
+++ b/gotennet_amd/_lib.py
@@ -21,6 +21,10 @@
                 ("res", _P), ("gate", _P), ("gate_mode", _I), ("pre_out", _P),
                 ("pro_mode", _I), ("pro_lo", _I), ("pro_hi", _I), ("a_pre", _P), ("ldp", _I),
                 ("a_gate", _P), ("ldg", _I), ("A2", _P), ("A3", _P), ("a_seg", _I), ("act_kind", _I), ("lda2", _I)]
+
+
+class GemmSeg(C.Structure):
+    _fields_ = [("c_seg", _I), ("W2", _P), ("bias2", _P), ("C2", _P), ("ldc2", _I)]
 
 
 class WgradDesc(C.Structure):
@@ -65,6 +69,8 @@
     "gn_split_f16x2": [_P, _I, _I, _P, _P],
     "gn_split_f16x2_size": [_I, _I],
     "gn_gemm_group_f16x2": [_P, _I, _P],
+    "gn_gemm_group_seg": [_P, _P, _I, _I, _P],
+    "gn_htr_edge_update": [_P, _P, _P, _P, _P, _I, _I, _I, _P, _P, _I, _P, _P, _P],
     "gn_htr_backward": [_P, _P, _P, _P, _P, _P, _P, _P, _P, _P, _P, _P, _I, _I, _I, _I, _P, _P, _P, _P, _I, _P],
     "gn_message_backward": [_P, _P, _I, _P, _I, _P, _P, _I, _P, _P, _P, _P, _P, _P, _P, _P, _P, _P, _P,
                             _P, _P, _P, _I, _P, _P, _P, _P, _P, _P, C.c_long, _I, _I, _I, _I, _I, _I, _I, _P],
diff --git a/gotennet_amd/csrc/gn_backward.hip b/gotennet_amd/csrc/gn_backward.hip
--- a/gotennet_amd/csrc/gn_backward.hip
+++ b/gotennet_amd/csrc/gn_backward.hip
@@ -2,12 +2,13 @@
 #include "gn_tune.h"
 #include "gn_sh.h"
 #include "gn_highl.h"
+#include "gn_htr.h"
 
 namespace gn {
 
 
 
-template <int LMAX, int FC = 0>
+template <int LMAX, int FC = 0, bool RW = false>
 __global__ __launch_bounds__(256) GN_WPE(GN_W_HTR_TGT) void htr_bwd_target_kernel(
     const float* __restrict__ gtp, const float* __restrict__ pre_t, const float* __restrict__ w,
     const float* __restrict__ EQ, const float* __restrict__ EK, const float* __restrict__ rl,
@@ -31,7 +32,8 @@
         float4 a_pt, d_pt;
         act_pair4(pte, act, a_pt, d_pt);
         const float4 gw = gte * a_pt;
-        st4(g_pre_t + (size_t)e * F + c0, gte * ld4_nt(w + (size_t)e * F + c0) * d_pt);
+        float4 wsum = zero4();
+        if constexpr (!RW) st4(g_pre_t + (size_t)e * F + c0, gte * ld4_nt(w + (size_t)e * F + c0) * d_pt);
         const float* kj = EK + (size_t)src[e] * D * F + c0;
         const float* re = rl + (size_t)e * D;
         float part[KP];
@@ -59,8 +61,10 @@
                 acc[m0 + mm] = fma4(r[mm], u, fma4(gw, ek[mm], acc[m0 + mm]));
                 part[m0 + mm] = hsum4(fma4(r[mm], s2, fma4(v, ek[mm], u * eq[m0 + mm])));
             }
+            if constexpr (RW) wsum = htr_w_literal_l(l, eq + m0, ek, r, wsum);
             m0 += 2 * l + 1;
         }
+        if constexpr (RW) st4(g_pre_t + (size_t)e * F + c0, gte * wsum * d_pt);
         if (lps >= KP) {
             multi_group_sum<KP>(part, lps, lp);
             const int stride = lps / KP;
@@ -1184,6 +1188,8 @@
     if ((lmax_arg & ~(0xff | GN_LMAX_SLICED)) || !bwd_dim_ok_wide(F) || N < 0 || lmax < 1 || lmax > 8 || mode < 0 || mode > 31 ||
         act < 0 || act >= GN_ACT_COUNT)
         return GN_ERR_BAD_ARG;
+    if (!w && !(mode & GN_HTR_DIRECT) && (mode || lmax > 2 || F > 256 || act != GN_ACT_SILU || gn_use_highl(lmax_arg)))
+        return GN_ERR_BAD_ARG;
     if (N == 0) return GN_OK;
     hipStream_t st = (hipStream_t)stream;
     if (gn_use_highl(lmax_arg) || F > 256 || (!mode && act != GN_ACT_SILU))
@@ -1202,10 +1208,12 @@
 #define GN_HTRB(L, LLO, LHI, FIRST, FC) GN_HTRB_T(L, LLO, LHI, FIRST, FC); GN_HTRB_S(L, LLO, LHI, FC)
 #define GN_HTRB_ALL(FC)                                                                                          \
     if (lmax == 1) {                                                                                             \
-        hipLaunchKernelGGL((gn::htr_bwd_target_kernel<1, FC>), grid, block, 0, st, g_t_out, pre_t, w, EQ, EK, rl, rowptr, src, N, F, gEQ, g_rl, g_pre_t, act); \
+        if (w) hipLaunchKernelGGL((gn::htr_bwd_target_kernel<1, FC>), grid, block, 0, st, g_t_out, pre_t, w, EQ, EK, rl, rowptr, src, N, F, gEQ, g_rl, g_pre_t, act); \
+        else hipLaunchKernelGGL((gn::htr_bwd_target_kernel<1, FC, true>), grid, block, 0, st, g_t_out, pre_t, w, EQ, EK, rl, rowptr, src, N, F, gEQ, g_rl, g_pre_t, act); \
         hipLaunchKernelGGL((gn::htr_bwd_source_kernel<1, FC>), grid, block, 0, st, g_t_out, pre_t, EQ, EK, rl, colptr, perm, dst, N, F, gEK, act); \
     } else if (lmax == 2) {                                                                                      \
-        hipLaunchKernelGGL((gn::htr_bwd_target_kernel<2, FC>), grid, block, 0, st, g_t_out, pre_t, w, EQ, EK, rl, rowptr, src, N, F, gEQ, g_rl, g_pre_t, act); \
+        if (w) hipLaunchKernelGGL((gn::htr_bwd_target_kernel<2, FC>), grid, block, 0, st, g_t_out, pre_t, w, EQ, EK, rl, rowptr, src, N, F, gEQ, g_rl, g_pre_t, act); \
+        else hipLaunchKernelGGL((gn::htr_bwd_target_kernel<2, FC, true>), grid, block, 0, st, g_t_out, pre_t, w, EQ, EK, rl, rowptr, src, N, F, gEQ, g_rl, g_pre_t, act); \
         hipLaunchKernelGGL((gn::htr_bwd_source_kernel<2, FC>), grid, block, 0, st, g_t_out, pre_t, EQ, EK, rl, colptr, perm, dst, N, F, gEK, act); \
     } else if (lmax == 3) {                                                                                      \
         if (GN_HTRB_TGT_MODE == 1) { GN_HTRB_T(3, 1, 3, true, FC); }                                             \
diff --git a/gotennet_amd/csrc/gn_gata.hip b/gotennet_amd/csrc/gn_gata.hip
--- a/gotennet_amd/csrc/gn_gata.hip
+++ b/gotennet_amd/csrc/gn_gata.hip
@@ -2,6 +2,7 @@
 #include "gn_tune.h"
 #include "gn_highl.h"
 #include "gn_dropout.h"
+#include "gn_htr.h"
 
 namespace gn {
 
@@ -415,10 +416,11 @@
     message_aggregate_group_body<LMAX, SEP_DIR, SEP_TENSOR, LLO, LHI, SCALAR, FC>(GN_MSG_GROUP_PASS);
 }
 
-template <int LMAX, int FC = 0>
+template <int LMAX, int FC = 0, bool UPD = false, bool STW = true>
 __global__ __launch_bounds__(256) GN_WPE(GN_W_HTR_EDGE) void htr_edge_kernel(
     const float* __restrict__ EQ, const float* __restrict__ EK, const float* __restrict__ rl,
-    const int* __restrict__ rowptr, const int* __restrict__ src, int N, int F_rt, float* __restrict__ w) {
+    const int* __restrict__ rowptr, const int* __restrict__ src, int N, int F_rt, float* __restrict__ w,
+    const float* __restrict__ t, const float* __restrict__ pre_t, float* __restrict__ t2) {
     constexpr int D = (LMAX + 1) * (LMAX + 1) - 1;
     constexpr bool CLOSED = LMAX == 3 && GN_HTR_CLOSED;
     const int F = FC ? FC : F_rt;
@@ -432,6 +434,19 @@
     for (int e = e0 + slot; e < e1; e += ns) {
         const float* kj = EK + (size_t)src[e] * D * F + c0;
         const float* re = rl + (size_t)e * D;
+        float4 te = zero4(), pe = zero4();
+        if constexpr (UPD) {
+            te = ld4(t + (size_t)e * F + c0);
+            pe = ld4_nt(pre_t + (size_t)e * F + c0);
+        }
+        auto finish = [&](float4 wsum) __attribute__((always_inline)) {
+            if constexpr (UPD) {
+                if constexpr (STW) st4_nt(w + (size_t)e * F + c0, wsum);
+                st4(t2 + (size_t)e * F + c0, te + act4(pe, GN_ACT_SILU) * wsum);
+            } else {
+                st4_nt(w + (size_t)e * F + c0, wsum);
+            }
+        };
         float4 wsum = zero4();
         int m0 = 0;
 #if GN_HTR_CLOSED_ALL
@@ -442,20 +457,8 @@
             for (int m = 0; m < D; ++m) { eka[m] = ld4(kj + (size_t)m * F); ra[m] = re[m]; }
             __builtin_amdgcn_sched_barrier(0);
 #pragma unroll
-            for (int l = 1; l <= LMAX; ++l) {
-                float4 pq = zero4(), pk = zero4(), ab = zero4();
-                float rr = 0.f;
-#pragma unroll
-                for (int mm = 0; mm < 2 * l + 1; ++mm) {
-                    const int m = l * l - 1 + mm;
-                    rr = fmaf(ra[m], ra[m], rr);
-                    pq = fma4(ra[m], eq[m], pq);
-                    pk = fma4(ra[m], eka[m], pk);
-                    ab = fma4(eq[m], eka[m], ab);
-                }
-                wsum = wsum + (ab + (pq * pk) * (rr - 2.0f));
-            }
-            st4_nt(w + (size_t)e * F + c0, wsum);
+            for (int l = 1; l <= LMAX; ++l) wsum = htr_w_closed_l(l, eq + (l * l - 1), eka + (l * l - 1), ra + (l * l - 1), wsum);
+            finish(wsum);
             continue;
         }
 #endif
@@ -463,41 +466,15 @@
         for (int l = 1; l <= LMAX; ++l) {
             float4 ek[2 * LMAX + 1];
             float r[2 * LMAX + 1];
-            float4 pq = zero4(), pk = zero4();
-            if constexpr (CLOSED) {
-                float4 ab = zero4();
-                float rr = 0.f;
-#pragma unroll
-                for (int mm = 0; mm < 2 * l + 1; ++mm) {
-                    ek[mm] = ld4(kj + (size_t)(m0 + mm) * F);
-                    r[mm] = re[m0 + mm];
-                }
-#pragma unroll
-                for (int mm = 0; mm < 2 * l + 1; ++mm) {
-                    rr = fmaf(r[mm], r[mm], rr);
-                    pq = fma4(r[mm], eq[m0 + mm], pq);
-                    pk = fma4(r[mm], ek[mm], pk);
-                    ab = fma4(eq[m0 + mm], ek[mm], ab);
-                }
-                wsum = wsum + (ab + (pq * pk) * (rr - 2.0f));
-            } else {
-#pragma unroll
-                for (int mm = 0; mm < 2 * l + 1; ++mm) {
-                    ek[mm] = ld4(kj + (size_t)(m0 + mm) * F);
-                    r[mm] = re[m0 + mm];
-                    pq = fma4(r[mm], eq[m0 + mm], pq);
-                    pk = fma4(-r[mm], ek[mm], pk);
-                }
-#pragma unroll
-                for (int mm = 0; mm < 2 * l + 1; ++mm) {
-                    const float4 a_ = eq[m0 + mm] + pq * (-r[mm]);
-                    const float4 b_ = ek[mm] + pk * r[mm];
-                    wsum = fma4(a_, b_, wsum);
-                }
+#pragma unroll
+            for (int mm = 0; mm < 2 * l + 1; ++mm) {
+                ek[mm] = ld4(kj + (size_t)(m0 + mm) * F);
+                r[mm] = re[m0 + mm];
             }
+            wsum = CLOSED ? htr_w_closed_l(l, eq + m0, ek, r, wsum) : htr_w_literal_l(l, eq + m0, ek, r, wsum);
             m0 += 2 * l + 1;
         }
-        st4_nt(w + (size_t)e * F + c0, wsum);
+        finish(wsum);
     }
 }
 
@@ -674,14 +651,44 @@
     if (gn_use_highl(lmax_arg)) return gn_highl_htr_edge(EQ, EK, rl, rowptr, src, N, F, lmax, mode, w_raw, w, st);
     if (mode) return gn_htr_edge_general(EQ, EK, rl, rowptr, src, N, F, lmax, mode, w_raw, w, st);
     const dim3 grid(gn::xcd_grid(N)), block(256);
+    const float* const no_t = nullptr;
+    float* const no_t2 = nullptr;
 #define GN_HTR_EDGE(FC)                                                                                                  \
     switch (lmax) {                                                                                                      \
-        case 1: hipLaunchKernelGGL((gn::htr_edge_kernel<1, FC>), grid, block, 0, st, EQ, EK, rl, rowptr, src, N, F, w); break; \
-        case 2: hipLaunchKernelGGL((gn::htr_edge_kernel<2, FC>), grid, block, 0, st, EQ, EK, rl, rowptr, src, N, F, w); break; \
-        case 3: hipLaunchKernelGGL((gn::htr_edge_kernel<3, FC>), grid, block, 0, st, EQ, EK, rl, rowptr, src, N, F, w); break; \
-        default: hipLaunchKernelGGL((gn::htr_edge_kernel<4, FC>), grid, block, 0, st, EQ, EK, rl, rowptr, src, N, F, w); break; \
+        case 1: hipLaunchKernelGGL((gn::htr_edge_kernel<1, FC>), grid, block, 0, st, EQ, EK, rl, rowptr, src, N, F, w, no_t, no_t, no_t2); break; \
+        case 2: hipLaunchKernelGGL((gn::htr_edge_kernel<2, FC>), grid, block, 0, st, EQ, EK, rl, rowptr, src, N, F, w, no_t, no_t, no_t2); break; \
+        case 3: hipLaunchKernelGGL((gn::htr_edge_kernel<3, FC>), grid, block, 0, st, EQ, EK, rl, rowptr, src, N, F, w, no_t, no_t, no_t2); break; \
+        default: hipLaunchKernelGGL((gn::htr_edge_kernel<4, FC>), grid, block, 0, st, EQ, EK, rl, rowptr, src, N, F, w, no_t, no_t, no_t2); break; \
     }
     if (F == 256) { GN_HTR_EDGE(256) } else { GN_HTR_EDGE(0) }
+#undef GN_HTR_EDGE
     GN_LAUNCH_CHECK();
     return GN_OK;
 }
+
+extern "C" int gn_htr_edge_update(const float* EQ, const float* EK, const float* rl, const int* rowptr, const int* src,
+                                  int N, int F, int lmax_arg, const float* t, const float* pre_t, int act, float* w, float* t2,
+                                  void* stream) {
+    const int lmax = lmax_arg & 0xff;
+    if ((lmax_arg & ~0xff) || !feature_dim_ok(F) || F > 256 || N < 0 || lmax < 1 || lmax > 4 || gn_use_highl(lmax_arg) ||
+        act != GN_ACT_SILU)
+        return GN_ERR_BAD_ARG;
+    if (N == 0) return GN_OK;
+    hipStream_t st = (hipStream_t)stream;
+    const dim3 grid(gn::xcd_grid(N)), block(256);
+#define GN_HTR_EDGE_UPD_W(L, FC)                                                                                         \
+    if (w) hipLaunchKernelGGL((gn::htr_edge_kernel<L, FC, true, true>), grid, block, 0, st, EQ, EK, rl, rowptr, src, N, F, w, t, pre_t, t2); \
+    else hipLaunchKernelGGL((gn::htr_edge_kernel<L, FC, true, false>), grid, block, 0, st, EQ, EK, rl, rowptr, src, N, F, w, t, pre_t, t2)
+#define GN_HTR_EDGE_UPD(FC)                                                                                              \
+    switch (lmax) {                                                                                                      \
+        case 1: GN_HTR_EDGE_UPD_W(1, FC); break; \
+        case 2: GN_HTR_EDGE_UPD_W(2, FC); break; \
+        case 3: GN_HTR_EDGE_UPD_W(3, FC); break; \
+        default: GN_HTR_EDGE_UPD_W(4, FC); break; \
+    }
+    if (F == 256) { GN_HTR_EDGE_UPD(256) } else { GN_HTR_EDGE_UPD(0) }
+#undef GN_HTR_EDGE_UPD
+#undef GN_HTR_EDGE_UPD_W
+    GN_LAUNCH_CHECK();
+    return GN_OK;
+}
diff --git a/gotennet_amd/csrc/gn_gemm.h b/gotennet_amd/csrc/gn_gemm.h
--- a/gotennet_amd/csrc/gn_gemm.h
+++ b/gotennet_amd/csrc/gn_gemm.h
@@ -18,6 +18,7 @@
     int nt_store;
     int act_kind;
     int lda2;
+    const float* W2; const float* bias2; float* C2; int ldc2, c_seg;
 };
 
 constexpr int GN_MAX_GROUP = 4;
diff --git a/gotennet_amd/csrc/gn_gemm.hip b/gotennet_amd/csrc/gn_gemm.hip
--- a/gotennet_amd/csrc/gn_gemm.hip
+++ b/gotennet_amd/csrc/gn_gemm.hip
@@ -573,10 +573,10 @@
     return 1;
 }
 
-static int gemm_group_impl(const gn_gemm_desc* d, int n, void* stream, int split) {
+static int gemm_group_impl(const gn_gemm_desc* d, int n, void* stream, int split, const gn_gemm_seg* segs = nullptr) {
     if (n < 0 || n > gn::GN_MAX_GROUP || (n > 0 && !d)) return GN_ERR_BAD_ARG;
     gn::GemmArgs g[gn::GN_MAX_GROUP];
-    int m = 0;
+    int m = 0, nseg = 0;
     for (int i = 0; i < n; ++i) {
         const gn_gemm_desc& q = d[i];
         if (!gemm_args_ok(q.M, q.N, q.K, q.lda, q.ldc, q.act_lo, q.act_hi, q.row_cnt, q.res, q.gate, q.gate_mode,
@@ -592,7 +592,16 @@
         if (q.act_kind < 0 || q.act_kind >= GN_ACT_COUNT) return GN_ERR_BAD_ARG;
         g[m - 1].act_kind = q.act_kind;
         g[m - 1].lda2 = q.lda2 ? q.lda2 : q.lda;
-    }
+        if (segs && segs[i].c_seg) {
+            const gn_gemm_seg& sg = segs[i];
+            if (sg.c_seg < 0 || (sg.c_seg % 128) || sg.c_seg >= q.N || !sg.W2 || !sg.C2 || (sg.ldc2 & 3) ||
+                sg.ldc2 < q.N - sg.c_seg || q.act_hi > sg.c_seg)
+                return GN_ERR_BAD_ARG;
+            g[m - 1].W2 = sg.W2; g[m - 1].bias2 = sg.bias2; g[m - 1].C2 = sg.C2; g[m - 1].ldc2 = sg.ldc2; g[m - 1].c_seg = sg.c_seg;
+            ++nseg;
+        }
+    }
+    if (m + nseg > gn::GN_MAX_GROUP) return GN_ERR_BAD_ARG;
     if (m == 0) return GN_OK;
     return gn_gemm_launch(g, m, (hipStream_t)stream, split);
 }
@@ -600,8 +609,45 @@
 extern "C" int gn_gemm_group(const gn_gemm_desc* d, int n, void* stream) { return gemm_group_impl(d, n, stream, 0); }
 extern "C" int gn_gemm_group_split(const gn_gemm_desc* d, int n, void* stream) { return gemm_group_impl(d, n, stream, 1); }
 extern "C" int gn_gemm_group_f16x2(const gn_gemm_desc* d, int n, void* stream) { return gemm_group_impl(d, n, stream, 2); }
+extern "C" int gn_gemm_group_seg(const gn_gemm_desc* d, const gn_gemm_seg* segs, int n, int arith, void* stream) {
+    if (arith < 0 || arith > 2 || (n > 0 && !segs)) return GN_ERR_BAD_ARG;
+    return gemm_group_impl(d, n, stream, arith, segs);
+}
+
+static int nt_first_column(int M, int N, int K) {
+    const double nt_min = (double)GN_GEMM_NT_MB * 1048576.0;
+    const int nt_lo = GN_GEMM_NT_LO >= 0 ? GN_GEMM_NT_LO : K;
+    return (double)M * N * 4.0 >= nt_min ? (N > nt_lo ? nt_lo : 0) : 0x7fffffff;
+}
 
 int gn_gemm_launch(const gn::GemmArgs* g, int n, hipStream_t st, int split) {
+    bool seg = false;
+    for (int i = 0; i < n; ++i) seg = seg || g[i].c_seg != 0;
+    if (seg) {
+        gn::GemmArgs s[gn::GN_MAX_GROUP];
+        if (split == 2) {
+            for (int i = 0; i < n; ++i) {
+                s[i] = g[i];
+                s[i].nt_store = nt_first_column(g[i].M, g[i].c_seg ? g[i].c_seg : g[i].N, g[i].K);
+            }
+            const int r = gn_gemm_colpipe_launch(s, n, st);
+            if (r != 0) return r > 0 ? GN_OK : -r;
+        }
+        int m = 0;
+        for (int i = 0; i < n; ++i) {
+            if (m + (g[i].c_seg ? 2 : 1) > gn::GN_MAX_GROUP) return GN_ERR_BAD_ARG;
+            gn::GemmArgs a = g[i];
+            a.W2 = a.bias2 = nullptr; a.C2 = nullptr; a.ldc2 = a.c_seg = 0;
+            if (g[i].c_seg) a.N = g[i].c_seg;
+            s[m++] = a;
+            if (g[i].c_seg) {
+                a.W = g[i].W2; a.bias = g[i].bias2; a.C = g[i].C2; a.ldc = g[i].ldc2; a.N = g[i].N - g[i].c_seg;
+                a.res = a.gate = nullptr; a.pre_out = nullptr; a.gate_mode = a.act_lo = a.act_hi = 0;
+                s[m++] = a;
+            }
+        }
+        return gn_gemm_launch(s, m, st, split);
+    }
 #ifndef GN_SPLIT_GRID
 #define GN_SPLIT_GRID 14
 #endif
@@ -634,11 +680,9 @@
     }
     const bool mid = wide && !use_big && gated && GN_F16_MID_ROWS > 0 && rows_all >= (long)GN_F16_MID_ROWS;
     long end = 0;
-    const double nt_min = (double)GN_GEMM_NT_MB * 1048576.0;
     for (int i = 0; i < gn::GN_MAX_GROUP; ++i) {
         ga.g[i] = g[i < n ? i : n - 1];
-        const int nt_lo = GN_GEMM_NT_LO >= 0 ? GN_GEMM_NT_LO : ga.g[i].K;
-        ga.g[i].nt_store = (double)ga.g[i].M * ga.g[i].N * 4.0 >= nt_min ? (ga.g[i].N > nt_lo ? nt_lo : 0) : 0x7fffffff;
+        ga.g[i].nt_store = nt_first_column(ga.g[i].M, ga.g[i].N, ga.g[i].K);
         if (i < n) end += use_big ? (long)((g[i].M + BMB - 1) / BMB) * ((g[i].N + BNB - 1) / BNB)
                                   : (mid ? (long)((g[i].M + 63) / 64) * ((g[i].N + 127) / 128)
                                   : wide ? (long)((g[i].M + 31) / 32) * ((g[i].N + 127) / 128)
diff --git a/gotennet_amd/csrc/gn_gemm_colpipe.hip b/gotennet_amd/csrc/gn_gemm_colpipe.hip
--- a/gotennet_amd/csrc/gn_gemm_colpipe.hip
+++ b/gotennet_amd/csrc/gn_gemm_colpipe.hip
@@ -59,18 +59,21 @@
         int k = (int)k0l;
         const int k1 = (int)k1l;
         if (k >= k1) continue;
-        const uint4* const wfrag = reinterpret_cast<const uint4*>(p.W) + 16 + lane;
+        const int ps_seg = p.c_seg ? p.c_seg / BN : npass;
         const int ewt = __builtin_amdgcn_readfirstlane(*reinterpret_cast<const int*>(p.W));
-        const int nt_last = (N + 31) / 32 - 1;
-        auto boff = [&](int ps) -> unsigned {
-            int nt = ps * 4 + wave;
+        const int dew = p.c_seg ? __builtin_amdgcn_readfirstlane(*reinterpret_cast<const int*>(p.W2)) - ewt : 0;
+        auto boff = [&](int ps) -> const uint4* {
+            const bool sg = ps >= ps_seg;
+            const int nseg = sg ? N - ps_seg * BN : (N < ps_seg * BN ? N : ps_seg * BN);
+            int nt = (ps - (sg ? ps_seg : 0)) * 4 + wave;
+            const int nt_last = (nseg + 31) / 32 - 1;
             nt = nt < nt_last ? nt : nt_last;
-            return (unsigned)nt * (NS * 128u);
+            return reinterpret_cast<const uint4*>(sg ? p.W2 : p.W) + 16 + (unsigned)nt * (NS * 128u) + lane;
         };
         uint4 bq[NB][2];
-        auto load_b = [&](unsigned bo, int g, uint4 (&q)[2]) __attribute__((always_inline)) {
-            q[0] = wfrag[bo + (unsigned)g * 128u];
-            q[1] = wfrag[bo + (unsigned)g * 128u + 64u];
+        auto load_b = [&](const uint4* bo, int g, uint4 (&q)[2]) __attribute__((always_inline)) {
+            q[0] = bo[(unsigned)g * 128u];
+            q[1] = bo[(unsigned)g * 128u + 64u];
         };
         const int kind = GN_ACT_SILU;
         const float* const res = p.res; const float* const gate = p.gate; float* const pre_out = p.pre_out; float* const C = p.C;
@@ -90,7 +93,7 @@
 #pragma unroll
                 for (int u = 0; u < RPW; ++u)
                     va[u] = ld4(Ak + (size_t)__builtin_amdgcn_readlane(prow_v, 4 * u + wave) * lda);
-                const unsigned bo0 = boff(ps0);
+                const uint4* const bo0 = boff(ps0);
 #pragma unroll
                 for (int g = 0; g < NB; ++g) load_b(bo0, g, bq[g]);
 #pragma unroll
@@ -136,8 +139,13 @@
                 const int i = g >> 3, sub = g & 7;
                 const int gn = ps * BN + wave * 32 + 4 * c4;
                 const bool col_ok = gn < N;
+                const bool sg = ps >= ps_seg;
+                const float* const bias_s = sg ? (p.bias2 ? p.bias2 - ps_seg * BN : nullptr) : bias;
+                const float* const res_s = sg ? nullptr : res; const float* const gate_s = sg ? nullptr : gate;
+                float* const pre_s = sg ? nullptr : pre_out; float* const C_s = sg ? p.C2 - ps_seg * BN : C;
+                const int ld_s = sg ? p.ldc2 : ldc, nt_s = sg ? 0x7fffffff : nt_store, de_s = sg ? dew : 0;
                 if (sub == 0) {
-                    if (i == 0) bias4 = (bias && col_ok) ? ld4(bias + gn) : zero4();
+                    if (i == 0) bias4 = (bias_s && col_ok) ? ld4(bias_s + gn) : zero4();
                     __builtin_amdgcn_wave_barrier();
 #pragma unroll
                     for (int gg = 0; gg < 4; ++gg)
@@ -150,13 +158,13 @@
                         const int rr = 8 * q + rq;
                         t[q] = ld4(scr + rr * 32 + ((c4 ^ (rr & 7)) << 2));
                     }
-                    if (res || gate) {
+                    if (res_s || gate_s) {
 #pragma unroll
                         for (int q = 0; q < 4; ++q) {
                             const bool ok = m0 + i * 32 + 8 * q + rq < M && col_ok;
-                            const size_t off = (size_t)prow_e[i][q] * ldc + gn;
-                            rv[q] = (ok && res) ? ld4(res + off) : zero4();
-                            gv[q] = (ok && gate) ? ld4(gate + off) : zero4();
+                            const size_t off = (size_t)prow_e[i][q] * ld_s + gn;
+                            rv[q] = (ok && res_s) ? ld4(res_s + off) : zero4();
+                            gv[q] = (ok && gate_s) ? ld4(gate_s + off) : zero4();
                         }
                     }
                     __builtin_amdgcn_wave_barrier();
@@ -167,21 +175,21 @@
                         const int q = (sub == 4 ? 0 : 2) + qq;
                         const bool ok = m0 + i * 32 + 8 * q + rq < M && col_ok;
                         if (!ok) continue;
-                        const size_t off = (size_t)prow_e[i][q] * ldc + gn;
-                        const int e = e_r[i][q];
+                        const size_t off = (size_t)prow_e[i][q] * ld_s + gn;
+                        const int e = e_r[i][q] + de_s;
                         float4 v = make_float4(ldexpf(t[q].x, e), ldexpf(t[q].y, e), ldexpf(t[q].z, e), ldexpf(t[q].w, e)) + bias4;
-                        if (pre_out) st4(pre_out + off, v);
+                        if (pre_s) st4(pre_s + off, v);
                         if (act) v = act4(v, kind);
-                        if (gate) v = v * (gate_mode ? dact4(gv[q], kind) : gv[q]);
-                        if (res) v = rv[q] + v;
-                        if (gn >= nt_store) st4_nt(C + off, v); else st4(C + off, v);
+                        if (gate_s) v = v * (gate_mode ? dact4(gv[q], kind) : gv[q]);
+                        if (res_s) v = rv[q] + v;
+                        if (gn >= nt_s) st4_nt(C_s + off, v); else st4(C_s + off, v);
                     }
                 }
             };
             auto pass = [&](auto PP, auto EE, int ps, bool has_next) __attribute__((always_inline)) {
                 constexpr int P = decltype(PP)::value;
                 constexpr bool EPI = decltype(EE)::value;
-                const unsigned bo = boff(ps), bo_next = boff(has_next ? ps + 1 : ps);
+                const uint4* const bo = boff(ps); const uint4* const bo_next = boff(has_next ? ps + 1 : ps);
                 f16x8 ab[2][TM][2];
                 read_a(0, ab[0]);
 #pragma unroll
diff --git a/gotennet_amd/csrc/gn_htr.h b/gotennet_amd/csrc/gn_htr.h
--- /dev/null
+++ b/gotennet_amd/csrc/gn_htr.h
@@ -0,0 +1,55 @@
+#pragma once
+#include "gn_common.h"
+
+namespace gn {
+
+
+template <int NR>
+__device__ __forceinline__ float4 htr_w_literal(const float4* eq, const float4* ek, const float* r, float4 wsum) {
+    float4 pq = zero4(), pk = zero4();
+#pragma unroll
+    for (int mm = 0; mm < NR; ++mm) {
+        pq = fma4(r[mm], eq[mm], pq);
+        pk = fma4(-r[mm], ek[mm], pk);
+    }
+#pragma unroll
+    for (int mm = 0; mm < NR; ++mm) {
+        const float4 a_ = eq[mm] + pq * (-r[mm]);
+        const float4 b_ = ek[mm] + pk * r[mm];
+        wsum = fma4(a_, b_, wsum);
+    }
+    return wsum;
+}
+
+template <int NR>
+__device__ __forceinline__ float4 htr_w_closed(const float4* eq, const float4* ek, const float* r, float4 wsum) {
+    float4 pq = zero4(), pk = zero4(), ab = zero4();
+    float rr = 0.f;
+#pragma unroll
+    for (int mm = 0; mm < NR; ++mm) {
+        rr = fmaf(r[mm], r[mm], rr);
+        pq = fma4(r[mm], eq[mm], pq);
+        pk = fma4(r[mm], ek[mm], pk);
+        ab = fma4(eq[mm], ek[mm], ab);
+    }
+    return wsum + (ab + (pq * pk) * (rr - 2.0f));
+}
+
+__device__ __forceinline__ float4 htr_w_literal_l(int l, const float4* eq, const float4* ek, const float* r, float4 wsum) {
+    switch (l) {
+        case 1: return htr_w_literal<3>(eq, ek, r, wsum);
+        case 2: return htr_w_literal<5>(eq, ek, r, wsum);
+        case 3: return htr_w_literal<7>(eq, ek, r, wsum);
+        default: return htr_w_literal<9>(eq, ek, r, wsum);
+    }
+}
+__device__ __forceinline__ float4 htr_w_closed_l(int l, const float4* eq, const float4* ek, const float* r, float4 wsum) {
+    switch (l) {
+        case 1: return htr_w_closed<3>(eq, ek, r, wsum);
+        case 2: return htr_w_closed<5>(eq, ek, r, wsum);
+        case 3: return htr_w_closed<7>(eq, ek, r, wsum);
+        default: return htr_w_closed<9>(eq, ek, r, wsum);
+    }
+}
+
+}
diff --git a/gotennet_amd/engine.py b/gotennet_amd/engine.py
--- a/gotennet_amd/engine.py
+++ b/gotennet_amd/engine.py
@@ -48,11 +48,21 @@
 ZERO_X_FIRST = os.environ.get("GN_ZERO_X_FIRST", "1") != "0"
 MSG_BWD_PAIR = False
 DT_KCAT = True
+EDGE_NCAT = True
 
 
 def zero_X_in(cfg: "Config", li: int) -> bool:
     return (ZERO_X_FIRST and li == 0 and cfg.lmax <= 4 and cfg.act == 0 and not cfg.steerable_norm and not cfg.sliced
             and cfg.aggr == 0 and not cfg.wide)
+
+
+def _edge_ncat(cfg: "Config") -> bool:
+    return (EDGE_NCAT and not cfg.composed_update and cfg.htr_mode == 0 and cfg.act == 0 and cfg.lmax <= 4
+            and not cfg.sliced and not cfg.wide and cfg.Fe == cfg.F)
+
+
+def _w_recomputed(cfg: "Config") -> bool:
+    return _edge_ncat(cfg) and cfg.lmax <= 2
 
 
 def derived(holder, key, build):
@@ -200,6 +210,14 @@
     for i0 in range(0, len(problems), 4):
         chunk = problems[i0:i0 + 4]
         arr = (_lib.GemmDesc * len(chunk))()
+        segs = None
+        if any(q.get("c_seg") for q in chunk):
+            segs = (_lib.GemmSeg * len(chunk))()
+            for sg, q in zip(segs, chunk):
+                if q.get("c_seg"):
+                    sg.c_seg, sg.ldc2 = q["c_seg"], q["ldc2"]
+                    sg.W2 = ptr(split_weight(q["W2"], mode) if split else q["W2"])
+                    sg.bias2, sg.C2 = ptr(q.get("bias2")), ptr(q["C2"])
         for d, q in zip(arr, chunk):
             g = q.get
             act, rowmap, pro = g("act", (0, 0)), g("rowmap", (1, 1, 0)), g("pro", (0, 0, 0))
@@ -222,7 +240,10 @@
             d.A2, d.A3, d.a_seg = ptr(g("A2")), ptr(g("A3")), g("a_seg", 0)
             d.act_kind = g("kind", kind)
             d.lda2 = g("lda2", 0)
-        call(_PLANE_MODES[mode][1] if split else "gn_gemm_group", arr, len(chunk), _stream())
+        if segs is not None:
+            call("gn_gemm_group_seg", arr, segs, len(chunk), {"f32": 0, "split": 1, "f16x2": 2}[mode], _stream())
+        else:
+            call(_PLANE_MODES[mode][1] if split else "gn_gemm_group", arr, len(chunk), _stream())
 
 
 class _Call:
@@ -450,20 +471,33 @@
     if save:
         lt.nproj, lt.pre_g1 = new(N, 4 * F_), new(N, F_)
     if not last:
-        lt.EQ, lt.EK, lt.w = new(N, D, Fe), new(N, D, Fe), new(E, Fe)
+        lt.EQ, lt.EK = new(N, D, Fe), new(N, D, Fe)
+        ncat = _edge_ncat(cfg)
+        if not ncat or (save and (pgrads or not _w_recomputed(cfg))):
+            lt.w = new(E, Fe)
+        if save or ncat:
+            lt.pre_t = new(E, F_)
         if save:
-            lt.pre_t = new(E, F_)
             lt.w_raw = new(E, Fe) if (cfg.htr_mode >> 2) else None
     if pgrads:
         lt.nact, lt.g1act = new(N, 4 * F_), new(N, F_)
     return lt, new(N, F_), new(N, D, F_), (None if last else new(E, F_))
 
 
-def _gata_forward(p: _Call, lw: LayerWeights, lt: LayerTape, nact, h, X, t, h2, X2, li: int = 0):
+def _gata_forward(p: _Call, lw: LayerWeights, lt: LayerTape, nact, h, X, t, h2, X2, li: int = 0, pre_t=None):
     cfg, g, st, F_, lde, N, E, first = p.cfg, p.g, p.st, p.F, p.lde, p.N, p.E, lt.first
     H, M, xs, vs, eproj, attn = cfg.H, cfg.M, lt.xs, lt.vs, lt.eproj, lt.attn
     ne, nv = p.cols[first]
-    p.group([dict(A=t, lda=F_, W=_rows(lw, "We", ne) if first else lw.We, bias=lw.be, C=eproj, ldc=lde, rows=E, nout=ne, K=F_),
+    ep = dict(A=t, lda=F_, W=_rows(lw, "We", ne) if first else lw.We, bias=lw.be, C=eproj, ldc=lde, rows=E, nout=ne, K=F_)
+    if pre_t is not None:
+        if ne % 128 == 0:
+            ep.update(nout=ne + F_, c_seg=ne, W2=lw.Wt, bias2=lw.bt, C2=pre_t, ldc2=F_)
+            pt = None
+        else:
+            pt = dict(A=t, lda=F_, W=lw.Wt, bias=lw.bt, C=pre_t, ldc=F_, rows=E, nout=F_, K=F_)
+    else:
+        pt = None
+    p.group([ep, pt,
              dict(A=h, lda=F_, W=lw.Wn1, bias=lw.bn1, C=nact, ldc=4 * F_, rows=N, nout=4 * F_, K=F_,
                   act=(2 * F_, 4 * F_), pre_out=lt.nproj)])
     p.group([dict(A=nact, lda=4 * F_, W=_rows(lw, "Ws2", nv) if first else lw.Ws2, bias=lw.bs2, C=xs, ldc=M * F_, rows=N,
@@ -499,6 +533,10 @@
         m0 = dict(A=ctx, lda=2 * F_, W=lw.Wm0, bias=lw.bm0, C=g1act, ldc=F_, rows=N, nout=F_, K=2 * F_, act=(0, F_),
                   pre_out=lt.pre_g1)
     if last:
+        p.group([m0])
+    elif _edge_ncat(cfg):
+        call("gn_htr_edge_update", ptr(lt.EQ), ptr(lt.EK), ptr(g.rl), ptr(g.rowptr), ptr(g.src), N, Fe, cfg.lmax_arg,
+             ptr(t), ptr(lt.pre_t), cfg.act, ptr(lt.w), ptr(t2), st)
         p.group([m0])
     else:
         call("gn_htr_edge", ptr(lt.EQ), ptr(lt.EK), ptr(g.rl), ptr(g.rowptr), ptr(g.src), N, Fe, cfg.lmax_arg, cfg.htr_mode,
@@ -554,7 +592,7 @@
             if pgrads:
                 nact, g1act = lt.nact, lt.g1act
         lt.first = first
-        _gata_forward(p, lw, lt, nact, h, X, t, h2, X2, li)
+        _gata_forward(p, lw, lt, nact, h, X, t, h2, X2, li, lt.pre_t if (lw.Wt is not None and _edge_ncat(cfg)) else None)
         h, h2 = h2, h
         X, X2 = X2, X
         if pgrads:
diff --git a/include/gotennet_hip.h b/include/gotennet_hip.h
--- a/include/gotennet_hip.h
+++ b/include/gotennet_hip.h
@@ -105,6 +105,13 @@
                   const float* a_gate, int ldg, int act_kind, void* stream);
 int gn_gemm_group_f16x2(const gn_gemm_desc* problems, int n, void* stream);
 
+typedef struct gn_gemm_seg {
+    int c_seg;
+    const float* W2; const float* bias2;
+    float* C2; int ldc2;
+} gn_gemm_seg;
+int gn_gemm_group_seg(const gn_gemm_desc* problems, const gn_gemm_seg* segs, int n, int arith, void* stream);
+
 int gn_attn_softmax(const float* q, const float* k, int ldqk, const float* t_attn, int ldt,
                     const int* rowptr, const int* src, const int* outdeg,
                     int N, int F, int H, float* a, int act , void* stream);
@@ -137,6 +144,9 @@
 #define GN_HTR_DIRECT 16
 int gn_htr_edge(const float* EQ, const float* EK, const float* rl, const int* rowptr, const int* src,
                 int N, int F, int lmax, int mode, float* w_raw, float* w, void* stream);
+int gn_htr_edge_update(const float* EQ, const float* EK, const float* rl, const int* rowptr, const int* src,
+                       int N, int F, int lmax, const float* t, const float* pre_t, int act, float* w, float* t2,
+                       void* stream);
 
 int gn_eqff_context(const float* h, const float* Xp, float eps, int N, int F, int D, float* ctx, void* stream);
 int gn_eqff_update(const float* m, const float* Xp, int N, int F, int D, float* h, float* X, void* stream);
```

Result: no change. 22380 molecules/s (-0.0%).
